# Samsung/tf-fast-rnnt

Hardware: AMD Instinct MI355X
Metric: rnnt_loss_pruned_fwd_bwd_throughput (higher is better)
Workload: dtype f32; 1 GPU; c3: rnnt_loss_pruned fwd+bwd step, B=32/GPU T=1000 S=200 C=500 s_range=5, regular, full boundary, first pass rnnt_loss_simple; global_batch=32, am_pruned=broadcast view

## Files before the change

### tf-fast-rnnt_amd/csrc/capi.hip

```cpp
#include "ftr_common.h"
#ifdef FTR_DIAG
#include "../../include/ftr_diag.h"
#endif
#include <stdlib.h>
#include <string.h>

namespace ftr {
namespace {
thread_local char g_err[512] = {0};
#ifdef FTR_DIAG
int g_mi_impl = -1;
#endif

int device_ok() {
  int n = 0;
  hipError_t e = hipGetDeviceCount(&n);
  if (e != hipSuccess || n <= 0) {
    (void)hipGetLastError();
    set_error("no usable HIP device (%s); this library has no CPU path", e == hipSuccess ? "device count is 0" : hipGetErrorString(e));
    return FTR_ERR_NO_DEVICE;
  }
  return FTR_OK;
}

// ... 547 lines not shown
  clear_error();
  FTR_TRY(check_builder(what, B >= 0 && T >= 1 && S >= 0 && C >= 1 && r >= 1, termination_symbol, C, true, hat));
  FTR_TRY(check_scale_stride(what, scale_stride));
  if (B == 0) return FTR_OK;
  FTR_TRY(pointers_then_device(what, logits && ranges && lse && gpy && glogits && (symbols || S == 0) && (gpx || S == 0)));
  return pruned_logprobs_bwd(logits, dtype, symbols, ranges, boundary, termination_symbol, lse, gpx, gpy, Scale{scale, scale_stride, scale_mul}, glogits, B, T, S, C, r, modified, hat, stream_of(stream));
}

int ftr_pruned_logprobs_bwd_scaled_f32(const float* logits, const int32_t* symbols, const int32_t* ranges,
                                       const int32_t* boundary, int termination_symbol, const float* lse,
                                       const float* gpx, const float* gpy, const float* scale, int scale_stride,
                                       float scale_mul, float* glogits, int B, int T, int S, int C, int r,
                                       int modified, void* stream) {
  return pruned_logprobs_bwd_scaled_entry(logits, FTR_DTYPE_F32, symbols, ranges, boundary, termination_symbol, lse, gpx, gpy, scale, scale_stride, scale_mul, glogits, B, T, S, C, r, modified, 0, stream);
}

int ftr_hat_pruned_logprobs_bwd_scaled_f32(const float* logits, const int32_t* symbols, const int32_t* ranges,
                                           const int32_t* boundary, int termination_symbol, const float* lse,
                                           const float* gpx, const float* gpy, const float* scale, int scale_stride,
                                           float scale_mul, float* glogits, int B, int T, int S, int C, int r,
                                           int modified, void* stream) {
  return pruned_logprobs_bwd_scaled_entry(logits, FTR_DTYPE_F32, symbols, ranges, boundary, termination_symbol, lse, gpx, gpy, scale, scale_stride, scale_mul, glogits, B, T, S, C, r, modified, 1, stream);
}

int ftr_pruned_logprobs_bwd_scaled_dt(const void* logits, int kind, const int32_t* symbols, const int32_t* ranges,
                                      const int32_t* boundary, int termination_symbol, const float* lse,
                                      const float* gpx, const float* gpy, const float* scale, int scale_stride,
                                      float scale_mul, void* glogits, int B, int T, int S, int C, int r, int modified,
                                      int flags, void* stream) {
  clear_error();
  FTR_TRY(check_dtype("pruned_logprobs_bwd_scaled_dt", kind, flags));
  return pruned_logprobs_bwd_scaled_entry(logits, kind, symbols, ranges, boundary, termination_symbol, lse, gpx, gpy, scale, scale_stride, scale_mul, glogits, B, T, S, C, r, modified, flags & FTR_PRUNED_HAT, stream);
}

int ftr_simple_logprobs_fused_supported(int C) { return simple_fused_supported(C); }
int ftr_simple_logprobs_fused_bwd_supported(int T, int C) { return simple_fused_bwd_supported(T, C); }

int ftr_normalizer_gemm_f32(int kind, const float* x, const float* y, float* out, int B, int T, int S1, int C, void* stream) {
  FTR_REQUIRE(B >= 0 && T >= 0 && S1 >= 0 && C >= 0, "normalizer_gemm: bad sizes");
  if ((size_t)B * T * S1 * C == 0) return FTR_OK;
  FTR_REQUIRE(x && y && out, "normalizer_gemm: null pointer");
  return normalizer_gemm(kind, x, y, out, B, T, S1, C, reinterpret_cast<hipStream_t>(stream));
}

int ftr_normalizer_gemm_choice(int kind, int B, int T, int S1, int C, int* solution, float* us, float* us_default, int* candidates) {
  return normalizer_gemm_choice(kind, B, T, S1, C, solution, us, us_default, candidates);
}

int ftr_normalizer_gemm_set_choice(int kind, int B, int T, int S1, int C, int solution) {
  return normalizer_gemm_set_choice(kind, B, T, S1, C, solution);
}

static int fused_fwd_entry(const char* what, bool smoothed, const float* am, const float* lm, const int32_t* symbols,
                           const float* am_probs, const float* lm_probs, const float* am_max, const float* lm_max,
                           const float* lmonly_norm, const float* amonly_norm, const float* unigram_log,
                           const int32_t* boundary, int termination_symbol, double delay_penalty, float combined_scale,
                           float lm_only_scale, float am_only_scale, float* px, float* py, float* prod, int B, int T,
                           int S, int C, int modified, void* stream) {
  clear_error();
  FTR_TRY(check_builder(what, B >= 0 && T >= 1 && S >= 0 && C >= 1, termination_symbol, C));
  if (B == 0) return FTR_OK;
  FTR_TRY(pointers_then_device(what, am && lm && am_probs && lm_probs && am_max && lm_max && (!smoothed || (lmonly_norm && amonly_norm && unigram_log)) && py && (symbols || S == 0) && (px || S == 0)));
  return simple_fused_fwd(am, lm, symbols, am_probs, lm_probs, am_max, lm_max, boundary, termination_symbol, delay_penalty, lmonly_norm, amonly_norm, unigram_log, combined_scale, lm_only_scale, am_only_scale, px, py, prod, B, T, S, C, modified, stream_of(stream));
}

int ftr_simple_logprobs_fused_fwd_f32(const float* am, const float* lm, const int32_t* symbols, const float* am_probs,
                                      const float* lm_probs, const float* am_max, const float* lm_max,
                                      const int32_t* boundary, int termination_symbol, double delay_penalty, float* px,
                                      float* py, float* prod, int B, int T, int S, int C, int modified, void* stream) {
  return fused_fwd_entry("simple_logprobs_fused_fwd", false, am, lm, symbols, am_probs, lm_probs, am_max, lm_max, nullptr, nullptr, nullptr, boundary, termination_symbol, delay_penalty, 1.0f, 0.0f, 0.0f, px, py, prod, B, T, S, C, modified, stream);
}

int ftr_smoothed_logprobs_fused_fwd_f32(const float* am, const float* lm, const int32_t* symbols, const float* am_probs,
                                        const float* lm_probs, const float* am_max, const float* lm_max,
                                        const float* lmonly_norm, const float* amonly_norm, const float* unigram_log,
                                        const int32_t* boundary, int termination_symbol, double delay_penalty,
                                        float combined_scale, float lm_only_scale, float am_only_scale, float* px,
                                        float* py, float* prod, int B, int T, int S, int C, int modified, void* stream) {
  return fused_fwd_entry("smoothed_logprobs_fused_fwd", true, am, lm, symbols, am_probs, lm_probs, am_max, lm_max, lmonly_norm, amonly_norm, unigram_log, boundary, termination_symbol, delay_penalty, combined_scale, lm_only_scale, am_only_scale, px, py, prod, B, T, S, C, modified, stream);
}

static int fused_bwd_am_entry(const char* what, bool smoothed, const float* gpx, const float* gpy, const float* scale,
                              int scale_stride, float scale_mul, const float* prod, const float* lm_probs,
                              const float* am_probs, const int32_t* symbols, const int32_t* boundary,
                              int termination_symbol, float combined_scale, float direct_scale, const float* unigram,
                              const float* am_dot, float am_only_scale, float* R, float* d_am, int B, int T, int S, int C,
                              int modified, void* stream) {
  clear_error();
  FTR_TRY(check_builder(what, B >= 0 && T >= 1 && S >= 0 && C >= 1, termination_symbol, C, true));
  FTR_TRY(check_scale_stride(what, scale_stride));
  if (B == 0) return FTR_OK;
  FTR_TRY(pointers_then_device(what, gpy && prod && lm_probs && am_probs && d_am && (!smoothed || (unigram && am_dot && R)) && (gpx || S == 0) && (symbols || S == 0)));
  return simple_fused_bwd_am(gpx, gpy, Scale{scale, scale_stride, scale_mul}, prod, lm_probs, am_probs, symbols, boundary, termination_symbol, combined_scale, direct_scale, unigram, am_dot, am_only_scale, R, d_am, B, T, S, C, modified, stream_of(stream));
}

int ftr_simple_logprobs_fused_bwd_am_f32(const float* gpx, const float* gpy, const float* scale, int scale_stride,
                                         float scale_mul, const float* prod, const float* lm_probs, const float* am_probs,
                                         const int32_t* symbols, const int32_t* boundary, int termination_symbol,
                                         float* d_am, int B, int T, int S, int C, int modified, void* stream) {
  return fused_bwd_am_entry("simple_logprobs_fused_bwd_am", false, gpx, gpy, scale, scale_stride, scale_mul, prod, lm_probs, am_probs, symbols, boundary, termination_symbol, 1.0f, 1.0f, nullptr, nullptr, 0.0f, nullptr, d_am, B, T, S, C, modified, stream);
}

int ftr_smoothed_logprobs_fused_bwd_am_f32(const float* gpx, const float* gpy, const float* scale, int scale_stride,
                                           float scale_mul, const float* prod, const float* lm_probs,
                                           const float* am_probs, const int32_t* symbols, const int32_t* boundary,
                                           int termination_symbol, float combined_scale, float direct_scale,
                                           const float* unigram, const float* am_dot, float am_only_scale, float* R,
                                           float* d_am, int B, int T, int S, int C, int modified, void* stream) {
  return fused_bwd_am_entry("smoothed_logprobs_fused_bwd_am", true, gpx, gpy, scale, scale_stride, scale_mul, prod, lm_probs, am_probs, symbols, boundary, termination_symbol, combined_scale, direct_scale, unigram, am_dot, am_only_scale, R, d_am, B, T, S, C, modified, stream);
}

static int fused_bwd_am_w_entry(const char* what, bool smoothed, const float* gpx, const float* gpy, const float* scale,
                                int scale_stride, float scale_mul, const float* W, const float* lm_probs,
                                const float* am_probs, const int32_t* symbols, const int32_t* boundary,
                                int termination_symbol, float direct_scale, const float* unigram, const float* am_dot,
                                float am_only_scale, float* R, float* d_am, int B, int T, int S, int C, int modified,
                                void* stream) {
  clear_error();
  FTR_TRY(check_builder(what, B >= 0 && T >= 1 && S >= 0 && C >= 1, termination_symbol, C, true));
  FTR_TRY(check_scale_stride(what, scale_stride));
  if (B == 0) return FTR_OK;
  FTR_TRY(pointers_then_device(what, gpy && W && lm_probs && am_probs && d_am && (!smoothed || (unigram && am_dot && R)) && (gpx || S == 0) && (symbols || S == 0)));
  return simple_fused_bwd_am_w(gpx, gpy, Scale{scale, scale_stride, scale_mul}, W, lm_probs, am_probs, symbols, boundary, termination_symbol, direct_scale, unigram, am_dot, am_only_scale, R, d_am, B, T, S, C, modified, stream_of(stream));
}

int ftr_simple_logprobs_fused_bwd_am_w_f32(const float* gpx, const float* gpy, const float* scale, int scale_stride,
                                           float scale_mul, const float* W, const float* lm_probs, const float* am_probs,
                                           const int32_t* symbols, const int32_t* boundary, int termination_symbol,
                                           float* d_am, int B, int T, int S, int C, int modified, void* stream) {
  return fused_bwd_am_w_entry("simple_logprobs_fused_bwd_am_w", false, gpx, gpy, scale, scale_stride, scale_mul, W, lm_probs, am_probs, symbols, boundary, termination_symbol, 1.0f, nullptr, nullptr, 0.0f, nullptr, d_am, B, T, S, C, modified, stream);
}

int ftr_smoothed_logprobs_fused_bwd_am_w_f32(const float* gpx, const float* gpy, const float* scale, int scale_stride,
                                             float scale_mul, const float* W, const float* lm_probs,
                                             const float* am_probs, const int32_t* symbols, const int32_t* boundary,
                                             int termination_symbol, float direct_scale, const float* unigram,
                                             const float* am_dot, float am_only_scale, float* R, float* d_am, int B, int T,
                                             int S, int C, int modified, void* stream) {
  return fused_bwd_am_w_entry("smoothed_logprobs_fused_bwd_am_w", true, gpx, gpy, scale, scale_stride, scale_mul, W, lm_probs, am_probs, symbols, boundary, termination_symbol, direct_scale, unigram, am_dot, am_only_scale, R, d_am, B, T, S, C, modified, stream);
}

int ftr_simple_logprobs_fused_bwd_am_w_columns(int B, int T, int C) { return simple_fused_bwd_columns(B, T, C); }

int ftr_mutual_information_band_supported(int T, int S, int r) { return mi_band_supported(T, S, r); }

static int pruned_band_fwd_entry(const void* logits, int dtype, const int32_t* symbols, const int32_t* ranges, const int32_t* boundary,
                                 int termination_symbol, double delay_penalty, float* lse, float* px_band, float* py_band,
                                 int B, int T, int S, int C, int r, int modified, int hat, void* stream) {
  const char* what = hat ? "hat_pruned_band_fwd" : "pruned_band_fwd";
  clear_error();
  FTR_TRY(check_builder(what, B >= 0 && T >= 1 && S >= 0 && C >= 1 && r >= 1, termination_symbol, C, false, hat));
  if (B == 0) return FTR_OK;
  FTR_TRY(pointers_then_device(what, logits && ranges && lse && px_band && py_band && (symbols || S == 0)));
  FTR_TRY(lse_rows_dtype(logits, dtype, lse, (size_t)B * T * r, C, termination_symbol, hat, stream_of(stream)));
  return band_gather(logits, dtype, symbols, ranges, boundary, lse, termination_symbol, delay_penalty, px_band, py_band, B, T, S, C, r, modified, hat, stream_of(stream));
}

int ftr_pruned_band_fwd_f32(const float* logits, const int32_t* symbols, const int32_t* ranges, const int32_t* boundary,
                            int termination_symbol, double delay_penalty, float* lse, float* px_band, float* py_band,
                            int B, int T, int S, int C, int r, int modified, void* stream) {
  return pruned_band_fwd_entry(logits, FTR_DTYPE_F32, symbols, ranges, boundary, termination_symbol, delay_penalty, lse, px_band, py_band, B, T, S, C, r, modified, 0, stream);
}

int ftr_hat_pruned_band_fwd_f32(const float* logits, const int32_t* symbols, const int32_t* ranges, const int32_t* boundary,
                                int termination_symbol, double delay_penalty, float* lse, float* px_band, float* py_band,
                                int B, int T, int S, int C, int r, int modified, void* stream) {
  return pruned_band_fwd_entry(logits, FTR_DTYPE_F32, symbols, ranges, boundary, termination_symbol, delay_penalty, lse, px_band, py_band, B, T, S, C, r, modified, 1, stream);
}

int ftr_pruned_band_fwd_dt(const void* logits, int kind, const int32_t* symbols, const int32_t* ranges,
                           const int32_t* boundary, int termination_symbol, double delay_penalty, float* lse,
                           float* px_band, float* py_band, int B, int T, int S, int C, int r, int modified, int flags,
                           void* stream) {
  clear_error();
  FTR_TRY(check_dtype("pruned_band_fwd_dt", kind, flags));
  return pruned_band_fwd_entry(logits, kind, symbols, ranges, boundary, termination_symbol, delay_penalty, lse, px_band, py_band, B, T, S, C, r, modified, flags & FTR_PRUNED_HAT, stream);
}

int ftr_band_ranges_check_i32(const int32_t* ranges, const int32_t* boundary, int32_t* flags, int B, int T, int r, void* stream) {
  clear_error();
  FTR_TRY(check_sizes("band_ranges_check", B >= 0 && T >= 0 && r >= 1));
  FTR_TRY(pointers_then_device("band_ranges_check", flags && (ranges || B == 0 || T == 0)));
  return band_ranges_check(ranges, boundary, flags, B, T, r, stream_of(stream));
}

int ftr_mutual_information_band_f32(const float* px_band, const float* py_band, const int32_t* ranges,
                                    const int32_t* boundary, float* ans, float* gx_band, float* gy_band, int B, int T,
                                    int S, int r, int modified, void* stream) {
  return ftr_mutual_information_band_ws_f32(px_band, py_band, ranges, boundary, nullptr, 0, ans, gx_band, gy_band, B, T, S, r, modified, stream);
}

size_t ftr_mutual_information_band_workspace_floats(int B, int T, int S, int r) {
  return (B < 0 || T < 1 || S < 0 || r < 1) ? 0 : mi_band_workspace_floats(B, T, S, r);
}

int ftr_mutual_information_band_ws_f32(const float* px_band, const float* py_band, const int32_t* ranges,
                                       const int32_t* boundary, float* workspace, size_t workspace_floats, float* ans,
                                       float* gx_band, float* gy_band, int B, int T, int S, int r, int modified,
                                       void* stream) {
  clear_error();
  FTR_TRY(check_sizes("mutual_information_band", B >= 0 && T >= 1 && S >= 0 && r >= 1));
  if (B == 0) return FTR_OK;
  FTR_TRY(pointers_then_device("mutual_information_band", px_band && py_band && ranges && ans && gx_band && gy_band));
  return mi_band(px_band, py_band, ranges, boundary, workspace, workspace_floats, ans, gx_band, gy_band, B, T, S, r, modified, stream_of(stream));
}

static int pruned_band_bwd_scaled_entry(const void* logits, int dtype, const int32_t* symbols, const int32_t* ranges,
                                        const int32_t* boundary, int termination_symbol, const float* lse,
                                        const float* gx_band, const float* gy_band, const float* scale, int scale_stride,
                                        float scale_mul, void* glogits, int B, int T, int S, int C, int r, int modified,
                                        int hat, void* stream) {
  const char* what = hat ? "hat_pruned_band_bwd_scaled" : "pruned_band_bwd_scaled";
  clear_error();
  FTR_TRY(check_builder(what, B >= 0 && T >= 1 && S >= 0 && C >= 1 && r >= 1, termination_symbol, C, true, hat));
  FTR_TRY(check_scale_stride(what, scale_stride));
  if (B == 0) return FTR_OK;
  FTR_TRY(pointers_then_device(what, logits && ranges && lse && gx_band && gy_band && glogits && (symbols || S == 0)));
  return band_grad_banded(logits, dtype, symbols, ranges, boundary, termination_symbol, lse, gx_band, gy_band, Scale{scale, scale_stride, scale_mul}, glogits, B, T, S, C, r, modified, hat, stream_of(stream));
}

int ftr_pruned_band_bwd_scaled_f32(const float* logits, const int32_t* symbols, const int32_t* ranges,
                                   const int32_t* boundary, int termination_symbol, const float* lse,
                                   const float* gx_band, const float* gy_band, const float* scale, int scale_stride,
                                   float scale_mul, float* glogits, int B, int T, int S, int C, int r, int modified,
                                   void* stream) {
  return pruned_band_bwd_scaled_entry(logits, FTR_DTYPE_F32, symbols, ranges, boundary, termination_symbol, lse, gx_band, gy_band, scale, scale_stride, scale_mul, glogits, B, T, S, C, r, modified, 0, stream);
}

int ftr_hat_pruned_band_bwd_scaled_f32(const float* logits, const int32_t* symbols, const int32_t* ranges,
                                       const int32_t* boundary, int termination_symbol, const float* lse,
                                       const float* gx_band, const float* gy_band, const float* scale, int scale_stride,
                                       float scale_mul, float* glogits, int B, int T, int S, int C, int r, int modified,
                                       void* stream) {
  return pruned_band_bwd_scaled_entry(logits, FTR_DTYPE_F32, symbols, ranges, boundary, termination_symbol, lse, gx_band, gy_band, scale, scale_stride, scale_mul, glogits, B, T, S, C, r, modified, 1, stream);
}

int ftr_pruned_band_bwd_scaled_dt(const void* logits, int kind, const int32_t* symbols, const int32_t* ranges,
                                  const int32_t* boundary, int termination_symbol, const float* lse,
                                  const float* gx_band, const float* gy_band, const float* scale, int scale_stride,
                                  float scale_mul, void* glogits, int B, int T, int S, int C, int r, int modified,
                                  int flags, void* stream) {
  clear_error();
  FTR_TRY(check_dtype("pruned_band_bwd_scaled_dt", kind, flags));
  return pruned_band_bwd_scaled_entry(logits, kind, symbols, ranges, boundary, termination_symbol, lse, gx_band, gy_band, scale, scale_stride, scale_mul, glogits, B, T, S, C, r, modified, flags & FTR_PRUNED_HAT, stream);
}

namespace {
int mb_check_durations(const char* what, const int32_t* durations, int D, bool first_is_one) {
  FTR_REQUIRE(D >= 1 && D <= 8, "%s: D = %d, the number of blanks must be in 1..8", what, D);
  FTR_REQUIRE(durations, "%s: null durations", what);
  for (int j = 0; j < D; ++j) {
    FTR_REQUIRE(durations[j] >= 1 && durations[j] <= 32, "%s: durations[%d] = %d is outside 1..32", what, j, durations[j]);
    FTR_REQUIRE(j == 0 || durations[j] > durations[j - 1], "%s: durations must be strictly increasing (durations[%d] = %d after %d)",
                what, j, durations[j], durations[j - 1]);
  }
  FTR_REQUIRE(!first_is_one || durations[0] == 1, "%s: durations[0] = %d, the standard blank advances one frame", what, durations[0]);
  return FTR_OK;
}
int mb_check_ids(const char* what, const int32_t* ids, int D, int blank, int C) {
  FTR_REQUIRE(C >= 1 && blank >= 0 && blank < C, "%s: termination_symbol %d not in [0,%d)", what, blank, C);
  FTR_REQUIRE(ids || D == 1, "%s: null big_blank_ids", what);
  for (int j = 0; j + 1 < D; ++j) {
    FTR_REQUIRE(ids[j] >= 0 && ids[j] < C, "%s: big_blank_ids[%d] = %d not in [0,%d)", what, j, ids[j], C);
    FTR_REQUIRE(ids[j] != blank, "%s: big_blank_ids[%d] = %d is the termination_symbol", what, j, ids[j]);
    for (int i = 0; i < j; ++i)
      FTR_REQUIRE(ids[i] != ids[j], "%s: big_blank_ids[%d] = %d is a duplicate of big_blank_ids[%d]", what, j, ids[j], i);
  }
  return FTR_OK;
}
}

namespace {
int tdt_check_list(const char* what, const char* name, const int32_t* v, int n, int nmax, int lo, int hi = 16) {
  FTR_REQUIRE(n >= 1 && n <= nmax, "%s: %s holds %d values, must be 1..%d", what, name, n, nmax);
  FTR_REQUIRE(v, "%s: null %s", what, name);
  for (int j = 0; j < n; ++j) {
    FTR_REQUIRE(v[j] >= lo && v[j] <= hi, "%s: %s[%d] = %d is outside %d..%d", what, name, j, v[j], lo, hi);
    FTR_REQUIRE(j == 0 || v[j] > v[j - 1], "%s: %s must be strictly increasing (%s[%d] = %d after %d)", what, name, name, j,
                v[j], v[j - 1]);
  }
  return FTR_OK;
}
int tdt_check_moves(const char* what, const int32_t* token_durations, int Dx, const int32_t* blank_durations, int Dy,
                    int blank_hi = 16) {
  FTR_TRY(tdt_check_list(what, "token_durations", token_durations, Dx, 8, 0));
  FTR_TRY(tdt_check_list(what, "blank_durations", blank_durations, Dy, 8, 1, blank_hi));
  FTR_REQUIRE(Dx + Dy <= 9, "%s: Dx + Dy = %d moves (token_durations and blank_durations together), at most 9", what, Dx + Dy);
  return FTR_OK;
}
int tdt_check_head(const char* what, const int32_t* durations, int N, double sigma, int blank, int C) {
  FTR_TRY(tdt_check_list(what, "durations", durations, N, 5, 0));
  FTR_REQUIRE(durations[N - 1] >= 1, "%s: durations holds no positive value: no move advances a frame", what);
  FTR_REQUIRE(sigma >= 0.0, "%s: sigma = %g must not be negative", what, sigma);
  FTR_REQUIRE(C >= 1 && blank >= 0 && blank < C, "%s: termination_symbol %d not in [0,%d)", what, blank, C);
  return FTR_OK;
}
}

size_t ftr_mutual_information_multiblank_workspace_floats(int B, int S, int T) {
  return mi_multiblank_workspace_floats(B, S, T);
}

int ftr_mutual_information_multiblank_fwd_f32(const float* px, const float* py, const int32_t* boundary,
                                              const int32_t* durations, int D, float* workspace, size_t workspace_floats,
                                              float* ans, int B, int S, int T, void* stream) {
  const char* what = "mutual_information_multiblank_fwd";
  clear_error();
  FTR_TRY(mb_check_durations(what, durations, D, false));
  FTR_TRY(check_lattice(what, B, S, T));
  if (B == 0) return FTR_OK;
  FTR_TRY(check_ws_size(what, workspace_floats, mi_multiblank_workspace_floats(B, S, T), "floats"));
  FTR_REQUIRE(workspace && ans && (py || T == 0) && (px || S == 0), "%s: null px / py / workspace / ans", what);
  FTR_TRY(check_ws_aligned(what, workspace));
  FTR_TRY(device_ok());
  return mi_multiblank_fwd(px, py, boundary, durations, D, workspace, workspace_floats, ans, B, S, T, stream_of(stream));
}

int ftr_mutual_information_multiblank_bwd_f32(const float* px, const float* py, const int32_t* boundary,
                                              const int32_t* durations, int D, float* workspace, size_t workspace_floats,
                                              const float* ans_grad, float* px_grad, float* py_grad, int B, int S, int T,
                                              void* stream) {
  const char* what = "mutual_information_multiblank_bwd";
  clear_error();
  FTR_TRY(mb_check_durations(what, durations, D, false));
  FTR_TRY(check_lattice(what, B, S, T));
  if (B == 0) return FTR_OK;
  FTR_TRY(check_ws_size(what, workspace_floats, mi_multiblank_workspace_floats(B, S, T), "floats"));
  FTR_REQUIRE(workspace && (py || T == 0) && (px || S == 0), "%s: null px / py / workspace", what);
  FTR_REQUIRE((py_grad || T == 0) && (px_grad || S == 0), "%s: null px_grad / py_grad", what);
// ... 201 lines not shown
```

### tf-fast-rnnt_amd/csrc/ftr_common.h

```cpp
#pragma once
#include <hip/hip_runtime.h>
#include <stdint.h>
#include <stdio.h>
#include <stdarg.h>
#include "../../include/ftr_kd.h"
#include "../../include/ftr_fused.h"

namespace ftr {

void set_error(const char* fmt, ...);
void clear_error();

inline int check_launch(const char* what) {
  hipError_t e = hipGetLastError();
  if (e != hipSuccess) {
    set_error("%s: launch failed: %s", what, hipGetErrorString(e));
    return FTR_ERR_LAUNCH;
  }
  return FTR_OK;
}

inline int require_rows_32bit(const char* what, size_t rows) {
  if (rows > 0x7fffffffull) {
    set_error("%s: %zu rows (B*T*s_range) exceed the 2^31 - 1 that the launch grids index", what, rows);
    return FTR_ERR_INVALID_ARG;
  }
  return FTR_OK;
}

__global__ void zero_words_kernel(uint32_t* __restrict__ p, size_t n);
__global__ void copy_words_kernel(uint32_t* __restrict__ dst, const uint32_t* __restrict__ src, size_t n);
inline int zero_words(void* p, size_t n_words, hipStream_t st, const char* what) {
  if (n_words == 0) return FTR_OK;
  const size_t blocks = (n_words + 4 * 256 - 1) / (4 * 256);
  hipLaunchKernelGGL(zero_words_kernel, dim3((unsigned)(blocks > 4096 ? 4096 : blocks)), dim3(256), 0, st, static_cast<uint32_t*>(p), n_words);
  return check_launch(what);
}
inline int copy_words(void* dst, const void* src, size_t n_words, hipStream_t st, const char* what) {
  if (n_words == 0) return FTR_OK;
  const size_t blocks = (n_words + 255) / 256;
  hipLaunchKernelGGL(copy_words_kernel, dim3((unsigned)(blocks > 4096 ? 4096 : blocks)), dim3(256), 0, st, static_cast<uint32_t*>(dst),
                     static_cast<const uint32_t*>(src), n_words);
  return check_launch(what);
}

constexpr float kNeg = -1.0e30f;
constexpr float kNegThresh = -1.0e29f;
constexpr float kLog2e = 1.4426950408889634f;
constexpr float kLn2 = 0.6931471805599453f;

typedef float f4u __attribute__((ext_vector_type(4), aligned(4)));
typedef float f4 __attribute__((ext_vector_type(4)));

struct bf16_t { uint16_t bits; };
struct fp16_t { uint16_t bits; };
typedef uint16_t h4 __attribute__((ext_vector_type(4)));

__device__ __forceinline__ float elem_to_float(float v) { return v; }
__device__ __forceinline__ float elem_to_float(bf16_t v) { return (float)__builtin_bit_cast(__bf16, v.bits); }
__device__ __forceinline__ float elem_to_float(fp16_t v) { return (float)__builtin_bit_cast(_Float16, v.bits); }
template <typename E> __device__ __forceinline__ E elem_from_float(float v);
template <> __device__ __forceinline__ float elem_from_float<float>(float v) { return v; }
template <> __device__ __forceinline__ bf16_t elem_from_float<bf16_t>(float v) { return bf16_t{__builtin_bit_cast(uint16_t, (__bf16)v)}; }
template <> __device__ __forceinline__ fp16_t elem_from_float<fp16_t>(float v) { return fp16_t{__builtin_bit_cast(uint16_t, (_Float16)v)}; }

__device__ __forceinline__ f4 load4(const float* row, int i) { return reinterpret_cast<const f4u*>(row)[i]; }
__device__ __forceinline__ void store4(float* row, int i, f4 v) { reinterpret_cast<f4u*>(row)[i] = v; }
template <typename E>
__device__ __forceinline__ f4 load4(const E* row, int i) {
  const h4 h = reinterpret_cast<const h4*>(row)[i];
  f4 v;
#pragma unroll
  for (int e = 0; e < 4; ++e) v[e] = elem_to_float(E{h[e]});
  return v;
}
template <typename E>
__device__ __forceinline__ void store4(E* row, int i, f4 v) {
  h4 h;
#pragma unroll
  for (int e = 0; e < 4; ++e) h[e] = elem_from_float<E>(v[e]).bits;
  reinterpret_cast<h4*>(row)[i] = h;
}

struct Scale {
  const float* p; int stride; float mul;
  __device__ __forceinline__ float at(int b) const { return (p ? p[(size_t)b * stride] : 1.0f) * mul; }
};
inline Scale scale_none() { return Scale{nullptr, 0, 1.0f}; }

template <int CTRL, int ROW_MASK, int BANK_MASK>
__device__ __forceinline__ float dpp_take(float identity, float src) {
  return __builtin_bit_cast(float, __builtin_amdgcn_update_dpp(__builtin_bit_cast(int, identity), __builtin_bit_cast(int, src),
                                                               CTRL, ROW_MASK, BANK_MASK, false));
}
__device__ __forceinline__ float wave_sum_dpp(float v) {
  v += dpp_take<0x111, 0xf, 0xf>(0.0f, v);
  v += dpp_take<0x112, 0xf, 0xf>(0.0f, v);
  v += dpp_take<0x114, 0xf, 0xe>(0.0f, v);
  v += dpp_take<0x118, 0xf, 0xc>(0.0f, v);
  v += dpp_take<0x142, 0xa, 0xf>(0.0f, v);
  v += dpp_take<0x143, 0xc, 0xf>(0.0f, v);
  return __builtin_bit_cast(float, __builtin_amdgcn_readlane(__builtin_bit_cast(int, v), 63));
}
__device__ __forceinline__ float wave_max_dpp(float v) {
  constexpr float ninf = -__builtin_inff();
  v = fmaxf(v, dpp_take<0x111, 0xf, 0xf>(ninf, v));
  v = fmaxf(v, dpp_take<0x112, 0xf, 0xf>(ninf, v));
  v = fmaxf(v, dpp_take<0x114, 0xf, 0xe>(ninf, v));
  v = fmaxf(v, dpp_take<0x118, 0xf, 0xc>(ninf, v));
  v = fmaxf(v, dpp_take<0x142, 0xa, 0xf>(ninf, v));
  v = fmaxf(v, dpp_take<0x143, 0xc, 0xf>(ninf, v));
  return __builtin_bit_cast(float, __builtin_amdgcn_readlane(__builtin_bit_cast(int, v), 63));
}

struct Shift { float cx2, cy2; };
__device__ __forceinline__ bool shift_sample_ok(float v) { return v > -1.0e4f && v < 1.0e4f; }
template <bool MOD>
__device__ __forceinline__ Shift shift_from_sums(float sumx, float nx, float sumy, float ny, int Sn, int Tn) {
  const float steps = MOD ? (float)(Tn - 1) : (float)(Sn - 1 + Tn - 1);
  float f = steps > 0.0f ? (float)(Sn - 1) / steps : 0.5f;
  f = fminf(fmaxf(f, 1.0e-3f), 1.0f - 1.0e-3f);
  const float mx = nx > 0.0f ? sumx / nx : 0.0f, my = ny > 0.0f ? sumy / ny : 0.0f;
  Shift s;
  s.cx2 = mx * kLog2e - __builtin_amdgcn_logf(f);
  s.cy2 = my * kLog2e - __builtin_amdgcn_logf(1.0f - f);
  return s;
}
template <bool MOD>
__device__ __forceinline__ double shift_total(const Shift s, int Sn, int Tn) {
  const int nx = Sn - 1, ny = MOD ? (Tn - 1) - (Sn - 1) : (Tn - 1);
  return (double)nx * (double)s.cx2 + (double)ny * (double)s.cy2;
}

struct Bound { int sb, tb, se, te; };
__device__ __forceinline__ Bound load_boundary(const int32_t* __restrict__ boundary, int b, int S, int T) {
  Bound r;
  if (boundary) {
    r.sb = max(boundary[4 * b + 0], 0); r.tb = max(boundary[4 * b + 1], 0);
    r.se = min(boundary[4 * b + 2], S); r.te = min(boundary[4 * b + 3], T);
  } else { r.sb = 0; r.tb = 0; r.se = S; r.te = T; }
  return r;
}

__device__ __forceinline__ float softplus(float v) { return fmaxf(v, 0.0f) + log1pf(expf(-fabsf(v))); }
__device__ __forceinline__ void hat_logprobs(float xb, float xs, float Z, bool sym_is_blank, float* vx, float* vy) {
  *vy = -softplus(-xb);
  *vx = sym_is_blank ? -INFINITY : (xs - Z) - softplus(xb);
}
__device__ __forceinline__ void hat_sigmoids(float xb, float* sp, float* sn) {
  const float e = expf(-fabsf(xb)), big = 1.0f / (1.0f + e), small = e / (1.0f + e);
  *sp = xb >= 0.0f ? big : small;
  *sn = xb >= 0.0f ? small : big;
}

}

namespace ftr {
int mi_plain_fwd(const float* px, const float* py, const int32_t* boundary, float* p, float* ans, int B, int S, int T, int modified, hipStream_t st);
int mi_plain_bwd(const float* px, const float* py, const int32_t* boundary, const float* p, float* p_grad, float* px_grad, float* py_grad, float* ans_grad, int overwrite, int B, int S, int T, int modified, hipStream_t st);
int mi_bidir_fwd(const float* px, const float* py, const int32_t* boundary, float* ws, size_t ws_floats, int flags, float* ans, int B, int S, int T, int modified, hipStream_t st);
int mi_bidir_bwd(const int32_t* boundary, const float* ws, size_t ws_floats, int flags, float* px_grad, float* py_grad, float* ans_grad, int overwrite, int B, int S, int T, int modified, hipStream_t st, const float* ans = nullptr, float* loss_out = nullptr, int loss_code = 0);
int mi_bidir_ws_init(float* ws, size_t ws_floats, int B, int S, int T, hipStream_t st);
int mi_bidir_status(const float* ws, size_t ws_floats, int B, int S, int T, int* status_host, long long* dirty_host, hipStream_t st);
size_t mi_bidir_workspace_floats(int B, int S, int T);
size_t mi_bidir_handoff_floats(int B, int S, int T);
size_t mi_viterbi_workspace_bytes(int B, int S, int T);
int mi_viterbi(const float* px, const float* py, const int32_t* boundary, void* ws, size_t ws_bytes, float* score, int32_t* frames, int B, int S, int T, int modified, hipStream_t st);
size_t mi_multiblank_workspace_floats(int B, int S, int T);
int mi_multiblank_fwd(const float* px, const float* py, const int32_t* boundary, const int32_t* durations, int D, float* ws, size_t ws_floats, float* ans, int B, int S, int T, hipStream_t st);
int mi_multiblank_bwd(const float* px, const float* py, const int32_t* boundary, const int32_t* durations, int D, float* ws, size_t ws_floats, const float* ans_grad, float* px_grad, float* py_grad, int B, int S, int T, hipStream_t st);
int multiblank_logprobs_fwd(const float* logits, const int32_t* symbols, const int32_t* ranges, const int32_t* boundary, int blank, const int32_t* big_ids, const int32_t* durations, int D, double sigma, double delay_penalty, float* lse, float* px, float* py, int B, int T, int S, int C, int r, hipStream_t st);
int multiblank_logprobs_bwd(const float* logits, const int32_t* symbols, const int32_t* ranges, const int32_t* boundary, int blank, const int32_t* big_ids, const int32_t* durations, int D, const float* lse, const float* gpx, const float* gpy, Scale scale, float* glogits, int B, int T, int S, int C, int r, hipStream_t st);
size_t mi_tdt_workspace_floats(int B, int S, int T);
int mi_tdt_fwd(const float* px, const float* py, const int32_t* boundary, const int32_t* token_durations, int Dx, const int32_t* blank_durations, int Dy, float* ws, size_t ws_floats, float* ans, int B, int S, int T, hipStream_t st);
int mi_tdt_bwd(const float* px, const float* py, const int32_t* boundary, const int32_t* token_durations, int Dx, const int32_t* blank_durations, int Dy, float* ws, size_t ws_floats, const float* ans_grad, float* px_grad, float* py_grad, int B, int S, int T, hipStream_t st);
int tdt_logprobs_fwd(const float* logits, const int32_t* symbols, const int32_t* ranges, const int32_t* boundary, int blank, const int32_t* durations, int N, double sigma, double delay_penalty, float* lse_tok, float* lse_dur, float* px, float* py, int B, int T, int S, int C, int r, hipStream_t st);
int tdt_logprobs_bwd(const float* logits, const int32_t* symbols, const int32_t* ranges, const int32_t* boundary, int blank, const int32_t* durations, int N, const float* lse_tok, const float* lse_dur, const float* gpx, const float* gpy, Scale scale, float* glogits, int B, int T, int S, int C, int r, hipStream_t st);
size_t mi_viterbi_tdt_workspace_bytes(int B, int S, int T);
int mi_viterbi_tdt(const float* px, const float* py, const int32_t* boundary, const int32_t* token_durations, int Dx, const int32_t* blank_durations, int Dy, void* ws, size_t ws_bytes, float* score, int32_t* frames, int32_t* durations, int32_t* blank_steps, int B, int S, int T, hipStream_t st);
int cummin_i32(const int32_t* in, int32_t* out, int rows, int cols, hipStream_t st);
int prune_ranges(const float* px_grad, const float* py_grad, const int32_t* boundary, int32_t* ranges, int32_t* s_begin, int B, int S, int T, int T1, int r, hipStream_t st);
int do_pruning(const float* am, const float* lm, const int32_t* ranges, float* am_p, float* lm_p, int B, int T, int S1, int C, int r, hipStream_t st);
size_t do_pruning_bwd_workspace_bytes(int B, int T, int S1, int C, int r);
int do_pruning_bwd_ws(const float* g_am_p, const float* g_lm_p, const int32_t* ranges, float* d_am, float* d_lm, int B, int T, int S1, int C, int r, void* ws, size_t ws_bytes, hipStream_t st);
int do_pruning_bwd(const float* g_am_p, const float* g_lm_p, const int32_t* ranges, float* d_am, float* d_lm, int B, int T, int S1, int C, int r, hipStream_t st);
int pruned_logprobs_fwd(const void* logits, int dtype, const int32_t* symbols, const int32_t* ranges, const int32_t* boundary, int blank, double delay_penalty, float* lse, float* px, float* py, int B, int T, int S, int C, int r, int modified, int hat, hipStream_t st);
int pruned_logprobs_bwd(const void* logits, int dtype, const int32_t* symbols, const int32_t* ranges, const int32_t* boundary, int blank, const float* lse, const float* gpx, const float* gpy, Scale scale, void* glogits, int B, int T, int S, int C, int r, int modified, int hat, hipStream_t st);
int simple_rowmax_exp(const float* x, float* probs, float* rowmax, float* rowsum, const float* dotvec, float* dot, size_t rows, int C, hipStream_t st);
int simple_rowmax_exp_pair(const float* x1, float* probs1, float* rowmax1, size_t rows1, const float* x2, float* probs2, float* rowmax2, size_t rows2, int C, hipStream_t st);
int simple_rowdot(const float* x, const float* v, float* dot, size_t rows, int C, hipStream_t st);
size_t simple_colsum_workspace_floats(size_t rows, int C);
int simple_colsum_weighted(const float* x, const float* w, float* out, float* ws, size_t ws_floats, size_t rows, int C, hipStream_t st);
int simple_logprobs_fwd(const float* am, const float* lm, const int32_t* symbols, const float* prod, const float* am_max, const float* lm_max, const int32_t* boundary, int blank, double delay_penalty, const float* lmonly_norm, const float* amonly_norm, const float* ulog, float cs, float ls, float as, float* px, float* py, int B, int T, int S, int C, int modified, hipStream_t st);
int simple_logprobs_bwd_w(const float* gpx, const float* gpy, Scale scale, const float* prod, const int32_t* boundary, float* W, float* rsx, float* rsy, float cs, int B, int T, int S, int modified, hipStream_t st);
int simple_logprobs_bwd_am(const float* gpx, const float* gpy, Scale scale, const float* damp, const float* am_probs, const int32_t* symbols, const int32_t* boundary, int blank, float kdir, const float* uvec, const float* amdot, float as, float* Rout, float* d_am, int B, int T, int S, int C, int modified, hipStream_t st);
int simple_logprobs_bwd_lm(const float* dlmp, const float* lm_probs, const int32_t* symbols, const float* rsx, const float* rsy, int blank, float kdir, const float* arow, const float* invsum, const float* gu, float* d_lm, int B, int S, int C, hipStream_t st);
int simple_fused_supported(int C);
int simple_fused_bwd_supported(int T, int C);
int normalizer_gemm(int kind, const float* x, const float* y, float* out, int B, int T, int S1, int C, hipStream_t st);
int normalizer_gemm_choice(int kind, int B, int T, int S1, int C, int* solution, float* us, float* us_default, int* candidates);
int normalizer_gemm_set_choice(int kind, int B, int T, int S1, int C, int solution);
int simple_fused_fwd(const float* am, const float* lm, const int32_t* symbols, const float* am_probs, const float* lm_probs, const float* am_max, const float* lm_max, const int32_t* boundary, int blank, double delay_penalty, const float* lmonly_norm, const float* amonly_norm, const float* ulog, float cs, float ls, float as, float* px, float* py, float* prod_out, int B, int T, int S, int C, int modified, hipStream_t st);
int simple_fused_bwd_am(const float* gpx, const float* gpy, Scale scale, const float* prod, const float* lm_probs, const float* am_probs, const int32_t* symbols, const int32_t* boundary, int blank, float cs, float kdir, const float* uvec, const float* amdot, float as, float* Rout, float* d_am, int B, int T, int S, int C, int modified, hipStream_t st);
int simple_fused_bwd_columns(int B, int T, int C);
int simple_fused_bwd_am_w(const float* gpx, const float* gpy, Scale scale, const float* W, const float* lm_probs, const float* am_probs, const int32_t* symbols, const int32_t* boundary, int blank, float kdir, const float* uvec, const float* amdot, float as, float* Rout, float* d_am, int B, int T, int S, int C, int modified, hipStream_t st);
int negated_reduce(const float* ans, int B, int reduction, float* out, hipStream_t st, float sign = -1.0f);
int pruned_kd_fwd(const void* logits, int dtype, const void* teacher, int teacher_dtype, const int32_t* symbols, const int32_t* ranges, const int32_t* boundary, int blank, float temperature, int collapsed, float* node, float* saved, float* utt, int B, int T, int S, int C, int r, hipStream_t st);
int pruned_kd_bwd(const void* logits, int dtype, const void* teacher, int teacher_dtype, const int32_t* symbols, const int32_t* ranges, const int32_t* boundary, int blank, float temperature, int collapsed, const float* saved, Scale scale, void* glogits, int B, int T, int S, int C, int r, hipStream_t st);
int lse_rows(const float* logits, float* lse, size_t rows, int C, int blank, int hat, hipStream_t st);
int lse_rows_dtype(const void* logits, int dtype, float* lse, size_t rows, int C, int blank, int hat, hipStream_t st);
int mi_band_supported(int T, int S, int r);
int band_ranges_check(const int32_t* ranges, const int32_t* boundary, int* flags, int B, int T, int r, hipStream_t st);
int band_gather(const void* logits, int dtype, const int32_t* symbols, const int32_t* ranges, const int32_t* boundary, const float* lse, int blank, double delay_penalty, float* pxb, float* pyb, int B, int T, int S, int C, int r, int modified, int hat, hipStream_t st);
size_t mi_band_workspace_floats(int B, int T, int S, int r);
int mi_band_seg_supported(int T, int S, int r);
size_t mi_band_seg_workspace_floats(int B, int T, int S, int r);
int mi_band_seg(const float* pxb, const float* pyb, const int32_t* ranges, const int32_t* boundary, float* ws, size_t ws_floats, float* ans, float* gxb, float* gyb, int B, int T, int S, int r, int modified, hipStream_t st);
int mi_band(const float* pxb, const float* pyb, const int32_t* ranges, const int32_t* boundary, float* ws, size_t ws_floats, float* ans, float* gxb, float* gyb, int B, int T, int S, int r, int modified, hipStream_t st);
int band_grad_banded(const void* logits, int dtype, const int32_t* symbols, const int32_t* ranges, const int32_t* boundary, int blank, const float* lse, const float* gxb, const float* gyb, Scale scale, void* glogits, int B, int T, int S, int C, int r, int modified, int hat, hipStream_t st);
int selftest(hipStream_t st, int* result_dev);
int debug_stamps(unsigned long long* out16);
int debug_trace(unsigned long long* out, int n);
}
```

### tf-fast-rnnt_amd/csrc/mi_band.hip

```cpp
#include "ftr_common.h"
#include "launch.h"
#include <type_traits>
#include <cstdlib>

namespace ftr {
namespace {

constexpr int kBandThreads = 512;

__device__ __forceinline__ float dpp_row_ror1(float v) {
  return __builtin_bit_cast(float, __builtin_amdgcn_update_dpp(0, __builtin_bit_cast(int, v), 0x121, 0xf, 0xf, false));
}
template <int N>
__device__ __forceinline__ float dpp_row_ror(float v) {
  return __builtin_bit_cast(float, __builtin_amdgcn_update_dpp(0, __builtin_bit_cast(int, v), 0x120 + N, 0xf, 0xf, false));
}
__device__ __forceinline__ float row16_max(float v) {
  v = fmaxf(v, dpp_row_ror<8>(v)); v = fmaxf(v, dpp_row_ror<4>(v));
  v = fmaxf(v, dpp_row_ror<2>(v)); v = fmaxf(v, dpp_row_ror<1>(v));
  return v;
}
__device__ __forceinline__ float row16_sum(float v) {
  v += dpp_row_ror<8>(v); v += dpp_row_ror<4>(v); v += dpp_row_ror<2>(v); v += dpp_row_ror<1>(v);
  return v;
}

template <typename E, bool MOD, bool HAT>
__global__ void band_gather_kernel(const E* __restrict__ logits, const int32_t* __restrict__ symbols,
                                   const int32_t* __restrict__ ranges, const int32_t* __restrict__ boundary,
                                   const float* __restrict__ lse, int blank, double delay_penalty,
                                   float* __restrict__ pxb, float* __restrict__ pyb, size_t rows, int T, int S, int C, int r) {
  const size_t row = (size_t)blockIdx.x * blockDim.x + threadIdx.x;
  if (row >= rows) return;
  const size_t bt = row / r;
  const int k = (int)(row - bt * r);
  const int b = (int)(bt / T);
  const int t = (int)(bt - (size_t)b * T);
  const int s = ranges[bt * r] + k;
  const int te = boundary ? boundary[4 * b + 3] : T;
  const float l = lse[row];
  float vy = -INFINITY, vx = -INFINITY;
  if (s >= 0 && s <= S) {
    if (HAT) {
      const float xb = elem_to_float(logits[row * C + blank]);
      int c = blank;
      if (s < S) c = min(max(symbols[(size_t)b * S + s], 0), C - 1);
      hat_logprobs(xb, elem_to_float(logits[row * C + c]), l, c == blank, &vx, &vy);
    } else {
      vy = elem_to_float(logits[row * C + blank]) - l;
    }
    if (s < S) {
      if (!HAT) vx = elem_to_float(logits[row * C + min(max(symbols[(size_t)b * S + s], 0), C - 1)]) - l;
      if (!MOD && t == te) vx = -INFINITY;
      if (delay_penalty > 0.0) vx += (float)((((double)te - 1.0) / 2.0 - (double)t) * delay_penalty);
    }
  }
  pxb[row] = vx;
  pyb[row] = vy;
}

__global__ void band_ranges_check_kernel(const int32_t* __restrict__ ranges, const int32_t* __restrict__ boundary,
                                         int* __restrict__ flags, int B, int T, int r) {
  const size_t bt = (size_t)blockIdx.x * blockDim.x + threadIdx.x;
  int bad = 0;
  if (bt < (size_t)B * T) {
    const int b = (int)(bt / T), t = (int)(bt - (size_t)b * T);
    const int tb = boundary ? max(boundary[4 * b + 1], 0) : 0, te = boundary ? min(boundary[4 * b + 3], T) : T;
    if (t >= tb && t < te) {
      const int32_t* row = ranges + bt * r;
      const int s0 = row[0];
      if (t > tb && s0 < row[-r]) bad |= 1;
      for (int k = 1; k < r; ++k) if (row[k] != s0 + k) bad |= 2;
    }
  }
  if (__any(bad != 0)) {
    int all = 0;
    for (int bit = 1; bit <= 2; bit <<= 1) if (__any((bad & bit) != 0)) all |= bit;
    if ((threadIdx.x & 63) == 0) atomicOr(flags, all);
  }
}

#ifdef FTR_BAND_STAMPS
static __device__ unsigned long long g_bstamp[16];
#define FTR_BSTAMP(k) do { if (b == 0 && tid == 0) g_bstamp[k] = __builtin_amdgcn_s_memrealtime(); } while (0)
#else
#define FTR_BSTAMP(k) do {} while (0)
#endif
constexpr int kBandAhead = 4;
constexpr int kRenormEvery = 4;
template <int LANES>
__host__ __device__ inline size_t band_lds_bytes(int T, int S) {
  const size_t ncap = ((size_t)S + T + 5 + 4 * kBandAhead) * LANES;
  return sizeof(int) * ((size_t)(T + 2) + 32) + sizeof(float) * (3 * ncap + 48) + 64;
}

template <bool MOD, int LANES>
__global__ __launch_bounds__(kBandThreads) void mi_band_kernel(
    const float* __restrict__ pxb, const float* __restrict__ pyb, const int32_t* __restrict__ ranges,
    const int32_t* __restrict__ boundary, float* __restrict__ ans, float* __restrict__ gxb, float* __restrict__ gyb,
    int B, int T, int S, int r, unsigned rinv) {
  extern __shared__ __attribute__((aligned(16))) unsigned char smem[];
  const int b = blockIdx.x;
  const int tid = threadIdx.x;
  const int lane = tid & 63;
  const int wave = __builtin_amdgcn_readfirstlane(tid >> 6);
  const Bound bd = load_boundary(boundary, b, S, T);
  const int Sn = bd.se - bd.sb + 1, Tn = bd.te - bd.tb + 1;
  const size_t cells_g = (size_t)T * r;
  float* gx_g = gxb + (size_t)b * cells_g;
  float* gy_g = gyb + (size_t)b * cells_g;
  if (Sn <= 0 || Tn <= 0 || Tn == 1) {
    for (size_t i = tid; i < cells_g; i += kBandThreads) { gx_g[i] = 0.0f; gy_g[i] = 0.0f; }
    if (tid == 0) ans[b] = (Sn <= 0 || Tn <= 0) ? 0.0f : ((Sn == 1) ? 0.0f : -INFINITY);
    return;
  }
  FTR_BSTAMP(0);
  const int te = bd.te, tb = bd.tb, sb = bd.sb, se = bd.se;
  const int D = (MOD ? 0 : (Sn - 1)) + (Tn - 1);
  const int jm = D >> 1;
  const int rowA = 1 + 2 * kBandAhead, rowB = rowA + jm + 2;
  int* lo = reinterpret_cast<int*>(smem);
  int* cutSA = lo + ((T + 2) & ~1); int* cutSB = cutSA + 16;
  const int ncap = (S + T + 5 + 4 * kBandAhead) * LANES;
  float2* O2 = reinterpret_cast<float2*>(cutSB + 16);
  float* G = reinterpret_cast<float*>(O2 + ncap);
  float* cutA = G + ncap; float* cutB = cutA + 16; float* occ = cutB + 16;
  auto div_r = [&](int i) { return rinv ? (int)__umulhi((unsigned)i, rinv) : i; };

  const int32_t* rg = ranges + (size_t)b * T * r;
  for (int t0 = 0; t0 <= T; t0 += 4 * kBandThreads) {
    int v[4];
#pragma unroll
    for (int u = 0; u < 4; ++u) { const int t = t0 + u * kBandThreads + tid; v[u] = (t <= T) ? rg[(size_t)min(t, te - 1) * r] : 0; }
#pragma unroll
    for (int u = 0; u < 4; ++u) { const int t = t0 + u * kBandThreads + tid; if (t <= T) lo[t] = v[u]; }
  }
  for (int i = tid; i < ncap; i += kBandThreads) O2[i] = make_float2(kNeg, kNeg);
  if (tid < 32) cutSA[tid] = -1;
  __syncthreads();
  FTR_BSTAMP(1);
  {
    int bad = 0;
    for (int t = tb + 1 + tid; t < te; t += kBandThreads) bad |= (lo[t] < lo[t - 1]);
    if (__syncthreads_or(bad)) {
      for (size_t i = tid; i < cells_g; i += kBandThreads) { gx_g[i] = 0.0f; gy_g[i] = 0.0f; }
      if (tid == 0) ans[b] = __builtin_nanf("");
      return;
    }
  }
  if (tid < LANES) O2[(rowA + jm + 1) * LANES + tid] = make_float2(kNeg, 0.0f);
  const bool end_above = MOD && se == lo[te] + r;
  auto in_band = [&](int s, int t) { const int l = lo[t]; return (s >= l && s <= l + r - 1) || (end_above && t == te && s == se); };
  auto slotA = [&](int s, int t) { return (rowA + (MOD ? (t - tb) : (s - sb) + (t - tb))) * LANES + ((s - sb) & (LANES - 1)); };
  auto slotB = [&](int s, int t) { return (rowB + (MOD ? (te - t) : (se - s) + (te - t))) * LANES + ((se - s) & (LANES - 1)); };

  const int nfr = (te - tb) * r;
  float* red = cutA;
  auto stage = [&](const float* src) {
    const float* g0 = src + ((size_t)b * T + tb) * r;
    float ssum = 0.0f, scnt = 0.0f;
    for (int i0 = 0; i0 < nfr; i0 += 8 * 4 * kBandThreads) {
      f4 v[8];
#pragma unroll
      for (int u = 0; u < 8; ++u) {
        const int i = i0 + 4 * (u * kBandThreads + tid);
        if (i + 3 < nfr) v[u] = *reinterpret_cast<const f4u*>(g0 + i);
        else { v[u] = f4{0.f, 0.f, 0.f, 0.f}; for (int e = 0; e < 4; ++e) if (i + e < nfr) v[u][e] = g0[i + e]; }
      }
#pragma unroll
      for (int u = 0; u < 8; ++u) {
        const int i = i0 + 4 * (u * kBandThreads + tid);
        for (int e = 0; e < 4; ++e) if (i + e < nfr) {
          G[i + e] = v[u][e] * kLog2e;
          if (shift_sample_ok(v[u][e])) { ssum += v[u][e]; scnt += 1.0f; }
        }
      }
    }
    ssum = wave_sum_dpp(ssum); scnt = wave_sum_dpp(scnt);
    if (lane == 0) { red[wave] = ssum; red[8 + wave] = scnt; }
  };
  auto staged_sums = [&](float& sum, float& cnt) {
    sum = 0.0f; cnt = 0.0f;
#pragma unroll
    for (int u = 0; u < kBandThreads / 64; ++u) { sum += red[u]; cnt += red[8 + u]; }
  };
  auto staged = [&](int s, int t) { return G[(t - tb) * r + (s - lo[t])]; };
  unsigned nan_acc = 0;
  auto operands = [&](auto xtag, const float c2) {
    constexpr bool ISX = decltype(xtag)::value;
    float* O = reinterpret_cast<float*>(O2) + (ISX ? 0 : 1);
    for (int i = tid; i < Tn * r; i += kBandThreads) {
      const int q = div_r(i);
      const int t = tb + q, k = i - q * r;
      const int s = lo[t] + k;
      if (s < sb || s > se) continue;
      const int dg = MOD ? (t - tb) : (s - sb) + (t - tb);
      if (dg <= jm) {
        float av = kNeg;
        if (ISX) { const int tx = MOD ? t - 1 : t; if (s - 1 >= sb && tx >= tb && tx <= te - 1 && in_band(s - 1, tx)) av = staged(s - 1, tx) - c2; }
        else { if (t - 1 >= tb && in_band(s, t - 1)) av = staged(s, t - 1) - c2; if (s == sb && t == tb) av = 0.0f; }
        nan_acc = max(nan_acc, __float_as_uint(av) & 0x7fffffffu);
        O[2 * slotA(s, t)] = fmaxf(av, kNeg);
        if (ISX && dg == jm) cutSA[(s - sb) & (LANES - 1)] = s;
      }
      if (dg >= jm) {
        float bv = kNeg;
        if (t <= te - 1) {
          if (ISX) { const int tnx = MOD ? t + 1 : t; if (s + 1 <= se && tnx <= te && in_band(s + 1, tnx)) bv = staged(s, t) - c2; }
          else if (in_band(s, t + 1)) bv = staged(s, t) - c2;
        }
        if (!ISX && s == se && t == te) bv = 0.0f;
// ... 352 lines not shown
    {
      float g[NS][U];
#pragma unroll
      for (int k = 0; k < NS - 1; ++k)
#pragma unroll
        for (int u = 0; u < U; ++u) g[k][u] = G[top - (1 + k * U + u) * LANES];
      for (int i = 1; i < 1 + nrun2; i += P) {
#pragma unroll
        for (int k = 0; k < NS; ++k) {
          const int kf = (k + NS - 1) % NS;
#pragma unroll
          for (int u = 0; u < U; ++u) g[kf][u] = G[top - (i + (k + NS - 1) * U + u) * LANES];
#pragma unroll
          for (int u = 0; u < U; ++u) flow(top - (i + k * U + u) * LANES, g[k][u], std::false_type{});
        }
      }
    }
    __builtin_amdgcn_s_waitcnt(0);
  }
  __syncthreads();
  __threadfence();
  for (int i = tid; i < T * r; i += kBandThreads) {
    const int t = div_r(i), k = i - t * r;
    float fx = 0.0f, fy = 0.0f;
    if (t >= tb && t < te) {
      const int s = lo[t] + k;
      if (s >= sb && s <= se) {
        const int dg = MOD ? (t - tb) : (s - sb) + (t - tb);
        if (dg < jm) { const float2 f = O2[slotA(s, t)]; fx = f.x; fy = f.y; }
        else {
          const int tnx = MOD ? t + 1 : t;
          if (s + 1 <= se && tnx <= te && in_band(s + 1, tnx)) fx = O2[slotB(s + 1, tnx)].x;
          if (in_band(s, t + 1)) fy = O2[slotB(s, t + 1)].y;
        }
      }
    }
    gx_g[i] = fx;
    gy_g[i] = fy;
  }
}

template <typename E, bool VEC, bool HAT>
__global__ void band_grad_banded_kernel(const E* __restrict__ logits, const int32_t* __restrict__ symbols,
                                        const int32_t* __restrict__ ranges, const int32_t* __restrict__ boundary,
                                        const float* __restrict__ lse, const float* __restrict__ gxb,
                                        const float* __restrict__ gyb, const Scale scale, int blank, int modified,
                                        E* __restrict__ glogits, size_t rows, int T, int S, int C, int r) {
  const int lane = threadIdx.x & 63;
  const size_t rowi = (size_t)blockIdx.x * (blockDim.x >> 6) + (threadIdx.x >> 6);
  if (rowi >= rows) return;
  const size_t row = rows - 1 - rowi;
  const size_t bt = row / r;
  const int k = (int)(row - bt * r);
  const int b = (int)(bt / T);
  const int t = (int)(bt - (size_t)b * T);
  const int s = ranges[bt * r] + k;
  const int te = boundary ? boundary[4 * b + 3] : T;
  const float sc = scale.at(b);
  float gx = 0.0f;
  int sym = blank;
  const bool sok = s >= 0 && s <= S;
  if (sok && s < S) {
    sym = symbols[(size_t)b * S + s];
    if (modified || t != te) gx = gxb[row] * sc;
  }
  const float gy = sok ? gyb[row] * sc : 0.0f;
  float tot = gx + gy;
  const float l = lse[row];
  if (HAT) {
    sym = min(max(sym, 0), C - 1);
    if (sym == blank) gx = 0.0f;
    tot = gx;
  }
  const E* x = logits + row * C;
  E* g = glogits + row * C;
  if (VEC) {
    const int n4 = C >> 2;
    for (int i = lane; i < n4; i += 64) {
      const f4 v = load4(x, i);
      f4 o;
#pragma unroll
      for (int e = 0; e < 4; ++e) {
        const int cc = 4 * i + e;
        float val = -tot * __expf(v[e] - l);
        if (cc == sym) val += gx;
        if (cc == blank) {
          if (HAT) {
            float sp, sn;
            hat_sigmoids(v[e], &sp, &sn);
            val = gy * sn - gx * sp;
          } else {
            val += gy;
          }
        }
        o[e] = val;
      }
      store4(g, i, o);
    }
  } else {
    for (int cc = lane; cc < C; cc += 64) {
      const float xc = elem_to_float(x[cc]);
      float val = -tot * __expf(xc - l);
      if (cc == sym) val += gx;
      if (cc == blank) {
        if (HAT) {
          float sp, sn;
          hat_sigmoids(xc, &sp, &sn);
          val = gy * sn - gx * sp;
        } else {
          val += gy;
        }
      }
      g[cc] = elem_from_float<E>(val);
    }
  }
}

}

static int band_lanes(int T, int S, int r) {
  if (r < 1 || T < 1 || S < 0) return 0;
  if (r <= 7 && band_lds_bytes<8>(T, S) <= (size_t)150 * 1024) return 8;
  if (r <= 15 && band_lds_bytes<16>(T, S) <= (size_t)150 * 1024) return 16;
  return 0;
}
static int band_stream_lanes(int T, int r) {
  if (r < 1 || r > 15 || band_stream_lds_bytes(T) > (size_t)150 * 1024) return 0;
  return r <= 7 ? 8 : 16;
}
int mi_band_supported(int T, int S, int r) {
  static const bool force_stream = getenv("FTR_BAND_FORCE_STREAM") != nullptr;
  if (!force_stream && band_lanes(T, S, r) != 0) return 1;
  return (T >= 1 && S >= 0 && band_stream_lanes(T, r) != 0) ? 2 : 0;
}
static size_t band_chain_workspace_floats(int B, int T, int S, int r) {
  if (mi_band_supported(T, S, r) != 2) return 0;
  const size_t per = band_stream_lanes(T, r) == 8 ? band_stream_floats_per_utt<8>(T, S) : band_stream_floats_per_utt<16>(T, S);
  return per * (size_t)B;
}
size_t mi_band_workspace_floats(int B, int T, int S, int r) {
  const size_t chain = band_chain_workspace_floats(B, T, S, r), seg = mi_band_seg_workspace_floats(B, T, S, r);
  return seg > chain ? seg : chain;
}

int band_ranges_check(const int32_t* ranges, const int32_t* boundary, int* flags, int B, int T, int r, hipStream_t st) {
  const int rcz = zero_words(flags, 1, st, "band_ranges_check");
  if (rcz != FTR_OK) return rcz;
  const size_t n = (size_t)B * T;
  if (n == 0) return FTR_OK;
  hipLaunchKernelGGL(band_ranges_check_kernel, dim3((unsigned)((n + 255) / 256)), dim3(256), 0, st, ranges, boundary, flags, B, T, r);
  return check_launch("band_ranges_check");
}

int band_gather(const void* logits, int dtype, const int32_t* symbols, const int32_t* ranges, const int32_t* boundary,
                const float* lse, int blank, double delay_penalty, float* pxb, float* pyb, int B, int T, int S, int C,
                int r, int modified, int hat, hipStream_t st) {
  const size_t rows = (size_t)B * T * r;
  if (rows == 0) return FTR_OK;
  { const int rc32 = require_rows_32bit("pruned_band_fwd", rows); if (rc32 != FTR_OK) return rc32; }
  const unsigned blocks = (unsigned)((rows + 255) / 256);
  dispatch_dtype(dtype, [&](auto tag) {
    using E = typename decltype(tag)::type;
    dispatch(modified != 0, [&](auto mod) {
      dispatch(hat != 0, [&](auto h) {
        hipLaunchKernelGGL((band_gather_kernel<E, decltype(mod)::value, decltype(h)::value>), dim3(blocks), dim3(256), 0, st,
                           static_cast<const E*>(logits), symbols, ranges, boundary, lse, blank, delay_penalty, pxb, pyb, rows, T, S, C, r);
      });
    });
  });
  return check_launch("band_gather");
}

constexpr size_t kBandLdsCeiling = 156 * 1024;

int mi_band(const float* pxb, const float* pyb, const int32_t* ranges, const int32_t* boundary, float* ws, size_t ws_floats,
            float* ans, float* gxb, float* gyb, int B, int T, int S, int r, int modified, hipStream_t st) {
  const int kind = mi_band_supported(T, S, r);
  if (!kind) { set_error("mutual_information_band: T=%d S=%d r=%d is outside the band kernels' domain (r <= 15)", T, S, r); return FTR_ERR_UNSUPPORTED; }
  if (B <= 65535 && mi_band_seg_supported(T, S, r) && ws && (reinterpret_cast<uintptr_t>(ws) & 15) == 0 && ws_floats >= mi_band_seg_workspace_floats(B, T, S, r))
    return mi_band_seg(pxb, pyb, ranges, boundary, ws, ws_floats, ans, gxb, gyb, B, T, S, r, modified, st);
  if ((uint64_t)(T + 1) * r * r >= (1ull << 32)) { set_error("mutual_information_band: T * r too large"); return FTR_ERR_UNSUPPORTED; }
  const unsigned rinv = (r == 1) ? 0u : (unsigned)(((1ull << 32) + r - 1) / r);
  if (kind == 2) {
    const size_t need = band_chain_workspace_floats(B, T, S, r);
    if (!ws || ws_floats < need || (reinterpret_cast<uintptr_t>(ws) & 15) != 0) {
      set_error("mutual_information_band: this size streams through a workspace of %zu floats (16-byte aligned), got %zu", need, ws_floats);
      return FTR_ERR_INVALID_ARG;
    }
    const size_t lds = band_stream_lds_bytes(T);
    return dispatch_among<8, 16>(band_stream_lanes(T, r), [&](auto lanes) {
      return dispatch(modified != 0, [&](auto mod) {
        constexpr auto kernel = mi_band_stream_kernel<decltype(mod)::value, decltype(lanes)::value>;
        const int rc = reserve_lds<kernel>(kBandLdsCeiling, "mutual_information_band");
        if (rc != FTR_OK) return rc;
        hipLaunchKernelGGL(kernel, dim3(B), dim3(kBandThreads), lds, st, pxb, pyb, ranges, boundary, ws, ans, gxb, gyb, B, T, S, r, rinv);
        return check_launch("mi_band_stream");
      });
    });
  }
  return dispatch_among<8, 16>(band_lanes(T, S, r), [&](auto lanes) {
    return dispatch(modified != 0, [&](auto mod) {
      constexpr int L = decltype(lanes)::value;
      constexpr auto kernel = mi_band_kernel<decltype(mod)::value, L>;
      const int rc = reserve_lds<kernel>(kBandLdsCeiling, "mutual_information_band");
      if (rc != FTR_OK) return rc;
      hipLaunchKernelGGL(kernel, dim3(B), dim3(kBandThreads), band_lds_bytes<L>(T, S), st, pxb, pyb, ranges, boundary, ans, gxb, gyb, B, T, S, r, rinv);
      return check_launch("mi_band");
    });
  });
}

#ifdef FTR_BAND_STAMPS
extern "C" int ftr_debug_band_stamps(unsigned long long* out) {
  return hipMemcpyFromSymbol(out, HIP_SYMBOL(g_bstamp), sizeof(unsigned long long) * 16) == hipSuccess ? 0 : 1;
}
#endif

int band_grad_banded(const void* logits, int dtype, const int32_t* symbols, const int32_t* ranges, const int32_t* boundary,
                     int blank, const float* lse, const float* gxb, const float* gyb, Scale scale, void* glogits, int B,
                     int T, int S, int C, int r, int modified, int hat, hipStream_t st) {
  const size_t rows = (size_t)B * T * r;
  if (rows == 0) return FTR_OK;
  { const int rc32 = require_rows_32bit("pruned_band_bwd", rows); if (rc32 != FTR_OK) return rc32; }
  const int wpb = 4;
  const unsigned blocks = (unsigned)((rows + wpb - 1) / wpb);
  dispatch_dtype(dtype, [&](auto tag) {
    using E = typename decltype(tag)::type;
    dispatch(rows_vec4<E>(C, logits, glogits), [&](auto vec) {
      dispatch(hat != 0, [&](auto h) {
        hipLaunchKernelGGL((band_grad_banded_kernel<E, decltype(vec)::value, decltype(h)::value>), dim3(blocks), dim3(64 * wpb), 0, st,
                           static_cast<const E*>(logits), symbols, ranges, boundary, lse, gxb, gyb, scale, blank, modified, static_cast<E*>(glogits), rows, T, S, C, r);
      });
    });
  });
  return check_launch("band_grad_banded");
}

}
```

### tf-fast-rnnt_amd/csrc/mi_band_seg.hip

```cpp
#include "ftr_common.h"
#include "launch.h"
#include <cstdlib>
#include <cstring>

namespace ftr {
namespace {

constexpr int kSegMaxK = 32;
constexpr int kSegTarget = 64;
constexpr int kSegU = 4;
constexpr int kSegFlagBad = 1, kSegFlagNaN = 2, kSegFlagNoOrigin = 4, kSegFlagNoEnd = 8;

__device__ __forceinline__ float seg_ror1(float v) {
  return __builtin_bit_cast(float, __builtin_amdgcn_update_dpp(0, __builtin_bit_cast(int, v), 0x121, 0xf, 0xf, false));
}
template <int N>
__device__ __forceinline__ float seg_ror(float v) {
  return __builtin_bit_cast(float, __builtin_amdgcn_update_dpp(0, __builtin_bit_cast(int, v), 0x120 + N, 0xf, 0xf, false));
}
__device__ __forceinline__ float seg_row_max(float v) {
  v = fmaxf(v, seg_ror<8>(v)); v = fmaxf(v, seg_ror<4>(v));
  v = fmaxf(v, seg_ror<2>(v)); v = fmaxf(v, seg_ror<1>(v));
  return v;
}

__device__ __forceinline__ double seg_ror1d(double v) {
  const int lo = __builtin_amdgcn_update_dpp(0, __double2loint(v), 0x121, 0xf, 0xf, false);
  const int hi = __builtin_amdgcn_update_dpp(0, __double2hiint(v), 0x121, 0xf, 0xf, false);
  return __hiloint2double(hi, lo);
}
template <int N>
__device__ __forceinline__ double seg_rord(double v) {
  const int lo = __builtin_amdgcn_update_dpp(0, __double2loint(v), 0x120 + N, 0xf, 0xf, false);
  const int hi = __builtin_amdgcn_update_dpp(0, __double2hiint(v), 0x120 + N, 0xf, 0xf, false);
  return __hiloint2double(hi, lo);
}
constexpr double kNegD = -1.0e30, kNegThreshD = -1.0e29;

struct SegGeom { int D, K, L; };
__host__ __device__ inline SegGeom seg_geom(int D) {
  const int steps = D + 1;
  int K = (steps + kSegTarget - 1) / kSegTarget;
  K = K > kSegMaxK ? kSegMaxK : (K < 1 ? 1 : K);
  const int L = (steps + K - 1) / K;
  K = (steps + L - 1) / L;
  return SegGeom{D, K, L};
}
__host__ __device__ inline int seg_lmax(int T, int S) {
  const int steps = S + T + 1;
  const int l = (steps + kSegMaxK - 1) / kSegMaxK;
  return l > kSegTarget ? l : kSegTarget;
}
__host__ __device__ inline size_t seg_rows(int T, int S) { return (size_t)S + T + 2 + seg_lmax(T, S) + 2 * kSegU + 2; }
template <int LANES>
__host__ __device__ inline size_t seg_floats_per_utt(int T, int S) {
  const size_t nr = seg_rows(T, S);
  const size_t f = 8 * nr * LANES + 2 * 2 * (size_t)kSegMaxK * (LANES * LANES + LANES) + 16;
  return (f + 3) & ~(size_t)3;
}
template <int LANES>
struct SegWs {
  float2* OA; float2* OB; double* PA; double* QB; double* M; double* ST; float* hdr;
  __device__ SegWs(float* base, int T, int S) {
    const size_t nr = seg_rows(T, S);
    OA = reinterpret_cast<float2*>(base); OB = OA + nr * LANES;
    PA = reinterpret_cast<double*>(base + 4 * nr * LANES); QB = PA + nr * LANES;
    M = QB + nr * LANES; ST = M + 2 * (size_t)kSegMaxK * (LANES * LANES);
    hdr = reinterpret_cast<float*>(ST + 2 * (size_t)kSegMaxK * LANES);
  }
  __device__ int* flags() const { return reinterpret_cast<int*>(hdr); }
  __device__ double* shift_back() const { return reinterpret_cast<double*>(hdr + 4); }
  __device__ double* mat(int dir, int seg) const { return M + ((size_t)dir * kSegMaxK + seg) * (LANES * LANES); }
  __device__ double* state(int dir, int seg) const { return ST + ((size_t)dir * kSegMaxK + seg) * LANES; }
};
constexpr int kRow0 = 1;

struct SegUtt { Bound bd; int Sn, Tn, D; bool degenerate; };
template <bool MOD>
__device__ __forceinline__ SegUtt seg_utt(const int32_t* boundary, int b, int S, int T) {
  SegUtt u;
  u.bd = load_boundary(boundary, b, S, T);
  u.Sn = u.bd.se - u.bd.sb + 1; u.Tn = u.bd.te - u.bd.tb + 1;
  u.degenerate = u.Sn <= 0 || u.Tn <= 0 || u.Tn == 1;
  u.D = (MOD ? 0 : (u.Sn - 1)) + (u.Tn - 1);
  return u;
}

template <bool MOD, int LANES>
__global__ __launch_bounds__(256) void band_seg_init_kernel(const float* __restrict__ pxb, const float* __restrict__ pyb,
                                                            const int32_t* __restrict__ ranges, const int32_t* __restrict__ boundary,
                                                            float* __restrict__ ws, int T, int S, int r) {
  const int b = blockIdx.y;
  const SegWs<LANES> w(ws + (size_t)b * seg_floats_per_utt<LANES>(T, S), T, S);
  const size_t n = 2 * seg_rows(T, S) * LANES;
  for (size_t i = (size_t)blockIdx.x * 256 + threadIdx.x; i < n; i += (size_t)gridDim.x * 256) w.OA[i] = make_float2(kNeg, 0.0f);
  if (blockIdx.x != 0) return;
  __shared__ float red[16];
  const SegUtt u = seg_utt<MOD>(boundary, b, S, T);
  if (threadIdx.x == 0) {
    int f = 0;
    if (!u.degenerate) {
      const int32_t* rg = ranges + (size_t)b * T * r;
      const int lo_b = rg[(size_t)min(u.bd.tb, u.bd.te - 1) * r], lo_e = rg[(size_t)(u.bd.te - 1) * r];
      if (!(u.bd.sb >= lo_b && u.bd.sb <= lo_b + r - 1)) f |= kSegFlagNoOrigin;
      if (!((u.bd.se >= lo_e && u.bd.se <= lo_e + r - 1) || (MOD && u.bd.se == lo_e + r))) f |= kSegFlagNoEnd;
    }
    *w.flags() = f;
  }
  if (u.degenerate) return;
  const float* pxu = pxb + (size_t)b * T * r;
  const float* pyu = pyb + (size_t)b * T * r;
  const unsigned nfr = (unsigned)(u.bd.te - u.bd.tb) * (unsigned)r;
  float sx = 0.0f, nx = 0.0f, sy = 0.0f, ny = 0.0f;
  float vx[8], vy[8];
#pragma unroll
  for (int q = 0; q < 8; ++q) {
    const unsigned i = (unsigned)u.bd.tb * (unsigned)r + __umulhi((unsigned)(threadIdx.x + 256 * q) * 0x9E3779B1u, nfr);
    vx[q] = pxu[i]; vy[q] = pyu[i];
  }
#pragma unroll
  for (int q = 0; q < 8; ++q) {
    if (shift_sample_ok(vx[q])) { sx += vx[q]; nx += 1.0f; }
    if (shift_sample_ok(vy[q])) { sy += vy[q]; ny += 1.0f; }
  }
  sx = wave_sum_dpp(sx); nx = wave_sum_dpp(nx); sy = wave_sum_dpp(sy); ny = wave_sum_dpp(ny);
  const int wave = threadIdx.x >> 6;
  if ((threadIdx.x & 63) == 0) { red[wave] = sx; red[4 + wave] = nx; red[8 + wave] = sy; red[12 + wave] = ny; }
  __syncthreads();
  if (threadIdx.x == 0) {
    float a = 0.f, c = 0.f, d = 0.f, e = 0.f;
    for (int q = 0; q < 4; ++q) { a += red[q]; c += red[4 + q]; d += red[8 + q]; e += red[12 + q]; }
    const Shift sh = shift_from_sums<MOD>(a, c, d, e, u.Sn, u.Tn);
    w.hdr[1] = sh.cx2; w.hdr[2] = sh.cy2;
    *w.shift_back() = shift_total<MOD>(sh, u.Sn, u.Tn);
  }
}

template <bool MOD, int LANES>
struct SegBand {
  const int32_t* rg; int r, sb, tb, se, te; bool end_above; int lo_te;
  __device__ SegBand(const int32_t* ranges, int b, int T, int r_, const Bound& bd) : rg(ranges + (size_t)b * T * r_), r(r_), sb(bd.sb), tb(bd.tb), se(bd.se), te(bd.te) {
    lo_te = lo(te);
    end_above = MOD && se == lo_te + r;
  }
  __device__ int lo(int t) const { return rg[(size_t)min(t, te - 1) * r]; }
  __device__ bool in_band(int s, int t, int l) const { return (s >= l && s <= l + r - 1) || (end_above && t == te && s == se); }
  __device__ int dgA(int s, int t) const { return MOD ? (t - tb) : (s - sb) + (t - tb); }
  __device__ int dgB(int s, int t) const { return MOD ? (te - t) : (se - s) + (te - t); }
  __device__ int slotA(int s, int t) const { return (kRow0 + dgA(s, t)) * LANES + ((s - sb) & (LANES - 1)); }
  __device__ int slotB(int s, int t) const { return (kRow0 + dgB(s, t)) * LANES + ((se - s) & (LANES - 1)); }
};

template <bool MOD, int LANES>
__device__ __forceinline__ void seg_cell_operands(const SegBand<MOD, LANES>& g, const float* __restrict__ pxu, const float* __restrict__ pyu,
                                                  float cx2, float cy2, int s, int t, int l0, int lm, int lp,
                                                  float& ax, float& ay, float& bx, float& by) {
  const int r = g.r, sb = g.sb, tb = g.tb, se = g.se, te = g.te;
  auto at = [&](const float* src, float c2, int ss, int tt, int l) { return __builtin_fmaf(src[(size_t)tt * r + (ss - l)], kLog2e, -c2); };
  ax = kNeg; ay = kNeg; bx = kNeg; by = kNeg;
  {
    const int tx = MOD ? t - 1 : t;
    const int lx = MOD ? lm : l0;
    if (s - 1 >= sb && tx >= tb && tx <= te - 1 && g.in_band(s - 1, tx, lx)) ax = at(pxu, cx2, s - 1, tx, lx);
    if (t - 1 >= tb && g.in_band(s, t - 1, lm)) ay = at(pyu, cy2, s, t - 1, lm);
    if (s == sb && t == tb) ay = 0.0f;
  }
  if (t <= te - 1) {
    const int tnx = MOD ? t + 1 : t;
    const int ln = MOD ? lp : l0;
    if (s + 1 <= se && tnx <= te && g.in_band(s + 1, tnx, ln)) bx = at(pxu, cx2, s, t, l0);
    if (g.in_band(s, t + 1, lp)) by = at(pyu, cy2, s, t, l0);
  }
  if (s == se && t == te) by = 0.0f;
}

template <bool MOD, int LANES>
__global__ __launch_bounds__(256) void band_seg_scatter_kernel(const float* __restrict__ pxb, const float* __restrict__ pyb,
                                                               const int32_t* __restrict__ ranges, const int32_t* __restrict__ boundary,
                                                               float* __restrict__ ws, int T, int S, int r) {
  const int b = blockIdx.y;
  const SegUtt u = seg_utt<MOD>(boundary, b, S, T);
  if (u.degenerate) return;
  const SegWs<LANES> w(ws + (size_t)b * seg_floats_per_utt<LANES>(T, S), T, S);
  const SegBand<MOD, LANES> g(ranges, b, T, r, u.bd);
  const int i = blockIdx.x * 256 + threadIdx.x;
  const int q = i / r, k = i - q * r;
  const int t = u.bd.tb + q;
  if (t > u.bd.te) return;
  const float cx2 = w.hdr[1], cy2 = w.hdr[2];
  const float* pxu = pxb + (size_t)b * T * r;
  const float* pyu = pyb + (size_t)b * T * r;
  const int sb = u.bd.sb, tb = u.bd.tb, se = u.bd.se, te = u.bd.te;
  const int l0 = g.lo(t), lm = t > tb ? g.lo(t - 1) : l0, lp = t < te ? g.lo(t + 1) : l0;
  unsigned nan_acc = 0;
  int bad = 0;
  if (k == 0 && t > tb && t < te && l0 < lm) bad = kSegFlagBad;
  auto at = [&](const float* src, float c2, int s, int tt, int l) { return __builtin_fmaf(src[(size_t)tt * r + (s - l)], kLog2e, -c2); };
  auto put = [&](float2* O, int slot, float x, float y) {
    nan_acc = max(nan_acc, max(__float_as_uint(x) & 0x7fffffffu, __float_as_uint(y) & 0x7fffffffu));
    O[slot] = make_float2(fmaxf(x, kNeg), fmaxf(y, kNeg));
  };
  const int s = l0 + k;
  if (s >= sb && s <= se) {
    float ax, ay, bx, by;
    seg_cell_operands<MOD, LANES>(g, pxu, pyu, cx2, cy2, s, t, l0, lm, lp, ax, ay, bx, by);
    put(w.OA, g.slotA(s, t), ax, ay);
    put(w.OB, g.slotB(s, t), bx, by);
  }
  if (g.end_above && i == 0) {
    float ax = kNeg;
    const int lq = g.lo(te - 1);
    if (se - 1 >= sb && te - 1 >= tb && g.in_band(se - 1, te - 1, lq)) ax = at(pxu, cx2, se - 1, te - 1, lq);
    put(w.OA, g.slotA(se, te), ax, kNeg);
    w.OB[g.slotB(se, te)] = make_float2(kNeg, 0.0f);
  }
  int fl = bad | ((nan_acc > 0x7f800000u) ? kSegFlagNaN : 0);
  if (__any(fl != 0)) {
    int all = 0;
    for (int bit = 1; bit <= 2; bit <<= 1) if (__any((fl & bit) != 0)) all |= bit;
    if ((threadIdx.x & 63) == 0) atomicOr(w.flags(), all);
  }
}

template <int LANES, bool STORE>
__device__ __forceinline__ void seg_chain(const float2* __restrict__ seg, int L, int lg, double& val, double* __restrict__ pbuf, bool writer) {
  constexpr int U = kSegU;
  auto fwd = [&](int row, float2 o) {
    const double up = seg_ror1d(val);
    const double a_ = up + (double)o.x, b_ = val + (double)o.y;
    const float d = (float)(a_ - b_);
    const float ex = __builtin_amdgcn_exp2f(-__builtin_fabsf(d));
    val = fmax(a_, b_) + (double)__builtin_amdgcn_logf(1.0f + ex);
    if (STORE && writer) pbuf[row * LANES + lg] = val;
  };
  float2 oa[U], ob[U];
#pragma unroll
  for (int q = 0; q < U; ++q) oa[q] = seg[q * LANES + lg];
  int i = 0;
  for (; i + 2 * U <= L; i += 2 * U) {
#pragma unroll
    for (int q = 0; q < U; ++q) ob[q] = seg[(i + U + q) * LANES + lg];
#pragma unroll
    for (int q = 0; q < U; ++q) fwd(i + q, oa[q]);
#pragma unroll
    for (int q = 0; q < U; ++q) oa[q] = seg[(i + 2 * U + q) * LANES + lg];
#pragma unroll
    for (int q = 0; q < U; ++q) fwd(i + U + q, ob[q]);
  }
  for (; i < L; ++i) fwd(i, seg[i * LANES + lg]);
}

template <int LANES>
__device__ __forceinline__ void seg_stage(float2* __restrict__ seg, const float2* __restrict__ O, int row0, int L, int tid, int nthreads) {
  const int n = (L + 2 * kSegU) * LANES;
  const float2* src = O + (size_t)row0 * LANES;
  for (int i = tid; i < n; i += nthreads) seg[i] = src[i];
}

template <bool MOD, int LANES>
__global__ __launch_bounds__(16 * LANES) void band_seg_transfer_kernel(const int32_t* __restrict__ boundary, float* __restrict__ ws, int T, int S) {
  extern __shared__ __attribute__((aligned(16))) float2 seg[];
  const int sg = blockIdx.x, dir = blockIdx.y, b = blockIdx.z;
  const SegUtt u = seg_utt<MOD>(boundary, b, S, T);
  if (u.degenerate) return;
  const SegGeom gm = seg_geom(u.D);
  if (sg >= gm.K - 1) return;
  const SegWs<LANES> w(ws + (size_t)b * seg_floats_per_utt<LANES>(T, S), T, S);
  seg_stage<LANES>(seg, dir ? w.OB : w.OA, kRow0 + sg * gm.L, gm.L, threadIdx.x, 16 * LANES);
  __syncthreads();
  const int l16 = threadIdx.x & 15, lg = l16 & (LANES - 1);
  const int basis = threadIdx.x >> 4;
  double val = (lg == basis) ? 0.0 : kNegD;
  seg_chain<LANES, false>(seg, gm.L, lg, val, nullptr, false);
  double* m = w.mat(dir, sg);
  if (l16 < LANES) m[basis * LANES + lg] = val;
}

template <bool MOD, int LANES>
__global__ __launch_bounds__(64) void band_seg_prefix_kernel(const int32_t* __restrict__ boundary, float* __restrict__ ws, int T, int S) {
  extern __shared__ __attribute__((aligned(16))) double mats[];
  const int dir = blockIdx.x, b = blockIdx.y;
  const SegUtt u = seg_utt<MOD>(boundary, b, S, T);
  if (u.degenerate) return;
  const SegGeom gm = seg_geom(u.D);
  const SegWs<LANES> w(ws + (size_t)b * seg_floats_per_utt<LANES>(T, S), T, S);
  const int lane = threadIdx.x, l16 = lane & 15, lg = l16 & (LANES - 1);
  const int nm = (gm.K - 1) * LANES * LANES;
  const double* m0 = w.mat(dir, 0);
  for (int i = lane; i < nm; i += 64) mats[i] = m0[i];
  const bool start_ok = (*w.flags() & (dir ? kSegFlagNoEnd : kSegFlagNoOrigin)) == 0;
  double val = (lg == 0 && start_ok) ? 0.0 : kNegD;
  if (lane < LANES) w.state(dir, 0)[lg] = val;
  __syncthreads();
  for (int g = 0; g + 1 < gm.K; ++g) {
    const double* m = mats + (size_t)g * LANES * LANES;
    double tt[LANES];
    double best = kNegD;
#pragma unroll
    for (int i = 0; i < LANES; ++i) {
      double si = val;
      switch (i) {
        case 0: break;
#define FTR_ROT(N) case N: si = seg_rord<N>(val); break;
        FTR_ROT(1) FTR_ROT(2) FTR_ROT(3) FTR_ROT(4) FTR_ROT(5) FTR_ROT(6) FTR_ROT(7) FTR_ROT(8)
        FTR_ROT(9) FTR_ROT(10) FTR_ROT(11) FTR_ROT(12) FTR_ROT(13) FTR_ROT(14) FTR_ROT(15)
#undef FTR_ROT
      }
      const int src = (lg - i) & (LANES - 1);
      tt[i] = si + m[src * LANES + lg];
      best = fmax(best, tt[i]);
    }
    if (best > kNegThreshD) {
      float sum = 0.0f;
#pragma unroll
      for (int i = 0; i < LANES; ++i) sum += __builtin_amdgcn_exp2f((float)(tt[i] - best));
      val = best + (double)__builtin_amdgcn_logf(sum);
    } else {
      val = kNegD;
    }
    if (lane < LANES) w.state(dir, g + 1)[lg] = val;
  }
}

template <bool MOD, int LANES>
__global__ __launch_bounds__(64) void band_seg_final_kernel(const int32_t* __restrict__ boundary, float* __restrict__ ws, int T, int S) {
  extern __shared__ __attribute__((aligned(16))) float2 seg[];
  const int sg = blockIdx.x, dir = blockIdx.y, b = blockIdx.z;
  const SegUtt u = seg_utt<MOD>(boundary, b, S, T);
  if (u.degenerate) return;
  const SegGeom gm = seg_geom(u.D);
  if (sg >= gm.K) return;
  const SegWs<LANES> w(ws + (size_t)b * seg_floats_per_utt<LANES>(T, S), T, S);
  const int lane = threadIdx.x, l16 = lane & 15, lg = l16 & (LANES - 1);
  double* pbuf = reinterpret_cast<double*>(seg + (size_t)(gm.L + 2 * kSegU) * LANES);
  seg_stage<LANES>(seg, dir ? w.OB : w.OA, kRow0 + sg * gm.L, gm.L, lane, 64);
  double val = w.state(dir, sg)[lg];
  __syncthreads();
  seg_chain<LANES, true>(seg, gm.L, lg, val, pbuf, lane < LANES);
  __syncthreads();
  double* P = (dir ? w.QB : w.PA) + (size_t)(kRow0 + sg * gm.L) * LANES;
  for (int i = lane; i < gm.L * LANES; i += 64) P[i] = pbuf[i];
}

template <bool MOD, int LANES>
__global__ __launch_bounds__(256) void band_seg_occupancy_kernel(const int32_t* __restrict__ ranges, const int32_t* __restrict__ boundary,
                                                                 const float* __restrict__ ws, float* __restrict__ ans,
                                                                 float* __restrict__ gxb, float* __restrict__ gyb, int T, int S, int r) {
  const int b = blockIdx.y;
  const int i = blockIdx.x * 256 + threadIdx.x;
  const size_t cells = (size_t)T * r;
  const SegUtt u = seg_utt<MOD>(boundary, b, S, T);
  float* gx_g = gxb + (size_t)b * cells;
  float* gy_g = gyb + (size_t)b * cells;
  if (u.degenerate) {
    if ((size_t)i < cells) { gx_g[i] = 0.0f; gy_g[i] = 0.0f; }
    if (i == 0) ans[b] = (u.Sn <= 0 || u.Tn <= 0) ? 0.0f : ((u.Sn == 1) ? 0.0f : -INFINITY);
    return;
  }
  const SegWs<LANES> w(const_cast<float*>(ws) + (size_t)b * seg_floats_per_utt<LANES>(T, S), T, S);
  const SegBand<MOD, LANES> g(ranges, b, T, r, u.bd);
  const int flags = *w.flags();
  const int fl = flags & (kSegFlagBad | kSegFlagNaN);
  const int sb = u.bd.sb, tb = u.bd.tb, se = u.bd.se, te = u.bd.te;
  const double pend = w.PA[g.slotA(se, te)];
  const double ans2 = pend;
  const bool dead = (flags & (kSegFlagNoOrigin | kSegFlagNoEnd)) != 0 || !(pend > kNegThreshD);
  if (i == 0) ans[b] = fl ? __builtin_nanf("") : (dead ? -INFINITY : (float)((ans2 + *w.shift_back()) * 0.6931471805599453));
  if ((size_t)i >= cells) return;
  const int t = i / r, k = i - t * r;
  float fx = 0.0f, fy = 0.0f;
  if (!fl && !dead && t >= tb && t < te) {
    const int l0 = g.lo(t);
    const int s = l0 + k;
    if (s >= sb && s <= se) {
      const double pa = w.PA[g.slotA(s, t)];
      if (pa > kNegThreshD) {
        const float2 ob = w.OB[g.slotB(s, t)];
        if (ob.x > kNegThresh) {
          const double qv = w.QB[g.slotB(s + 1, MOD ? t + 1 : t)];
          if (qv > kNegThreshD) fx = exp2f((float)((pa + (double)ob.x + qv) - ans2));
        }
        if (ob.y > kNegThresh) {
          const double qv = w.QB[g.slotB(s, t + 1)];
          if (qv > kNegThreshD) fy = exp2f((float)((pa + (double)ob.y + qv) - ans2));
        }
      }
    }
  }
  gx_g[i] = fx;
  gy_g[i] = fy;
}

inline int seg_lanes(int r) { return r <= 7 ? 8 : (r <= 15 ? 16 : 0); }
constexpr int kSegFrom = 1100;
inline size_t seg_lds_bytes(int T, int S, int lanes, bool store) {
  const size_t L = (size_t)seg_lmax(T, S);
  return sizeof(float2) * (L + 2 * kSegU) * lanes + (store ? sizeof(double) * (L * lanes) : 0) + 64;
}

}

int mi_band_seg_supported(int T, int S, int r) {
  bool forced = false;
  if (const char* e = getenv("FTR_BAND_IMPL")) { if (!strcmp(e, "chain")) return 0; forced = !strcmp(e, "segments"); }
  const int lanes = seg_lanes(r);
  if (!lanes || T < 1 || S < 0 || r < 1) return 0;
  if (!forced && (long long)S + T < kSegFrom) return 0;
  if (seg_lds_bytes(T, S, lanes, true) > (size_t)150 * 1024) return 0;
  if ((uint64_t)(T + 1) * r >= (1ull << 31) || (uint64_t)seg_rows(T, S) * lanes >= (1ull << 31)) return 0;
  return 1;
}
size_t mi_band_seg_workspace_floats(int B, int T, int S, int r) {
  if (!mi_band_seg_supported(T, S, r)) return 0;
  return (size_t)B * (seg_lanes(r) == 8 ? seg_floats_per_utt<8>(T, S) : seg_floats_per_utt<16>(T, S));
}

int mi_band_seg(const float* pxb, const float* pyb, const int32_t* ranges, const int32_t* boundary, float* ws, size_t ws_floats,
                float* ans, float* gxb, float* gyb, int B, int T, int S, int r, int modified, hipStream_t st) {
  if (B == 0) return FTR_OK;
  const size_t need = mi_band_seg_workspace_floats(B, T, S, r);
  if (!need || !ws || ws_floats < need || (reinterpret_cast<uintptr_t>(ws) & 15) != 0) {
    set_error("mutual_information_band (segments): workspace of %zu floats (16-byte aligned) required, got %zu", need, ws_floats);
    return FTR_ERR_INVALID_ARG;
  }
  const int lanes = seg_lanes(r);
  const size_t lds_t = seg_lds_bytes(T, S, lanes, false), lds_f = seg_lds_bytes(T, S, lanes, true);
  const unsigned cells_blocks = (unsigned)(((size_t)(T + 1) * r + 255) / 256);
  const unsigned fill_blocks = (unsigned)((2 * seg_rows(T, S) * lanes + 255) / 256);
  const dim3 gseg(kSegMaxK, 2, B);
  constexpr size_t ceiling = 156 * 1024;
  const char* what = "mutual_information_band (segments)";
  const int rc = dispatch_among<8, 16>(lanes, [&](auto lv) {
    return dispatch(modified != 0, [&](auto mod) {
      constexpr bool MODV = decltype(mod)::value;
      constexpr int LV = decltype(lv)::value;
      constexpr auto transfer = band_seg_transfer_kernel<MODV, LV>;
      constexpr auto final_k = band_seg_final_kernel<MODV, LV>;
      int rcl = reserve_lds<transfer>(ceiling, what);
      if (rcl == FTR_OK) rcl = reserve_lds<final_k>(ceiling, what);
      if (rcl != FTR_OK) return rcl;
      hipLaunchKernelGGL((band_seg_init_kernel<MODV, LV>), dim3(fill_blocks, B), dim3(256), 0, st, pxb, pyb, ranges, boundary, ws, T, S, r);
      hipLaunchKernelGGL((band_seg_scatter_kernel<MODV, LV>), dim3(cells_blocks, B), dim3(256), 0, st, pxb, pyb, ranges, boundary, ws, T, S, r);
      hipLaunchKernelGGL(transfer, gseg, dim3(16 * LV), lds_t, st, boundary, ws, T, S);
      hipLaunchKernelGGL((band_seg_prefix_kernel<MODV, LV>), dim3(2, B), dim3(64), sizeof(double) * (kSegMaxK - 1) * LV * LV, st, boundary, ws, T, S);
      hipLaunchKernelGGL(final_k, gseg, dim3(64), lds_f, st, boundary, ws, T, S);
      hipLaunchKernelGGL((band_seg_occupancy_kernel<MODV, LV>), dim3((unsigned)(((size_t)T * r + 255) / 256), B), dim3(256), 0, st,
                         ranges, boundary, ws, ans, gxb, gyb, T, S, r);
      return FTR_OK;
    });
  });
  if (rc != FTR_OK) return rc;
  return check_launch("mi_band_seg");
}

}
```

### tf-fast-rnnt_amd/csrc/pruned_logprobs.hip

```cpp
#include "ftr_common.h"
#include "launch.h"

namespace ftr {
namespace {

__device__ __forceinline__ float wave_max(float v) { return wave_max_dpp(v); }
__device__ __forceinline__ float wave_sum(float v) { return wave_sum_dpp(v); }

template <typename E, int NQ, bool HAT>
__global__ __launch_bounds__(256) void lse_rows_reg_kernel(const E* __restrict__ logits, float* __restrict__ lse,
                                                           size_t rows, int C, int blank) {
  const int lane = threadIdx.x & 63;
  const size_t rowi = (size_t)blockIdx.x * (blockDim.x >> 6) + (threadIdx.x >> 6);
  if (rowi >= rows) return;
  const size_t row = rows - 1 - rowi;
  const int n4 = C >> 2;
  const f4 ninf = {-INFINITY, -INFINITY, -INFINITY, -INFINITY};
  const E* x = logits + row * C;
  f4 v[NQ];
#pragma unroll
  for (int q = 0; q < NQ; ++q) {
    const int i = lane + 64 * q;
    v[q] = (i < n4) ? load4(x, i) : ninf;
    if (HAT) {
#pragma unroll
      for (int e = 0; e < 4; ++e) v[q][e] = (4 * i + e == blank) ? -INFINITY : v[q][e];
    }
  }
  float m = -INFINITY;
#pragma unroll
  for (int q = 0; q < NQ; ++q) m = fmaxf(fmaxf(m, fmaxf(v[q][0], v[q][1])), fmaxf(v[q][2], v[q][3]));
  m = wave_max(m);
  float sum = 0.0f;
#pragma unroll
  for (int q = 0; q < NQ; ++q) {
    if (lane + 64 * q < n4)
      sum += __expf(v[q][0] - m) + __expf(v[q][1] - m) + __expf(v[q][2] - m) + __expf(v[q][3] - m);
  }
  sum = wave_sum(sum);
  if (lane == 0) lse[row] = m + __logf(sum);
}

template <typename E, bool VEC, bool HAT>
__global__ void lse_rows_kernel(const E* __restrict__ logits, float* __restrict__ lse, size_t rows, int C, int blank) {
  const int lane = threadIdx.x & 63;
  const size_t row = (size_t)blockIdx.x * (blockDim.x >> 6) + (threadIdx.x >> 6);
  if (row >= rows) return;
  const E* x = logits + row * C;
  float m = -INFINITY;
  if (VEC) {
    const int n4 = C >> 2;
    for (int i = lane; i < n4; i += 64) {
      f4 v = load4(x, i);
      if (HAT) {
#pragma unroll
        for (int e = 0; e < 4; ++e) v[e] = (4 * i + e == blank) ? -INFINITY : v[e];
      }
      m = fmaxf(fmaxf(m, fmaxf(v[0], v[1])), fmaxf(v[2], v[3]));
    }
    m = wave_max(m);
    float s = 0.0f;
    for (int i = lane; i < n4; i += 64) {
      f4 v = load4(x, i);
      if (HAT) {
#pragma unroll
        for (int e = 0; e < 4; ++e) v[e] = (4 * i + e == blank) ? -INFINITY : v[e];
      }
      s += __expf(v[0] - m) + __expf(v[1] - m) + __expf(v[2] - m) + __expf(v[3] - m);
    }
    s = wave_sum(s);
    if (lane == 0) lse[row] = m + __logf(s);
  } else {
    for (int i = lane; i < C; i += 64) m = fmaxf(m, (HAT && i == blank) ? -INFINITY : elem_to_float(x[i]));
    m = wave_max(m);
    float s = 0.0f;
    for (int i = lane; i < C; i += 64) s += __expf(((HAT && i == blank) ? -INFINITY : elem_to_float(x[i])) - m);
    s = wave_sum(s);
    if (lane == 0) lse[row] = m + __logf(s);
  }
}

template <typename E, bool MOD, bool HAT>
__global__ void band_to_lattice_kernel(const E* __restrict__ logits, const int32_t* __restrict__ symbols,
                                       const int32_t* __restrict__ ranges, const int32_t* __restrict__ boundary,
                                       const float* __restrict__ lse, int blank, double delay_penalty,
                                       float* __restrict__ px, float* __restrict__ py, int T, int S, int C, int r) {
  const int t = blockIdx.x * blockDim.x + threadIdx.x;
  const int s = blockIdx.y, b = blockIdx.z;
  const int T1 = MOD ? T : T + 1;
  if (t >= T1 && t >= T) return;
  const int te = boundary ? boundary[4 * b + 3] : T;
  float vx = -INFINITY, vy = -INFINITY;
  if (t < T) {
    const size_t bt = (size_t)b * T + t;
    const int s0 = ranges[bt * r];
    int k = s - s0;
    if (k < 0) k += S + 1;
    if (k < r) {
      const size_t row = bt * r + k;
      const float l = lse[row];
      if (HAT) {
        const float xb = elem_to_float(logits[row * C + blank]);
        int c = blank;
        if (s < S) c = min(max(symbols[(size_t)b * S + s], 0), C - 1);
        float hx, hy;
        hat_logprobs(xb, elem_to_float(logits[row * C + c]), l, c == blank, &hx, &hy);
        vy = hy;
        if (s < S) vx = hx;
      } else {
        vy = elem_to_float(logits[row * C + blank]) - l;
        if (s < S) vx = elem_to_float(logits[row * C + min(max(symbols[(size_t)b * S + s], 0), C - 1)]) - l;
      }
    }
  }
  if (t < T) py[((size_t)b * (S + 1) + s) * T + t] = vy;
  if (s < S && t < T1) {
    if (!MOD && t == te) vx = -INFINITY;
    if (delay_penalty > 0.0) {
      const double offset = ((double)te - 1.0) / 2.0;
      vx += (float)((offset - (double)t) * delay_penalty);
    }
    px[((size_t)b * S + s) * T1 + t] = vx;
  }
}

template <typename E, bool MOD, bool VEC, bool HAT>
__global__ void band_grad_kernel(const E* __restrict__ logits, const int32_t* __restrict__ symbols,
                                 const int32_t* __restrict__ ranges, const int32_t* __restrict__ boundary,
                                 const float* __restrict__ lse, const float* __restrict__ gpx,
                                 const float* __restrict__ gpy, const Scale scale, int blank,
                                 E* __restrict__ glogits, size_t rows, int T, int S, int C, int r) {
  const int lane = threadIdx.x & 63;
  const size_t row = (size_t)blockIdx.x * (blockDim.x >> 6) + (threadIdx.x >> 6);
  if (row >= rows) return;
  const int T1 = MOD ? T : T + 1;
  const size_t bt = row / r;
  const int k = (int)(row - bt * r);
  const int b = (int)(bt / T);
  const int t = (int)(bt - (size_t)b * T);
  const int s0 = ranges[bt * r];
  int s = s0 + k;
  if (s > S) s -= S + 1;
  const int te = boundary ? boundary[4 * b + 3] : T;
  const float sc = scale.at(b);
  float gx = 0.0f;
  int sym = blank;
  const bool sok = s >= 0 && s <= S;
  if (sok && s < S) {
    sym = symbols[(size_t)b * S + s];
    if (MOD || t != te) gx = gpx[((size_t)b * S + s) * T1 + t] * sc;
  }
  const float gy = sok ? gpy[((size_t)b * (S + 1) + s) * T + t] * sc : 0.0f;
  float tot = gx + gy;
  const float l = lse[row];
  if (HAT) {
    sym = min(max(sym, 0), C - 1);
    if (sym == blank) gx = 0.0f;
    tot = gx;
  }
  const E* x = logits + row * C;
  E* g = glogits + row * C;
  if (VEC) {
    const int n4 = C >> 2;
    for (int i = lane; i < n4; i += 64) {
      const f4 v = load4(x, i);
      f4 o;
#pragma unroll
      for (int e = 0; e < 4; ++e) {
        const int c = 4 * i + e;
        float val = -tot * __expf(v[e] - l);
        if (c == sym) val += gx;
        if (c == blank) {
          if (HAT) {
            float sp, sn;
            hat_sigmoids(v[e], &sp, &sn);
            val = gy * sn - gx * sp;
          } else {
            val += gy;
          }
        }
        o[e] = val;
      }
      store4(g, i, o);
    }
  } else {
    for (int c = lane; c < C; c += 64) {
      const float xc = elem_to_float(x[c]);
      float val = -tot * __expf(xc - l);
      if (c == sym) val += gx;
      if (c == blank) {
        if (HAT) {
          float sp, sn;
          hat_sigmoids(xc, &sp, &sn);
          val = gy * sn - gx * sp;
        } else {
          val += gy;
        }
      }
      g[c] = elem_from_float<E>(val);
    }
  }
}

__global__ __launch_bounds__(256) void negated_reduce_kernel(const float* __restrict__ ans, int B, int reduction,
                                                             float* __restrict__ out, float sign) {
  __shared__ float red[4];
  if (reduction == 0) {
    for (int b = threadIdx.x; b < B; b += 256) out[b] = sign * ans[b];
    return;
  }
  float s = 0.0f;
  for (int b = threadIdx.x; b < B; b += 256) s += ans[b];
  s = wave_sum(s);
  if ((threadIdx.x & 63) == 0) red[threadIdx.x >> 6] = s;
  __syncthreads();
  if (threadIdx.x == 0) {
    const float t = (red[0] + red[1]) + (red[2] + red[3]);
    out[0] = sign * ((reduction == 1) ? t / (float)B : t);
  }
}
}

int negated_reduce(const float* ans, int B, int reduction, float* out, hipStream_t st, float sign) {
  hipLaunchKernelGGL(negated_reduce_kernel, dim3(1), dim3(256), 0, st, ans, B, reduction, out, sign);
  return check_launch("negated_reduce");
}

namespace {
template <typename E>
int lse_rows_of(const E* logits, float* lse, size_t rows, int C, int blank, int hat, hipStream_t st) {
  if (rows == 0) return FTR_OK;
  { const int rc32 = require_rows_32bit("lse_rows", rows); if (rc32 != FTR_OK) return rc32; }
  const int wpb = 4;
  const unsigned blocks = (unsigned)((rows + wpb - 1) / wpb);
  dispatch(hat != 0, [&](auto h) {
    constexpr bool HAT = decltype(h)::value;
    const bool vec4 = rows_vec4<E>(C, logits);
    if (vec4 && C <= 2048)
      dispatch_among<1, 2, 4, 8>(C <= 256 ? 1 : C <= 512 ? 2 : C <= 1024 ? 4 : 8, [&](auto n) {
        hipLaunchKernelGGL((lse_rows_reg_kernel<E, decltype(n)::value, HAT>), dim3(blocks), dim3(64 * wpb), 0, st, logits, lse, rows, C, blank);
      });
    else
      dispatch(vec4, [&](auto vec) {
        hipLaunchKernelGGL((lse_rows_kernel<E, decltype(vec)::value, HAT>), dim3(blocks), dim3(64 * wpb), 0, st, logits, lse, rows, C, blank);
      });
  });
  return check_launch("lse_rows");
}
}

int lse_rows(const float* logits, float* lse, size_t rows, int C, int blank, int hat, hipStream_t st) {
  return lse_rows_of(logits, lse, rows, C, blank, hat, st);
}
int lse_rows_dtype(const void* logits, int dtype, float* lse, size_t rows, int C, int blank, int hat, hipStream_t st) {
  return dispatch_dtype(dtype, [&](auto tag) {
    using E = typename decltype(tag)::type;
    return lse_rows_of(static_cast<const E*>(logits), lse, rows, C, blank, hat, st);
  });
}

int pruned_logprobs_fwd(const void* logits, int dtype, const int32_t* symbols, const int32_t* ranges,
                        const int32_t* boundary, int blank, double delay_penalty, float* lse, float* px,
                        float* py, int B, int T, int S, int C, int r, int modified, int hat, hipStream_t st) {
  const size_t rows = (size_t)B * T * r;
  if (rows == 0) return FTR_OK;
  { const int rc32 = require_rows_32bit("pruned_logprobs_fwd", rows); if (rc32 != FTR_OK) return rc32; }
  int rc = lse_rows_dtype(logits, dtype, lse, rows, C, blank, hat, st);
  if (rc != FTR_OK) return rc;
  const int threads = 256;
  const dim3 grid((T + 1 + threads - 1) / threads, S + 1, B);
  dispatch_dtype(dtype, [&](auto tag) {
    using E = typename decltype(tag)::type;
    dispatch(modified != 0, [&](auto mod) {
      dispatch(hat != 0, [&](auto h) {
        hipLaunchKernelGGL((band_to_lattice_kernel<E, decltype(mod)::value, decltype(h)::value>), grid, dim3(threads), 0, st,
                           static_cast<const E*>(logits), symbols, ranges, boundary, lse, blank, delay_penalty, px, py, T, S, C, r);
      });
    });
  });
  return check_launch("band_to_lattice");
}

int pruned_logprobs_bwd(const void* logits, int dtype, const int32_t* symbols, const int32_t* ranges,
                        const int32_t* boundary, int blank, const float* lse, const float* gpx,
                        const float* gpy, Scale scale, void* glogits, int B, int T, int S, int C,
                        int r, int modified, int hat, hipStream_t st) {
  const size_t rows = (size_t)B * T * r;
  if (rows == 0) return FTR_OK;
  { const int rc32 = require_rows_32bit("pruned_logprobs_bwd", rows); if (rc32 != FTR_OK) return rc32; }
  const int wpb = 4;
  const unsigned blocks = (unsigned)((rows + wpb - 1) / wpb);
  dispatch_dtype(dtype, [&](auto tag) {
    using E = typename decltype(tag)::type;
    dispatch(modified != 0, [&](auto mod) {
      dispatch(rows_vec4<E>(C, logits, glogits), [&](auto vec) {
        dispatch(hat != 0, [&](auto h) {
          hipLaunchKernelGGL((band_grad_kernel<E, decltype(mod)::value, decltype(vec)::value, decltype(h)::value>), dim3(blocks), dim3(64 * wpb), 0, st,
                             static_cast<const E*>(logits), symbols, ranges, boundary, lse, gpx, gpy, scale, blank, static_cast<E*>(glogits), rows, T, S, C, r);
        });
      });
    });
  });
  return check_launch("band_grad");
}

namespace {

struct MbCols { int id[8]; int d[8]; int D; };

__device__ __forceinline__ bool mb_is_big_blank(const MbCols& mc, int c) {
  bool hit = false;
  for (int j = 1; j < mc.D; ++j) hit |= (c == mc.id[j]);
  return hit;
}

__global__ void mb_to_lattice_kernel(const float* __restrict__ logits, const int32_t* __restrict__ symbols,
                                     const int32_t* __restrict__ ranges, const int32_t* __restrict__ boundary,
                                     const float* __restrict__ lse, const MbCols mc, float sigma, double delay_penalty,
                                     float* __restrict__ px, float* __restrict__ py, int T, int S, int C, int r) {
  const int t = blockIdx.x * blockDim.x + threadIdx.x;
  const int s = blockIdx.y, b = blockIdx.z;
  if (t > T) return;
  const int te = boundary ? boundary[4 * b + 3] : T;
  float vx = -INFINITY;
  bool inband = false;
  size_t row = 0;
  float l = 0.0f;
  if (t < T) {
    const size_t bt = (size_t)b * T + t;
    const int s0 = ranges[bt * r];
    int k = s - s0;
    if (k < 0) k += S + 1;
    if (k < r) {
      inband = true;
      row = bt * r + k;
      l = lse[row] + sigma;
      if (s < S) {
        const int c = min(max(symbols[(size_t)b * S + s], 0), C - 1);
        if (!mb_is_big_blank(mc, c)) vx = logits[row * C + c] - l;
      }
    }
    for (int j = 0; j < mc.D; ++j) {
      float vy = -INFINITY;
      if (inband && t + mc.d[j] <= te) vy = logits[row * C + mc.id[j]] - l;
      py[(((size_t)b * mc.D + j) * (S + 1) + s) * T + t] = vy;
    }
  }
  if (s < S) {
    if (t == te) vx = -INFINITY;
    if (delay_penalty > 0.0) {
      const double offset = ((double)te - 1.0) / 2.0;
      vx += (float)((offset - (double)t) * delay_penalty);
    }
    px[((size_t)b * S + s) * (T + 1) + t] = vx;
  }
}

template <bool VEC>
__global__ void mb_grad_kernel(const float* __restrict__ logits, const int32_t* __restrict__ symbols,
                               const int32_t* __restrict__ ranges, const int32_t* __restrict__ boundary,
                               const float* __restrict__ lse, const float* __restrict__ gpx,
                               const float* __restrict__ gpy, const Scale scale, const MbCols mc,
                               float* __restrict__ glogits, size_t rows, int T, int S, int C, int r) {
  const int lane = threadIdx.x & 63;
  const size_t row = (size_t)blockIdx.x * (blockDim.x >> 6) + (threadIdx.x >> 6);
  if (row >= rows) return;
  const int T1 = T + 1;
  const size_t bt = row / r;
  const int k = (int)(row - bt * r);
  const int b = (int)(bt / T);
  const int t = (int)(bt - (size_t)b * T);
  const int s0 = ranges[bt * r];
  int s = s0 + k;
  if (s > S) s -= S + 1;
  const int te = boundary ? boundary[4 * b + 3] : T;
  const float sc = scale.at(b);
  float gx = 0.0f;
  int sym = -1;
  const bool sok = s >= 0 && s <= S;
  if (sok && s < S) {
    sym = min(max(symbols[(size_t)b * S + s], 0), C - 1);
    if (t != te && !mb_is_big_blank(mc, sym)) gx = gpx[((size_t)b * S + s) * T1 + t] * sc;
  }
  float gy[8];
  float tot = gx;
#pragma unroll
  for (int j = 0; j < 8; ++j) {
    gy[j] = 0.0f;
    if (j < mc.D && sok && t + mc.d[j] <= te) gy[j] = gpy[(((size_t)b * mc.D + j) * (S + 1) + s) * T + t] * sc;
    tot += gy[j];
  }
  const float l = lse[row];
  const float* x = logits + row * C;
  float* g = glogits + row * C;
  if (VEC) {
    const f4u* x4 = reinterpret_cast<const f4u*>(x);
    f4u* g4 = reinterpret_cast<f4u*>(g);
    const int n4 = C >> 2;
    for (int i = lane; i < n4; i += 64) {
      const f4 v = x4[i];
      f4 o;
// ... 72 lines not shown
```

### tf-fast-rnnt_amd/tf_fast_rnnt/_lib.py

```python
from __future__ import annotations

import ctypes
import os

_HERE = os.path.dirname(os.path.abspath(__file__))
LIB_PATH = os.environ.get("FTR_LIB_PATH") or os.path.join(_HERE, "libftr_hip.so")
_lib = None

_c_fp = ctypes.c_void_p
_c_ip = ctypes.c_void_p
_c_st = ctypes.c_void_p
_c_hi = ctypes.POINTER(ctypes.c_int32)
_i = ctypes.c_int
_f = ctypes.c_float

_SIGNATURES = {
    "ftr_abi_version": (ctypes.c_int, []),
    "ftr_package_version": (ctypes.c_char_p, []),
    "ftr_last_error": (ctypes.c_char_p, []),
    "ftr_mutual_information_workspace_floats": (ctypes.c_size_t, [_i, _i, _i]),
    "ftr_mutual_information_handoff_floats": (ctypes.c_size_t, [_i, _i, _i]),
    "ftr_mutual_information_fwd_f32": (_i, [_c_fp, _c_fp, _c_ip, _c_fp, _c_fp, _i, _i, _i, _i, _c_st]),
    "ftr_mutual_information_bwd_f32": (_i, [_c_fp, _c_fp, _c_ip, _c_fp, _c_fp, _c_fp, _c_fp, _c_fp, _i, _i, _i, _i, _i, _c_st]),
    "ftr_mutual_information_fwd_ws_f32": (_i, [_c_fp, _c_fp, _c_ip, _c_fp, ctypes.c_size_t, _i, _c_fp, _i, _i, _i, _i, _c_st]),
    "ftr_mutual_information_bwd_ws_f32": (_i, [_c_fp, _c_fp, _c_ip, _c_fp, ctypes.c_size_t, _i, _c_fp, _c_fp, _c_fp, _c_fp, _i, _i, _i, _i, _i, _c_st]),
    "ftr_mutual_information_bwd_loss_ws_f32": (_i, [_c_fp, _c_fp, _c_ip, _c_fp, ctypes.c_size_t, _i, _c_fp, _c_fp, _c_fp, _i, _c_fp, _i, _i, _i, _i, _c_st]),
    "ftr_mutual_information_workspace_init": (_i, [_c_fp, ctypes.c_size_t, _i, _i, _i, _c_st]),
    "ftr_mutual_information_status": (_i, [_c_fp, ctypes.c_size_t, _i, _i, _i, ctypes.POINTER(ctypes.c_int), ctypes.POINTER(ctypes.c_longlong), _c_st]),
    "ftr_mutual_information_viterbi_workspace_bytes": (ctypes.c_size_t, [_i, _i, _i]),
    "ftr_mutual_information_viterbi_f32": (_i, [_c_fp, _c_fp, _c_ip, ctypes.c_void_p, ctypes.c_size_t, _c_fp, _c_ip, _i, _i, _i, _i, _c_st]),
    "ftr_cummin_i32": (_i, [_c_ip, _c_ip, _i, _i, _c_st]),
    "ftr_prune_ranges_i32": (_i, [_c_fp, _c_fp, _c_ip, _c_ip, _c_ip, _i, _i, _i, _i, _i, ctypes.POINTER(ctypes.c_int), _c_st]),
    "ftr_do_pruning_f32": (_i, [_c_fp, _c_fp, _c_ip, _c_fp, _c_fp, _i, _i, _i, _i, _i, _c_st]),
    "ftr_do_pruning_bwd_f32": (_i, [_c_fp, _c_fp, _c_ip, _c_fp, _c_fp, _i, _i, _i, _i, _i, _c_st]),
    "ftr_do_pruning_bwd_workspace_bytes": (ctypes.c_size_t, [_i, _i, _i, _i, _i]),
    "ftr_do_pruning_bwd_ws_f32": (_i, [_c_fp, _c_fp, _c_ip, _c_fp, _c_fp, _i, _i, _i, _i, _i, ctypes.c_void_p, ctypes.c_size_t, _c_st]),
    "ftr_pruned_logprobs_fwd_f32": (_i, [_c_fp, _c_ip, _c_ip, _c_ip, _i, ctypes.c_double, _c_fp, _c_fp, _c_fp, _i, _i, _i, _i, _i, _i, _c_st]),
    "ftr_pruned_logprobs_bwd_f32": (_i, [_c_fp, _c_ip, _c_ip, _c_ip, _i, _c_fp, _c_fp, _c_fp, _c_fp, _c_fp, _i, _i, _i, _i, _i, _i, _c_st]),
    "ftr_negated_reduce_f32": (_i, [_c_fp, _i, _i, _c_fp, _c_st]),
    "ftr_pruned_logprobs_bwd_scaled_f32": (_i, [_c_fp, _c_ip, _c_ip, _c_ip, _i, _c_fp, _c_fp, _c_fp, _c_fp, _i, _f, _c_fp, _i, _i, _i, _i, _i, _i, _c_st]),
    "ftr_simple_logprobs_bwd_w_scaled_f32": (_i, [_c_fp, _c_fp, _c_fp, _i, _f, _c_fp, _c_ip, _c_fp, _c_fp, _c_fp, _i, _i, _i, _i, _c_st]),
    "ftr_simple_logprobs_bwd_am_scaled_f32": (_i, [_c_fp, _c_fp, _c_fp, _i, _f, _c_fp, _c_fp, _c_ip, _c_ip, _i, _c_fp, _i, _i, _i, _i, _i, _c_st]),
    "ftr_rowmax_exp_f32": (_i, [_c_fp, _c_fp, _c_fp, ctypes.c_longlong, _i, _c_st]),
    "ftr_rowmax_exp_pair_f32": (_i, [_c_fp, _c_fp, _c_fp, ctypes.c_longlong, _c_fp, _c_fp, _c_fp, ctypes.c_longlong, _i, _c_st]),
    "ftr_rowmax_exp_sum_f32": (_i, [_c_fp, _c_fp, _c_fp, _c_fp, ctypes.c_longlong, _i, _c_st]),
    "ftr_smoothed_logprobs_fwd_f32": (_i, [_c_fp, _c_fp, _c_ip, _c_fp, _c_fp, _c_fp, _c_fp, _c_fp, _c_fp, _c_ip, _i, _f, _f, _f, _c_fp, _c_fp, _i, _i, _i, _i, _i, _c_st]),
    "ftr_smoothed_logprobs_bwd_w_f32": (_i, [_c_fp, _c_fp, _c_fp, _c_ip, _f, _c_fp, _c_fp, _c_fp, _i, _i, _i, _i, _c_st]),
    "ftr_smoothed_logprobs_bwd_am_f32": (_i, [_c_fp, _c_fp, _c_fp, _c_fp, _c_ip, _c_ip, _i, _f, _c_fp, _c_fp, _f, _c_fp, _c_fp, _i, _i, _i, _i, _i, _c_st]),
    "ftr_smoothed_logprobs_bwd_lm_f32": (_i, [_c_fp, _c_fp, _c_ip, _c_fp, _c_fp, _i, _f, _c_fp, _c_fp, _c_fp, _c_fp, _i, _i, _i, _c_st]),
    "ftr_smoothed_logprobs_fwd_pen_f32": (_i, [_c_fp, _c_fp, _c_ip, _c_fp, _c_fp, _c_fp, _c_fp, _c_fp, _c_fp, _c_ip, _i, ctypes.c_double, _f, _f, _f, _c_fp, _c_fp, _i, _i, _i, _i, _i, _c_st]),
    "ftr_smoothed_logprobs_bwd_w_scaled_f32": (_i, [_c_fp, _c_fp, _c_fp, _i, _f, _c_fp, _c_ip, _f, _c_fp, _c_fp, _c_fp, _i, _i, _i, _i, _c_st]),
    "ftr_smoothed_logprobs_bwd_am_scaled_f32": (_i, [_c_fp, _c_fp, _c_fp, _i, _f, _c_fp, _c_fp, _c_ip, _c_ip, _i, _f, _c_fp, _c_fp, _f, _c_fp, _c_fp, _i, _i, _i, _i, _i, _c_st]),
    "ftr_rowmax_exp_dot_f32": (_i, [_c_fp, _c_fp, _c_fp, _c_fp, _c_fp, ctypes.c_longlong, _i, _c_st]),
    "ftr_rowdot_f32": (_i, [_c_fp, _c_fp, _c_fp, ctypes.c_longlong, _i, _c_st]),
    "ftr_colsum_weighted_workspace_floats": (ctypes.c_size_t, [ctypes.c_longlong, _i]),
    "ftr_colsum_weighted_f32": (_i, [_c_fp, _c_fp, _c_fp, _c_fp, ctypes.c_size_t, ctypes.c_longlong, _i, _c_st]),
    "ftr_simple_logprobs_fused_supported": (_i, [_i]),
    "ftr_simple_logprobs_fused_bwd_supported": (_i, [_i, _i]),
    "ftr_normalizer_gemm_f32": (_i, [_i, _c_fp, _c_fp, _c_fp, _i, _i, _i, _i, _c_st]),
    "ftr_normalizer_gemm_set_choice": (_i, [_i, _i, _i, _i, _i, _i]),
    "ftr_normalizer_gemm_choice": (_i, [_i, _i, _i, _i, _i, ctypes.POINTER(ctypes.c_int), ctypes.POINTER(ctypes.c_float), ctypes.POINTER(ctypes.c_float), ctypes.POINTER(ctypes.c_int)]),
    "ftr_simple_logprobs_fused_fwd_f32": (_i, [_c_fp, _c_fp, _c_ip, _c_fp, _c_fp, _c_fp, _c_fp, _c_ip, _i, ctypes.c_double, _c_fp, _c_fp, _c_fp, _i, _i, _i, _i, _i, _c_st]),
    "ftr_smoothed_logprobs_fused_fwd_f32": (_i, [_c_fp, _c_fp, _c_ip, _c_fp, _c_fp, _c_fp, _c_fp, _c_fp, _c_fp, _c_fp, _c_ip, _i, ctypes.c_double, _f, _f, _f, _c_fp, _c_fp, _c_fp, _i, _i, _i, _i, _i, _c_st]),
    "ftr_simple_logprobs_fused_bwd_am_f32": (_i, [_c_fp, _c_fp, _c_fp, _i, _f, _c_fp, _c_fp, _c_fp, _c_ip, _c_ip, _i, _c_fp, _i, _i, _i, _i, _i, _c_st]),
    "ftr_smoothed_logprobs_fused_bwd_am_f32": (_i, [_c_fp, _c_fp, _c_fp, _i, _f, _c_fp, _c_fp, _c_fp, _c_ip, _c_ip, _i, _f, _f, _c_fp, _c_fp, _f, _c_fp, _c_fp, _i, _i, _i, _i, _i, _c_st]),
    "ftr_mutual_information_band_supported": (_i, [_i, _i, _i]),
    "ftr_band_ranges_check_i32": (_i, [_c_ip, _c_ip, _c_ip, _i, _i, _i, _c_st]),
    "ftr_pruned_band_fwd_f32": (_i, [_c_fp, _c_ip, _c_ip, _c_ip, _i, ctypes.c_double, _c_fp, _c_fp, _c_fp, _i, _i, _i, _i, _i, _i, _c_st]),
    "ftr_mutual_information_band_f32": (_i, [_c_fp, _c_fp, _c_ip, _c_ip, _c_fp, _c_fp, _c_fp, _i, _i, _i, _i, _i, _c_st]),
    "ftr_mutual_information_band_workspace_floats": (ctypes.c_size_t, [_i, _i, _i, _i]),
    "ftr_mutual_information_band_ws_f32": (_i, [_c_fp, _c_fp, _c_ip, _c_ip, _c_fp, ctypes.c_size_t, _c_fp, _c_fp, _c_fp, _i, _i, _i, _i, _i, _c_st]),
    "ftr_pruned_band_bwd_scaled_f32": (_i, [_c_fp, _c_ip, _c_ip, _c_ip, _i, _c_fp, _c_fp, _c_fp, _c_fp, _i, _f, _c_fp, _i, _i, _i, _i, _i, _i, _c_st]),
    "ftr_hat_pruned_logprobs_fwd_f32": (_i, [_c_fp, _c_ip, _c_ip, _c_ip, _i, ctypes.c_double, _c_fp, _c_fp, _c_fp, _i, _i, _i, _i, _i, _i, _c_st]),
    "ftr_hat_pruned_logprobs_bwd_scaled_f32": (_i, [_c_fp, _c_ip, _c_ip, _c_ip, _i, _c_fp, _c_fp, _c_fp, _c_fp, _i, _f, _c_fp, _i, _i, _i, _i, _i, _i, _c_st]),
    "ftr_hat_pruned_band_fwd_f32": (_i, [_c_fp, _c_ip, _c_ip, _c_ip, _i, ctypes.c_double, _c_fp, _c_fp, _c_fp, _i, _i, _i, _i, _i, _i, _c_st]),
    "ftr_hat_pruned_band_bwd_scaled_f32": (_i, [_c_fp, _c_ip, _c_ip, _c_ip, _i, _c_fp, _c_fp, _c_fp, _c_fp, _i, _f, _c_fp, _i, _i, _i, _i, _i, _i, _c_st]),
    "ftr_mutual_information_multiblank_workspace_floats": (ctypes.c_size_t, [_i, _i, _i]),
    "ftr_mutual_information_multiblank_fwd_f32": (_i, [_c_fp, _c_fp, _c_ip, _c_hi, _i, _c_fp, ctypes.c_size_t, _c_fp, _i, _i, _i, _c_st]),
    "ftr_mutual_information_multiblank_bwd_f32": (_i, [_c_fp, _c_fp, _c_ip, _c_hi, _i, _c_fp, ctypes.c_size_t, _c_fp, _c_fp, _c_fp, _i, _i, _i, _c_st]),
    "ftr_multiblank_pruned_logprobs_fwd_f32": (_i, [_c_fp, _c_ip, _c_ip, _c_ip, _i, _c_hi, _c_hi, _i, ctypes.c_double, ctypes.c_double, _c_fp, _c_fp, _c_fp, _i, _i, _i, _i, _i, _c_st]),
    "ftr_multiblank_pruned_logprobs_bwd_scaled_f32": (_i, [_c_fp, _c_ip, _c_ip, _c_ip, _i, _c_hi, _c_hi, _i, _c_fp, _c_fp, _c_fp, _c_fp, _i, _f, _c_fp, _i, _i, _i, _i, _i, _c_st]),
    "ftr_mutual_information_tdt_workspace_floats": (ctypes.c_size_t, [_i, _i, _i]),
    "ftr_mutual_information_tdt_fwd_f32": (_i, [_c_fp, _c_fp, _c_ip, _c_hi, _i, _c_hi, _i, _c_fp, ctypes.c_size_t, _c_fp, _i, _i, _i, _c_st]),
    "ftr_mutual_information_tdt_bwd_f32": (_i, [_c_fp, _c_fp, _c_ip, _c_hi, _i, _c_hi, _i, _c_fp, ctypes.c_size_t, _c_fp, _c_fp, _c_fp, _i, _i, _i, _c_st]),
    "ftr_mutual_information_viterbi_tdt_workspace_bytes": (ctypes.c_size_t, [_i, _i, _i]),
    "ftr_mutual_information_viterbi_tdt_f32": (_i, [_c_fp, _c_fp, _c_ip, _c_hi, _i, _c_hi, _i, ctypes.c_void_p, ctypes.c_size_t, _c_fp, _c_ip, _c_ip, _c_ip, _i, _i, _i, _c_st]),
    "ftr_tdt_pruned_logprobs_fwd_f32": (_i, [_c_fp, _c_ip, _c_ip, _c_ip, _i, _c_hi, _i, ctypes.c_double, ctypes.c_double, _c_fp, _c_fp, _c_fp, _c_fp, _i, _i, _i, _i, _i, _c_st]),
    "ftr_tdt_pruned_logprobs_bwd_scaled_f32": (_i, [_c_fp, _c_ip, _c_ip, _c_ip, _i, _c_hi, _i, ctypes.c_double, ctypes.c_double, _c_fp, _c_fp, _c_fp, _c_fp, _c_fp, _i, _f, _c_fp, _i, _i, _i, _i, _i, _c_st]),
    "ftr_simple_logprobs_fwd_f32": (_i, [_c_fp, _c_fp, _c_ip, _c_fp, _c_fp, _c_fp, _c_ip, _i, ctypes.c_double, _c_fp, _c_fp, _i, _i, _i, _i, _i, _c_st]),
    "ftr_simple_logprobs_bwd_w_f32": (_i, [_c_fp, _c_fp, _c_fp, _c_ip, _c_fp, _c_fp, _c_fp, _i, _i, _i, _i, _c_st]),
    "ftr_simple_logprobs_bwd_am_f32": (_i, [_c_fp, _c_fp, _c_fp, _c_fp, _c_ip, _c_ip, _i, _c_fp, _i, _i, _i, _i, _i, _c_st]),
    "ftr_simple_logprobs_bwd_lm_f32": (_i, [_c_fp, _c_fp, _c_ip, _c_fp, _c_fp, _i, _c_fp, _i, _i, _i, _c_st]),
    "ftr_selftest": (_i, [ctypes.c_void_p, _c_st]),
}
_LOWP_SIGNATURES = {
    "ftr_pruned_logprobs_fwd_dt": (_i, [_c_fp, _i, _c_ip, _c_ip, _c_ip, _i, ctypes.c_double, _c_fp, _c_fp, _c_fp, _i, _i, _i, _i, _i, _i, _i, _c_st]),
    "ftr_pruned_logprobs_bwd_scaled_dt": (_i, [_c_fp, _i, _c_ip, _c_ip, _c_ip, _i, _c_fp, _c_fp, _c_fp, _c_fp, _i, _f, _c_fp, _i, _i, _i, _i, _i, _i, _i, _c_st]),
    "ftr_pruned_band_fwd_dt": (_i, [_c_fp, _i, _c_ip, _c_ip, _c_ip, _i, ctypes.c_double, _c_fp, _c_fp, _c_fp, _i, _i, _i, _i, _i, _i, _i, _c_st]),
    "ftr_pruned_band_bwd_scaled_dt": (_i, [_c_fp, _i, _c_ip, _c_ip, _c_ip, _i, _c_fp, _c_fp, _c_fp, _c_fp, _i, _f, _c_fp, _i, _i, _i, _i, _i, _i, _i, _c_st]),
}
_KD_SIGNATURES = {
    "ftr_pruned_kd_fwd_dt": (_i, [_c_fp, _i, _c_fp, _i, _c_ip, _c_ip, _c_ip, _i, _f, _i, _c_fp, _c_fp, _c_fp, _i, _i, _i, _i, _i, _c_st]),
    "ftr_pruned_kd_bwd_scaled_dt": (_i, [_c_fp, _i, _c_fp, _i, _c_ip, _c_ip, _c_ip, _i, _f, _i, _c_fp, _c_fp, _i, _f, _c_fp, _i, _i, _i, _i, _i, _c_st]),
    "ftr_pruned_kd_reduce_f32": (_i, [_c_fp, _i, _i, _c_fp, _c_st]),
}
_FUSED_SIGNATURES = {
    "ftr_simple_logprobs_fused_bwd_am_w_f32": (_i, [_c_fp, _c_fp, _c_fp, _i, _f, _c_fp, _c_fp, _c_fp, _c_ip, _c_ip, _i, _c_fp, _i, _i, _i, _i, _i, _c_st]),
    "ftr_smoothed_logprobs_fused_bwd_am_w_f32": (_i, [_c_fp, _c_fp, _c_fp, _i, _f, _c_fp, _c_fp, _c_fp, _c_ip, _c_ip, _i, _f, _c_fp, _c_fp, _f, _c_fp, _c_fp, _i, _i, _i, _i, _i, _c_st]),
    "ftr_simple_logprobs_fused_bwd_am_w_columns": (_i, [_i, _i, _i]),
}
EXPORTED_SYMBOLS = tuple(_SIGNATURES)
LOWP_SYMBOLS = tuple(_LOWP_SIGNATURES)
KD_SYMBOLS = tuple(_KD_SIGNATURES)
FUSED_SYMBOLS = tuple(_FUSED_SIGNATURES)
FTR_KD_FULL, FTR_KD_COLLAPSED = 0, 1
FTR_MI_WS_CLEAN = 1
FTR_DTYPE_F32, FTR_DTYPE_BF16, FTR_DTYPE_FP16 = 0, 1, 2
FTR_PRUNED_HAT = 1


def lib() -> ctypes.CDLL:
    global _lib
    if _lib is None:
        if not os.path.exists(LIB_PATH):
            raise ImportError(
                f"{LIB_PATH} is missing: build the HIP extension first (python -c 'import __graft_entry__ as g; "
                "g.build()' or make -C tf-fast-rnnt_amd/csrc).  tf_fast_rnnt has no CPU fallback.")
        handle = ctypes.CDLL(LIB_PATH)
        for name, (restype, argtypes) in {**_SIGNATURES, **_LOWP_SIGNATURES, **_KD_SIGNATURES, **_FUSED_SIGNATURES}.items():
            fn = getattr(handle, name)
            fn.restype = restype
            fn.argtypes = argtypes
        _lib = handle
    return _lib


class FtrError(RuntimeError):
    """A native entry point returned an FTR_ERR_* code (the reference raises tf.errors.Internal,
    tf_fast_rnnt_op.cc:114-116)."""


def check(rc: int, what: str) -> None:
    if rc != 1:
        msg = lib().ftr_last_error().decode("utf-8", "replace")
        raise FtrError(f"{what} failed with code {rc}: {msg}")


_profile_hook = None


def set_profile_hook(hook) -> None:
    global _profile_hook
    _profile_hook = hook


def call(name: str, *args) -> None:
    fn = getattr(lib(), name)
    if _profile_hook is None:
        rc = fn(*args)
    else:
        with _profile_hook(name):
            rc = fn(*args)
    check(rc, name)
```

### tf-fast-rnnt_amd/tf_fast_rnnt/rnnt_loss.py

```python
from __future__ import annotations

from typing import Optional, Tuple, Union

import ctypes
import os

import torch

from . import _lib
from .mutual_information import (_as_boundary, _ptr, _require_gpu, _stream_ptr, cummin,
                                 mb_forward_backward, mi_forward_backward, mutual_information_recursion,
                                 mutual_information_viterbi, mutual_information_viterbi_tdt, tdt_forward_backward)

_NEG_INF = float("-inf")
_TINY = 1.401298464324817e-45


def tune_normalizer_gemms(enable: bool = True, filename: Optional[str] = None, search: bool = True, when: str = "second") -> None:
    if when not in ("first", "second"):
        raise ValueError("when must be 'first' or 'second'")
    os.environ["FTR_GEMM_TUNE"] = when if (enable and search) else "off"


def normalizer_gemm_choice(kind: int, B: int, T: int, S: int, C: int):
# ... 451 lines not shown
    lse = torch.empty((B, T, r), dtype=torch.float32, device=x.device)
    px = torch.empty((B, S, T if modified else T + 1), dtype=torch.float32, device=x.device)
    py = torch.empty((B, S + 1, T), dtype=torch.float32, device=x.device)
    with torch.cuda.device(x.device):
        _pruned_call("pruned_logprobs_fwd", hat, x, (_ptr(symbols), _ptr(ranges), _ptr(boundary), int(blank),
                     float(delay_penalty), _ptr(lse), _ptr(px), _ptr(py), B, T, S, C, r, int(modified)), (_stream_ptr(x),))
    return lse, px, py


def _pruned_builder_bwd(x, symbols, ranges, boundary, blank, modified, lse, gpx, gpy, scale, stride, mul, band, hat):
    B, T, r, C = x.shape
    S = symbols.shape[1]
    g = torch.empty_like(x)
    with torch.cuda.device(x.device):
        _pruned_call("pruned_band_bwd_scaled" if band else "pruned_logprobs_bwd_scaled", hat, x,
                     (_ptr(symbols), _ptr(ranges), _ptr(boundary), blank, _ptr(lse), _ptr(gpx), _ptr(gpy), _ptr(scale), stride,
                      mul, _ptr(g), B, T, S, C, r, modified), (_stream_ptr(x),))
    return g


class _PrunedLogprobs(torch.autograd.Function):

    @staticmethod
    def forward(ctx, logits, symbols, ranges, termination_symbol, boundary, modified, delay_penalty, hat):
        x = logits.detach().contiguous()
        lse, px, py = _pruned_builder_fwd(x, symbols, ranges, boundary, termination_symbol, delay_penalty, modified, hat)
        ctx.save_for_backward(x, symbols, ranges, lse, boundary)
        ctx.meta = (int(termination_symbol), int(modified), bool(hat))
        return px, py

    @staticmethod
    def backward(ctx, gpx, gpy):
        x, symbols, ranges, lse, boundary = ctx.saved_tensors
        blank, modified, hat = ctx.meta
        g = _pruned_builder_bwd(x, symbols, ranges, boundary, blank, modified, lse, gpx.contiguous(), gpy.contiguous(),
                                None, 0, 1.0, False, hat)
        return g, None, None, None, None, None, None, None


def _pruned_inputs(logits, symbols, ranges, boundary, lowp=False):
    _require_gpu(logits, "logits")
    if logits.dim() != 4:
        raise ValueError("logits must be [B,T,s_range,C]")
    if lowp and logits.dtype in _LOWP_KIND:
        pass
    elif logits.dtype != torch.float32:
        raise TypeError("logits must be float32, bfloat16 or float16" if lowp else "logits must be float32")
    B, T, r, C = logits.shape
    symbols = torch.as_tensor(symbols, device=logits.device).to(torch.int32).contiguous()
    ranges_in = ranges
    ranges = torch.as_tensor(ranges, device=logits.device).to(torch.int32).contiguous()
    if ranges is not ranges_in and isinstance(ranges_in, torch.Tensor) and _band_mark_valid(ranges_in):
        _mark_band(ranges)
    if tuple(ranges.shape) != (B, T, r):
        raise ValueError(f"ranges must have shape {(B, T, r)}, got {tuple(ranges.shape)}")
    if symbols.dim() != 2 or symbols.shape[0] != B:
        raise ValueError("symbols must be [B,S]")
    boundary = _as_boundary(boundary, B, logits.device)
    return symbols, ranges, boundary


def get_rnnt_logprobs_pruned(
    logits: torch.Tensor,
    symbols: torch.Tensor,
    ranges: torch.Tensor,
    termination_symbol: int,
    boundary: torch.Tensor,
    rnnt_type: str = "regular",
) -> Tuple[torch.Tensor, torch.Tensor]:
    return _pruned_logprobs(logits, symbols, ranges, termination_symbol, boundary, rnnt_type, False)


def _pruned_logprobs(logits, symbols, ranges, termination_symbol, boundary, rnnt_type, hat):
    _check_type(rnnt_type)
    symbols, ranges, boundary = _pruned_inputs(logits, symbols, ranges, boundary, lowp=True)
    modified = rnnt_type != "regular"
    px, py = _PrunedLogprobs.apply(logits, symbols, ranges, termination_symbol, boundary, modified, 0.0, hat)
    if rnnt_type == "constrained":
        px = px + py[:, 1:, :]
    return px, py


def get_hat_logprobs_pruned(
    logits: torch.Tensor,
    symbols: torch.Tensor,
    ranges: torch.Tensor,
    termination_symbol: int,
    boundary: torch.Tensor,
    rnnt_type: str = "regular",
) -> Tuple[torch.Tensor, torch.Tensor]:
    return _pruned_logprobs(logits, symbols, ranges, termination_symbol, boundary, rnnt_type, True)


def rnnt_alignment_pruned(
    logits: torch.Tensor,
    symbols: torch.Tensor,
    ranges: torch.Tensor,
    termination_symbol: int,
    boundary: Optional[torch.Tensor] = None,
    rnnt_type: str = "regular",
) -> Tuple[torch.Tensor, torch.Tensor]:
    _check_type(rnnt_type)
    with torch.no_grad():
        symbols, ranges, boundary = _pruned_inputs(logits, symbols, ranges, boundary, lowp=True)
        _, px, py = _pruned_builder_fwd(logits.detach().contiguous(), symbols, ranges, boundary, termination_symbol, 0.0,
                                        rnnt_type != "regular", False)
        if rnnt_type == "constrained":
            px += py[:, 1:, :]
        return mutual_information_viterbi(px, py, boundary)


def _mark_band(ranges: torch.Tensor) -> None:
    ranges._ftr_band = ranges._version


def _band_mark_valid(ranges: torch.Tensor) -> bool:
    return getattr(ranges, "_ftr_band", None) == ranges._version


def _is_band(ranges: torch.Tensor, boundary) -> bool:
    if _band_mark_valid(ranges):
        return True
    if getattr(ranges, "_ftr_not_band", None) == ranges._version:
        return False
    if torch.cuda.is_current_stream_capturing():
        return False
    B, T, r = ranges.shape
    flags = torch.empty((1,), dtype=torch.int32, device=ranges.device)
    with torch.cuda.device(ranges.device):
        _lib.call("ftr_band_ranges_check_i32", _ptr(ranges), _ptr(boundary), _ptr(flags), B, T, r, _stream_ptr(ranges))
    ok = int(flags.item()) == 0
    if ok:
        _mark_band(ranges)
    else:
        ranges._ftr_not_band = ranges._version
    return ok


def _band_path_ok(ranges, boundary, T: int, S: int, r: int) -> bool:
    if os.environ.get("FTR_PRUNED_ROUTE") == "lattice":
        return False
    return _lib.lib().ftr_mutual_information_band_supported(int(T), int(S), int(r)) != 0 and _is_band(ranges, boundary)


class _PrunedLoss(torch.autograd.Function):

    @staticmethod
    def forward(ctx, logits, symbols, ranges, termination_symbol, boundary, modified, delay_penalty, code, hat):
        B, T, r, C = logits.shape
        S = symbols.shape[1]
        x = logits.detach().contiguous()
        need = logits.requires_grad
        ctx.band = _band_path_ok(ranges, boundary, T, S, r)
        if ctx.band:
            lse = torch.empty((B, T, r), dtype=torch.float32, device=x.device)
            pxb = torch.empty((B, T, r), dtype=torch.float32, device=x.device)
            pyb = torch.empty((B, T, r), dtype=torch.float32, device=x.device)
            gxb = torch.empty((B, T, r), dtype=torch.float32, device=x.device)
            gyb = torch.empty((B, T, r), dtype=torch.float32, device=x.device)
            ans = torch.empty((B,), dtype=torch.float32, device=x.device)
            with torch.cuda.device(x.device):
                st = _stream_ptr(x)
                _pruned_call("pruned_band_fwd", hat, x, (_ptr(symbols), _ptr(ranges), _ptr(boundary),
                             int(termination_symbol), float(delay_penalty), _ptr(lse), _ptr(pxb), _ptr(pyb),
                             B, T, S, C, r, int(modified)), (st,))
                nws = _lib.lib().ftr_mutual_information_band_workspace_floats(B, T, S, r)
                bws = torch.empty((nws,), dtype=torch.float32, device=x.device) if nws else None
                _lib.call("ftr_mutual_information_band_ws_f32", _ptr(pxb), _ptr(pyb), _ptr(ranges), _ptr(boundary), _ptr(bws),
                          nws, _ptr(ans), _ptr(gxb), _ptr(gyb), B, T, S, r, int(modified), st)
                del bws
            del pxb, pyb
            if need:
                ctx.save_for_backward(x, symbols, ranges, lse, gxb, gyb, boundary)
        else:
            lse, px, py = _pruned_builder_fwd(x, symbols, ranges, boundary, termination_symbol, delay_penalty, modified, hat)
            ans, px_grad, py_grad = mi_forward_backward(px, py, boundary, need, ans_grad_is_one=True)
            del px, py
            if need:
                ctx.save_for_backward(x, symbols, ranges, lse, px_grad, py_grad, boundary)
        ctx.meta = (int(termination_symbol), int(modified), int(code), bool(hat))
        return _negated_reduce_native(ans, code)

    @staticmethod
    def backward(ctx, g_loss):
        x, symbols, ranges, lse, px_grad, py_grad, boundary = ctx.saved_tensors
        blank, modified, code, hat = ctx.meta
        scale, stride, mul = _upstream_scale(g_loss, code, x.shape[0])
        g = _pruned_builder_bwd(x, symbols, ranges, boundary, blank, modified, lse, px_grad, py_grad, scale, stride, mul,
                                ctx.band, hat)
        return g, None, None, None, None, None, None, None, None


def rnnt_loss_pruned(
    logits: torch.Tensor,
    symbols: torch.Tensor,
    ranges: torch.Tensor,
    termination_symbol: int,
    boundary: torch.Tensor = None,
    rnnt_type: str = "regular",
    delay_penalty: float = 0.0,
    reduction: Optional[str] = "mean",
    calc_gradients: bool = False,
) -> torch.Tensor:
    return _pruned_loss(logits, symbols, ranges, termination_symbol, boundary, rnnt_type, delay_penalty, reduction, False)


def _pruned_loss(logits, symbols, ranges, termination_symbol, boundary, rnnt_type, delay_penalty, reduction, hat):
    _check_type(rnnt_type)
    code = _reduction_code(reduction)
    symbols_i, ranges_i, boundary_i = _pruned_inputs(logits, symbols, ranges, boundary, lowp=True)
    if rnnt_type == "constrained":
        px, py = _pruned_logprobs(logits, symbols_i, ranges_i, termination_symbol, boundary_i, rnnt_type, hat)
        px = _apply_delay_penalty(px, boundary_i, rnnt_type, delay_penalty)
        negated_loss = mutual_information_recursion(px=px, py=py, boundary=boundary_i, calc_gradients=False)
        return _reduce(negated_loss, reduction)
    return _PrunedLoss.apply(logits, symbols_i, ranges_i, termination_symbol, boundary_i, rnnt_type != "regular",
                             _penalty(delay_penalty), code, hat)


def hat_loss_pruned(
    logits: torch.Tensor,
    symbols: torch.Tensor,
    ranges: torch.Tensor,
    termination_symbol: int,
    boundary: torch.Tensor = None,
    rnnt_type: str = "regular",
    delay_penalty: float = 0.0,
    reduction: Optional[str] = "mean",
) -> torch.Tensor:
    return _pruned_loss(logits, symbols, ranges, termination_symbol, boundary, rnnt_type, delay_penalty, reduction, True)


def hat_loss(
    logits: torch.Tensor,
    symbols: torch.Tensor,
    termination_symbol: int,
    boundary: Optional[torch.Tensor] = None,
    rnnt_type: str = "regular",
    delay_penalty: float = 0.0,
    reduction: Optional[str] = "mean",
) -> torch.Tensor:
    _check_type(rnnt_type)
    boundary = _as_boundary(boundary, logits.shape[0], logits.device)
    return hat_loss_pruned(logits=logits, symbols=symbols, ranges=_joint_inputs(logits, symbols),
                           termination_symbol=termination_symbol, boundary=boundary, rnnt_type=rnnt_type,
                           delay_penalty=delay_penalty, reduction=reduction)



_KD_MODES = {"full": _lib.FTR_KD_FULL, "collapsed": _lib.FTR_KD_COLLAPSED}
_KD_DTYPES = (torch.float32, torch.bfloat16, torch.float16)


def _kd_head(x, y):
    return (_ptr(x), _LOWP_KIND.get(x.dtype, _lib.FTR_DTYPE_F32), _ptr(y), _LOWP_KIND.get(y.dtype, _lib.FTR_DTYPE_F32))


class _PrunedKdLoss(torch.autograd.Function):

    @staticmethod
    def forward(ctx, logits, teacher_logits, symbols, ranges, termination_symbol, boundary, mode, temperature, code):
        B, T, r, C = logits.shape
        S = symbols.shape[1]
        x = logits.detach().contiguous()
        y = teacher_logits.detach().contiguous()
        node = torch.empty((B, T, r), dtype=torch.float32, device=x.device)
        saved = torch.empty((4 if mode == _lib.FTR_KD_COLLAPSED else 2, B, T, r), dtype=torch.float32, device=x.device)
        utt = torch.empty((B,), dtype=torch.float32, device=x.device)
        out = utt
        with torch.cuda.device(x.device):
            st = _stream_ptr(x)
            _lib.call("ftr_pruned_kd_fwd_dt", *_kd_head(x, y), _ptr(symbols), _ptr(ranges), _ptr(boundary),
                      int(termination_symbol), float(temperature), mode, _ptr(node), _ptr(saved), _ptr(utt), B, T, S, C, r, st)
            if code != 0:
                out = torch.empty((), dtype=torch.float32, device=x.device)
                _lib.call("ftr_pruned_kd_reduce_f32", _ptr(utt), B, code, _ptr(out), st)
        if logits.requires_grad:
            ctx.save_for_backward(x, y, symbols, ranges, saved, boundary)
        ctx.meta = (int(termination_symbol), mode, float(temperature), int(code))
        return out

    @staticmethod
    def backward(ctx, g_loss):
        x, y, symbols, ranges, saved, boundary = ctx.saved_tensors
        blank, mode, temperature, code = ctx.meta
        B, T, r, C = x.shape
        scale, stride, mul = _upstream_scale(g_loss, code, B)
        g = torch.empty_like(x)
        with torch.cuda.device(x.device):
            _lib.call("ftr_pruned_kd_bwd_scaled_dt", *_kd_head(x, y), _ptr(symbols), _ptr(ranges), _ptr(boundary), blank,
                      temperature, mode, _ptr(saved), _ptr(scale), stride, -mul, _ptr(g), B, T, symbols.shape[1], C, r,
                      _stream_ptr(x))
        return g, None, None, None, None, None, None, None, None


def rnnt_kd_loss_pruned(
    logits: torch.Tensor,
    teacher_logits: torch.Tensor,
    symbols: torch.Tensor,
    ranges: torch.Tensor,
    termination_symbol: int,
    boundary: Optional[torch.Tensor] = None,
    mode: str = "full",
    temperature: float = 1.0,
    reduction: Optional[str] = "mean",
) -> torch.Tensor:
    for name, t in (("logits", logits), ("teacher_logits", teacher_logits)):
        if t.dtype not in _KD_DTYPES:
            raise TypeError(f"{name} must be float32, bfloat16 or float16, got {t.dtype}")
    if logits.dim() != 4:
        raise ValueError("logits must be [B,T,s_range,C]")
    if tuple(teacher_logits.shape) != tuple(logits.shape):
        raise ValueError(f"teacher_logits must have the shape of logits {tuple(logits.shape)}, got {tuple(teacher_logits.shape)}")
    if mode not in _KD_MODES:
        raise ValueError(f"mode should be ('full' | 'collapsed'), given {mode}")
    temperature = float(temperature)
    if not (0.0 < temperature < float("inf")):
        raise ValueError(f"temperature must be a finite number > 0, given {temperature}")
    code = _reduction_code(reduction)
    if not 0 <= int(termination_symbol) < logits.shape[3]:
        raise ValueError(f"termination_symbol {termination_symbol} not in [0,{logits.shape[3]})")
    symbols, ranges, boundary = _pruned_inputs(logits, symbols, ranges, boundary, lowp=True)
    _require_gpu(teacher_logits, "teacher_logits")
    if teacher_logits.device != logits.device:
        raise ValueError("teacher_logits and logits must be on the same device")
    return _PrunedKdLoss.apply(logits, teacher_logits, symbols, ranges, int(termination_symbol), boundary, _KD_MODES[mode],
                               temperature, code)



def _big_blank_args(big_blanks, termination_symbol: int, C: int):
    pairs = [(int(i), int(d)) for i, d in big_blanks]
    ids = [i for i, _ in pairs]
# ... 556 lines not shown
```

Measured before the change: 24380 utterances/s.

## Fuse band gather into LSE kernel and fold fill/reduce into band loss path

Moves the px/py band gather into the row log-sum-exp kernel so logits rows are read once and the separate gather launch goes away. The seg MI kernel's workspace fill and the final negated loss reduction are folded into existing launches, and a new single C entry point replaces several Python-side allocations and calls. The goal is fewer kernel launches, fewer allocations and less host overhead per step, at the cost of more template variants and a more complex kernel interface.

```diff
diff --git a/include/ftr_band_loss.h b/include/ftr_band_loss.h
--- /dev/null
+++ b/include/ftr_band_loss.h
@@ -0,0 +1,27 @@
+#ifndef FTR_BAND_LOSS_H_
+#define FTR_BAND_LOSS_H_
+#include "ftr_lowp.h"
+
+#ifdef __cplusplus
+extern "C" {
+#endif
+
+size_t ftr_pruned_band_loss_workspace_floats(int B, int T, int S, int r);
+int ftr_pruned_band_loss_fwd_f32(const float* logits, const int32_t* symbols, const int32_t* ranges, const int32_t* boundary,
+                                 int termination_symbol, double delay_penalty, int reduction, float* workspace,
+                                 size_t workspace_floats, float* lse, float* gx_band, float* gy_band, float* ans, float* loss,
+                                 int B, int T, int S, int C, int r, int modified, void* stream);
+int ftr_hat_pruned_band_loss_fwd_f32(const float* logits, const int32_t* symbols, const int32_t* ranges,
+                                     const int32_t* boundary, int termination_symbol, double delay_penalty, int reduction,
+                                     float* workspace, size_t workspace_floats, float* lse, float* gx_band, float* gy_band,
+                                     float* ans, float* loss, int B, int T, int S, int C, int r, int modified, void* stream);
+int ftr_pruned_band_loss_fwd_dt(const void* logits, int kind, const int32_t* symbols, const int32_t* ranges,
+                                const int32_t* boundary, int termination_symbol, double delay_penalty, int reduction,
+                                float* workspace, size_t workspace_floats, float* lse, float* gx_band, float* gy_band,
+                                float* ans, float* loss, int B, int T, int S, int C, int r, int modified, int flags,
+                                void* stream);
+
+#ifdef __cplusplus
+}
+#endif
+#endif
diff --git a/tf-fast-rnnt_amd/csrc/capi.hip b/tf-fast-rnnt_amd/csrc/capi.hip
--- a/tf-fast-rnnt_amd/csrc/capi.hip
+++ b/tf-fast-rnnt_amd/csrc/capi.hip
@@ -723,8 +723,8 @@
   FTR_TRY(check_builder(what, B >= 0 && T >= 1 && S >= 0 && C >= 1 && r >= 1, termination_symbol, C, false, hat));
   if (B == 0) return FTR_OK;
   FTR_TRY(pointers_then_device(what, logits && ranges && lse && px_band && py_band && (symbols || S == 0)));
-  FTR_TRY(lse_rows_dtype(logits, dtype, lse, (size_t)B * T * r, C, termination_symbol, hat, stream_of(stream)));
-  return band_gather(logits, dtype, symbols, ranges, boundary, lse, termination_symbol, delay_penalty, px_band, py_band, B, T, S, C, r, modified, hat, stream_of(stream));
+  return pruned_band_fwd(logits, dtype, symbols, ranges, boundary, termination_symbol, delay_penalty, lse, px_band, py_band, B, T, S, C, r, modified, hat,
+                         BandFill{nullptr, 0, 0, nullptr, 0, 0}, stream_of(stream));
 }
 
 int ftr_pruned_band_fwd_f32(const float* logits, const int32_t* symbols, const int32_t* ranges, const int32_t* boundary,
@@ -746,6 +746,55 @@
   clear_error();
   FTR_TRY(check_dtype("pruned_band_fwd_dt", kind, flags));
   return pruned_band_fwd_entry(logits, kind, symbols, ranges, boundary, termination_symbol, delay_penalty, lse, px_band, py_band, B, T, S, C, r, modified, flags & FTR_PRUNED_HAT, stream);
+}
+
+size_t ftr_pruned_band_loss_workspace_floats(int B, int T, int S, int r) {
+  return (B < 0 || T < 1 || S < 0 || r < 1) ? 0 : pruned_band_loss_workspace_floats(B, T, S, r);
+}
+
+static int pruned_band_loss_fwd_entry(const char* what, const void* logits, int dtype, const int32_t* symbols, const int32_t* ranges,
+                                      const int32_t* boundary, int termination_symbol, double delay_penalty, int reduction,
+                                      float* workspace, size_t workspace_floats, float* lse, float* gx_band, float* gy_band,
+                                      float* ans, float* loss, int B, int T, int S, int C, int r, int modified, int hat, void* stream) {
+  FTR_TRY(check_builder(what, B >= 0 && T >= 1 && S >= 0 && C >= 1 && r >= 1, termination_symbol, C, false, hat));
+  FTR_REQUIRE(reduction >= 0 && reduction <= 2, "%s: reduction %d is not 0 (none), 1 (mean) or 2 (sum)", what, reduction);
+  if (B == 0) {
+    if (reduction == 0) return FTR_OK;
+    FTR_TRY(pointers_then_device(what, loss != nullptr));
+    return negated_reduce(ans, 0, reduction, loss, stream_of(stream));
+  }
+  FTR_TRY(pointers_then_device(what, logits && ranges && workspace && lse && gx_band && gy_band && ans && loss && (symbols || S == 0)));
+  return pruned_band_loss_fwd(logits, dtype, symbols, ranges, boundary, termination_symbol, delay_penalty, reduction, workspace, workspace_floats,
+                              lse, gx_band, gy_band, ans, loss, B, T, S, C, r, modified, hat, stream_of(stream));
+}
+
+int ftr_pruned_band_loss_fwd_f32(const float* logits, const int32_t* symbols, const int32_t* ranges, const int32_t* boundary,
+                                 int termination_symbol, double delay_penalty, int reduction, float* workspace,
+                                 size_t workspace_floats, float* lse, float* gx_band, float* gy_band, float* ans, float* loss,
+                                 int B, int T, int S, int C, int r, int modified, void* stream) {
+  clear_error();
+  return pruned_band_loss_fwd_entry("pruned_band_loss_fwd", logits, FTR_DTYPE_F32, symbols, ranges, boundary, termination_symbol, delay_penalty, reduction,
+                                    workspace, workspace_floats, lse, gx_band, gy_band, ans, loss, B, T, S, C, r, modified, 0, stream);
+}
+
+int ftr_hat_pruned_band_loss_fwd_f32(const float* logits, const int32_t* symbols, const int32_t* ranges,
+                                     const int32_t* boundary, int termination_symbol, double delay_penalty, int reduction,
+                                     float* workspace, size_t workspace_floats, float* lse, float* gx_band, float* gy_band,
+                                     float* ans, float* loss, int B, int T, int S, int C, int r, int modified, void* stream) {
+  clear_error();
+  return pruned_band_loss_fwd_entry("hat_pruned_band_loss_fwd", logits, FTR_DTYPE_F32, symbols, ranges, boundary, termination_symbol, delay_penalty, reduction,
+                                    workspace, workspace_floats, lse, gx_band, gy_band, ans, loss, B, T, S, C, r, modified, 1, stream);
+}
+
+int ftr_pruned_band_loss_fwd_dt(const void* logits, int kind, const int32_t* symbols, const int32_t* ranges,
+                                const int32_t* boundary, int termination_symbol, double delay_penalty, int reduction,
+                                float* workspace, size_t workspace_floats, float* lse, float* gx_band, float* gy_band,
+                                float* ans, float* loss, int B, int T, int S, int C, int r, int modified, int flags,
+                                void* stream) {
+  clear_error();
+  FTR_TRY(check_dtype("pruned_band_loss_fwd_dt", kind, flags));
+  return pruned_band_loss_fwd_entry("pruned_band_loss_fwd_dt", logits, kind, symbols, ranges, boundary, termination_symbol, delay_penalty, reduction,
+                                    workspace, workspace_floats, lse, gx_band, gy_band, ans, loss, B, T, S, C, r, modified, flags & FTR_PRUNED_HAT, stream);
 }
 
 int ftr_band_ranges_check_i32(const int32_t* ranges, const int32_t* boundary, int32_t* flags, int B, int T, int r, void* stream) {
diff --git a/tf-fast-rnnt_amd/csrc/ftr_common.h b/tf-fast-rnnt_amd/csrc/ftr_common.h
--- a/tf-fast-rnnt_amd/csrc/ftr_common.h
+++ b/tf-fast-rnnt_amd/csrc/ftr_common.h
@@ -5,6 +5,7 @@
 #include <stdarg.h>
 #include "../../include/ftr_kd.h"
 #include "../../include/ftr_fused.h"
+#include "../../include/ftr_band_loss.h"
 
 namespace ftr {
 
@@ -130,6 +131,33 @@
 __device__ __forceinline__ double shift_total(const Shift s, int Sn, int Tn) {
   const int nx = Sn - 1, ny = MOD ? (Tn - 1) - (Sn - 1) : (Tn - 1);
   return (double)nx * (double)s.cx2 + (double)ny * (double)s.cy2;
+}
+
+template <typename F>
+__device__ __forceinline__ void negated_reduce_block(F ans_of, int B, int reduction, float* __restrict__ out, float sign, float* red) {
+  if (reduction == 0) {
+    for (int b = threadIdx.x; b < B; b += 256) out[b] = sign * ans_of(b);
+    return;
+  }
+  float s = 0.0f;
+  for (int b = threadIdx.x; b < B; b += 256) s += ans_of(b);
+  s = wave_sum_dpp(s);
+  if ((threadIdx.x & 63) == 0) red[threadIdx.x >> 6] = s;
+  __syncthreads();
+  if (threadIdx.x == 0) {
+    const float t = (red[0] + red[1]) + (red[2] + red[3]);
+    out[0] = sign * ((reduction == 1) ? t / (float)B : t);
+  }
+}
+
+struct BandFill { float2* base; size_t utt_stride; size_t n; int32_t* flag0; size_t flag_stride; int B; };
+__device__ __forceinline__ void band_fill(const BandFill& f, size_t gid, size_t gsize) {
+  const size_t total = f.n * (size_t)f.B;
+  for (size_t i = gid; i < total; i += gsize) {
+    const size_t b = total <= 0xffffffffull ? (size_t)((unsigned)i / (unsigned)f.n) : i / f.n, k = i - b * f.n;
+    f.base[b * f.utt_stride + k] = make_float2(kNeg, 0.0f);
+    if (k == 0) f.flag0[b * f.flag_stride] = 0;
+  }
 }
 
 struct Bound { int sb, tb, se, te; };
@@ -211,11 +239,14 @@
 int lse_rows_dtype(const void* logits, int dtype, float* lse, size_t rows, int C, int blank, int hat, hipStream_t st);
 int mi_band_supported(int T, int S, int r);
 int band_ranges_check(const int32_t* ranges, const int32_t* boundary, int* flags, int B, int T, int r, hipStream_t st);
-int band_gather(const void* logits, int dtype, const int32_t* symbols, const int32_t* ranges, const int32_t* boundary, const float* lse, int blank, double delay_penalty, float* pxb, float* pyb, int B, int T, int S, int C, int r, int modified, int hat, hipStream_t st);
+int pruned_band_fwd(const void* logits, int dtype, const int32_t* symbols, const int32_t* ranges, const int32_t* boundary, int blank, double delay_penalty, float* lse, float* pxb, float* pyb, int B, int T, int S, int C, int r, int modified, int hat, const BandFill& fill, hipStream_t st);
 size_t mi_band_workspace_floats(int B, int T, int S, int r);
 int mi_band_seg_supported(int T, int S, int r);
 size_t mi_band_seg_workspace_floats(int B, int T, int S, int r);
-int mi_band_seg(const float* pxb, const float* pyb, const int32_t* ranges, const int32_t* boundary, float* ws, size_t ws_floats, float* ans, float* gxb, float* gyb, int B, int T, int S, int r, int modified, hipStream_t st);
+BandFill mi_band_seg_fill(float* ws, int B, int T, int S, int r);
+int mi_band_seg(const float* pxb, const float* pyb, const int32_t* ranges, const int32_t* boundary, float* ws, size_t ws_floats, float* ans, float* gxb, float* gyb, int B, int T, int S, int r, int modified, hipStream_t st, bool filled = false, float* loss_out = nullptr, int reduction = 0);
+size_t pruned_band_loss_workspace_floats(int B, int T, int S, int r);
+int pruned_band_loss_fwd(const void* logits, int dtype, const int32_t* symbols, const int32_t* ranges, const int32_t* boundary, int blank, double delay_penalty, int reduction, float* ws, size_t ws_floats, float* lse, float* gxb, float* gyb, float* ans, float* loss, int B, int T, int S, int C, int r, int modified, int hat, hipStream_t st);
 int mi_band(const float* pxb, const float* pyb, const int32_t* ranges, const int32_t* boundary, float* ws, size_t ws_floats, float* ans, float* gxb, float* gyb, int B, int T, int S, int r, int modified, hipStream_t st);
 int band_grad_banded(const void* logits, int dtype, const int32_t* symbols, const int32_t* ranges, const int32_t* boundary, int blank, const float* lse, const float* gxb, const float* gyb, Scale scale, void* glogits, int B, int T, int S, int C, int r, int modified, int hat, hipStream_t st);
 int selftest(hipStream_t st, int* result_dev);
diff --git a/tf-fast-rnnt_amd/csrc/mi_band.hip b/tf-fast-rnnt_amd/csrc/mi_band.hip
--- a/tf-fast-rnnt_amd/csrc/mi_band.hip
+++ b/tf-fast-rnnt_amd/csrc/mi_band.hip
@@ -23,40 +23,6 @@
 __device__ __forceinline__ float row16_sum(float v) {
   v += dpp_row_ror<8>(v); v += dpp_row_ror<4>(v); v += dpp_row_ror<2>(v); v += dpp_row_ror<1>(v);
   return v;
-}
-
-template <typename E, bool MOD, bool HAT>
-__global__ void band_gather_kernel(const E* __restrict__ logits, const int32_t* __restrict__ symbols,
-                                   const int32_t* __restrict__ ranges, const int32_t* __restrict__ boundary,
-                                   const float* __restrict__ lse, int blank, double delay_penalty,
-                                   float* __restrict__ pxb, float* __restrict__ pyb, size_t rows, int T, int S, int C, int r) {
-  const size_t row = (size_t)blockIdx.x * blockDim.x + threadIdx.x;
-  if (row >= rows) return;
-  const size_t bt = row / r;
-  const int k = (int)(row - bt * r);
-  const int b = (int)(bt / T);
-  const int t = (int)(bt - (size_t)b * T);
-  const int s = ranges[bt * r] + k;
-  const int te = boundary ? boundary[4 * b + 3] : T;
-  const float l = lse[row];
-  float vy = -INFINITY, vx = -INFINITY;
-  if (s >= 0 && s <= S) {
-    if (HAT) {
-      const float xb = elem_to_float(logits[row * C + blank]);
-      int c = blank;
-      if (s < S) c = min(max(symbols[(size_t)b * S + s], 0), C - 1);
-      hat_logprobs(xb, elem_to_float(logits[row * C + c]), l, c == blank, &vx, &vy);
-    } else {
-      vy = elem_to_float(logits[row * C + blank]) - l;
-    }
-    if (s < S) {
-      if (!HAT) vx = elem_to_float(logits[row * C + min(max(symbols[(size_t)b * S + s], 0), C - 1)]) - l;
-      if (!MOD && t == te) vx = -INFINITY;
-      if (delay_penalty > 0.0) vx += (float)((((double)te - 1.0) / 2.0 - (double)t) * delay_penalty);
-    }
-  }
-  pxb[row] = vx;
-  pyb[row] = vy;
 }
 
 __global__ void band_ranges_check_kernel(const int32_t* __restrict__ ranges, const int32_t* __restrict__ boundary,
@@ -715,25 +681,6 @@
   return check_launch("band_ranges_check");
 }
 
-int band_gather(const void* logits, int dtype, const int32_t* symbols, const int32_t* ranges, const int32_t* boundary,
-                const float* lse, int blank, double delay_penalty, float* pxb, float* pyb, int B, int T, int S, int C,
-                int r, int modified, int hat, hipStream_t st) {
-  const size_t rows = (size_t)B * T * r;
-  if (rows == 0) return FTR_OK;
-  { const int rc32 = require_rows_32bit("pruned_band_fwd", rows); if (rc32 != FTR_OK) return rc32; }
-  const unsigned blocks = (unsigned)((rows + 255) / 256);
-  dispatch_dtype(dtype, [&](auto tag) {
-    using E = typename decltype(tag)::type;
-    dispatch(modified != 0, [&](auto mod) {
-      dispatch(hat != 0, [&](auto h) {
-        hipLaunchKernelGGL((band_gather_kernel<E, decltype(mod)::value, decltype(h)::value>), dim3(blocks), dim3(256), 0, st,
-                           static_cast<const E*>(logits), symbols, ranges, boundary, lse, blank, delay_penalty, pxb, pyb, rows, T, S, C, r);
-      });
-    });
-  });
-  return check_launch("band_gather");
-}
-
 constexpr size_t kBandLdsCeiling = 156 * 1024;
 
 int mi_band(const float* pxb, const float* pyb, const int32_t* ranges, const int32_t* boundary, float* ws, size_t ws_floats,
@@ -771,6 +718,33 @@
       return check_launch("mi_band");
     });
   });
+}
+
+static size_t band_loss_arrays_floats(int B, int T, int r) { return ((size_t)2 * B * T * r + 3) & ~(size_t)3; }
+size_t pruned_band_loss_workspace_floats(int B, int T, int S, int r) {
+  return band_loss_arrays_floats(B, T, r) + mi_band_workspace_floats(B, T, S, r);
+}
+int pruned_band_loss_fwd(const void* logits, int dtype, const int32_t* symbols, const int32_t* ranges, const int32_t* boundary,
+                         int blank, double delay_penalty, int reduction, float* ws, size_t ws_floats, float* lse, float* gxb,
+                         float* gyb, float* ans, float* loss, int B, int T, int S, int C, int r, int modified, int hat, hipStream_t st) {
+  if (!mi_band_supported(T, S, r)) { set_error("pruned_band_loss_fwd: T=%d S=%d r=%d is outside the band kernels' domain (r <= 15)", T, S, r); return FTR_ERR_UNSUPPORTED; }
+  const size_t need = pruned_band_loss_workspace_floats(B, T, S, r);
+  if (!ws || ws_floats < need || (reinterpret_cast<uintptr_t>(ws) & 15) != 0) {
+    set_error("pruned_band_loss_fwd: workspace of %zu floats (16-byte aligned) required, got %zu", need, ws_floats);
+    return FTR_ERR_INVALID_ARG;
+  }
+  float* pxb = ws;
+  float* pyb = ws + (size_t)B * T * r;
+  float* bws = ws + band_loss_arrays_floats(B, T, r);
+  const size_t bws_floats = ws_floats - band_loss_arrays_floats(B, T, r);
+  const bool seg = B <= 65535 && mi_band_seg_supported(T, S, r);
+  const BandFill fill = seg ? mi_band_seg_fill(bws, B, T, S, r) : BandFill{nullptr, 0, 0, nullptr, 0, 0};
+  int rc = pruned_band_fwd(logits, dtype, symbols, ranges, boundary, blank, delay_penalty, lse, pxb, pyb, B, T, S, C, r, modified, hat, fill, st);
+  if (rc != FTR_OK) return rc;
+  if (seg) return mi_band_seg(pxb, pyb, ranges, boundary, bws, bws_floats, ans, gxb, gyb, B, T, S, r, modified, st, true, loss, reduction);
+  rc = mi_band(pxb, pyb, ranges, boundary, bws, bws_floats, ans, gxb, gyb, B, T, S, r, modified, st);
+  if (rc != FTR_OK) return rc;
+  return negated_reduce(ans, B, reduction, loss, st);
 }
 
 #ifdef FTR_BAND_STAMPS
diff --git a/tf-fast-rnnt_amd/csrc/mi_band_seg.hip b/tf-fast-rnnt_amd/csrc/mi_band_seg.hip
--- a/tf-fast-rnnt_amd/csrc/mi_band_seg.hip
+++ b/tf-fast-rnnt_amd/csrc/mi_band_seg.hip
@@ -61,7 +61,7 @@
 template <int LANES>
 struct SegWs {
   float2* OA; float2* OB; double* PA; double* QB; double* M; double* ST; float* hdr;
-  __device__ SegWs(float* base, int T, int S) {
+  __host__ __device__ SegWs(float* base, int T, int S) {
     const size_t nr = seg_rows(T, S);
     OA = reinterpret_cast<float2*>(base); OB = OA + nr * LANES;
     PA = reinterpret_cast<double*>(base + 4 * nr * LANES); QB = PA + nr * LANES;
@@ -69,9 +69,10 @@
     hdr = reinterpret_cast<float*>(ST + 2 * (size_t)kSegMaxK * LANES);
   }
   __device__ int* flags() const { return reinterpret_cast<int*>(hdr); }
+  __device__ int* start_flags() const { return reinterpret_cast<int*>(hdr) + 3; }
+  __device__ int all_flags() const { return *flags() | *start_flags(); }
   __device__ double* shift_back() const { return reinterpret_cast<double*>(hdr + 4); }
   __device__ double* mat(int dir, int seg) const { return M + ((size_t)dir * kSegMaxK + seg) * (LANES * LANES); }
-  __device__ double* state(int dir, int seg) const { return ST + ((size_t)dir * kSegMaxK + seg) * LANES; }
 };
 constexpr int kRow0 = 1;
 
@@ -86,30 +87,12 @@
   return u;
 }
 
-template <bool MOD, int LANES>
-__global__ __launch_bounds__(256) void band_seg_init_kernel(const float* __restrict__ pxb, const float* __restrict__ pyb,
-                                                            const int32_t* __restrict__ ranges, const int32_t* __restrict__ boundary,
-                                                            float* __restrict__ ws, int T, int S, int r) {
-  const int b = blockIdx.y;
-  const SegWs<LANES> w(ws + (size_t)b * seg_floats_per_utt<LANES>(T, S), T, S);
-  const size_t n = 2 * seg_rows(T, S) * LANES;
-  for (size_t i = (size_t)blockIdx.x * 256 + threadIdx.x; i < n; i += (size_t)gridDim.x * 256) w.OA[i] = make_float2(kNeg, 0.0f);
-  if (blockIdx.x != 0) return;
-  __shared__ float red[16];
-  const SegUtt u = seg_utt<MOD>(boundary, b, S, T);
-  if (threadIdx.x == 0) {
-    int f = 0;
-    if (!u.degenerate) {
-      const int32_t* rg = ranges + (size_t)b * T * r;
-      const int lo_b = rg[(size_t)min(u.bd.tb, u.bd.te - 1) * r], lo_e = rg[(size_t)(u.bd.te - 1) * r];
-      if (!(u.bd.sb >= lo_b && u.bd.sb <= lo_b + r - 1)) f |= kSegFlagNoOrigin;
-      if (!((u.bd.se >= lo_e && u.bd.se <= lo_e + r - 1) || (MOD && u.bd.se == lo_e + r))) f |= kSegFlagNoEnd;
-    }
-    *w.flags() = f;
-  }
-  if (u.degenerate) return;
-  const float* pxu = pxb + (size_t)b * T * r;
-  const float* pyu = pyb + (size_t)b * T * r;
+__global__ __launch_bounds__(256) void band_seg_fill_kernel(const BandFill f) {
+  band_fill(f, (size_t)blockIdx.x * 256 + threadIdx.x, (size_t)gridDim.x * 256);
+}
+
+template <bool MOD>
+__device__ __forceinline__ Shift seg_shift_block(const float* __restrict__ pxu, const float* __restrict__ pyu, const SegUtt& u, int r, float* red) {
   const unsigned nfr = (unsigned)(u.bd.te - u.bd.tb) * (unsigned)r;
   float sx = 0.0f, nx = 0.0f, sy = 0.0f, ny = 0.0f;
   float vx[8], vy[8];
@@ -131,9 +114,10 @@
     float a = 0.f, c = 0.f, d = 0.f, e = 0.f;
     for (int q = 0; q < 4; ++q) { a += red[q]; c += red[4 + q]; d += red[8 + q]; e += red[12 + q]; }
     const Shift sh = shift_from_sums<MOD>(a, c, d, e, u.Sn, u.Tn);
-    w.hdr[1] = sh.cx2; w.hdr[2] = sh.cy2;
-    *w.shift_back() = shift_total<MOD>(sh, u.Sn, u.Tn);
-  }
+    red[16] = sh.cx2; red[17] = sh.cy2;
+  }
+  __syncthreads();
+  return Shift{red[16], red[17]};
 }
 
 template <bool MOD, int LANES>
@@ -183,13 +167,24 @@
   if (u.degenerate) return;
   const SegWs<LANES> w(ws + (size_t)b * seg_floats_per_utt<LANES>(T, S), T, S);
   const SegBand<MOD, LANES> g(ranges, b, T, r, u.bd);
+  const float* pxu = pxb + (size_t)b * T * r;
+  const float* pyu = pyb + (size_t)b * T * r;
+  __shared__ float red[18];
+  const Shift sh = seg_shift_block<MOD>(pxu, pyu, u, r, red);
+  const float cx2 = sh.cx2, cy2 = sh.cy2;
+  if (blockIdx.x == 0 && threadIdx.x == 0) {
+    int f = 0;
+    const int lo_b = g.rg[(size_t)min(u.bd.tb, u.bd.te - 1) * r], lo_e = g.rg[(size_t)(u.bd.te - 1) * r];
+    if (!(u.bd.sb >= lo_b && u.bd.sb <= lo_b + r - 1)) f |= kSegFlagNoOrigin;
+    if (!((u.bd.se >= lo_e && u.bd.se <= lo_e + r - 1) || (MOD && u.bd.se == lo_e + r))) f |= kSegFlagNoEnd;
+    *w.start_flags() = f;
+    w.hdr[1] = sh.cx2; w.hdr[2] = sh.cy2;
+    *w.shift_back() = shift_total<MOD>(sh, u.Sn, u.Tn);
+  }
   const int i = blockIdx.x * 256 + threadIdx.x;
   const int q = i / r, k = i - q * r;
   const int t = u.bd.tb + q;
   if (t > u.bd.te) return;
-  const float cx2 = w.hdr[1], cy2 = w.hdr[2];
-  const float* pxu = pxb + (size_t)b * T * r;
-  const float* pyu = pyb + (size_t)b * T * r;
   const int sb = u.bd.sb, tb = u.bd.tb, se = u.bd.se, te = u.bd.te;
   const int l0 = g.lo(t), lm = t > tb ? g.lo(t - 1) : l0, lp = t < te ? g.lo(t + 1) : l0;
   unsigned nan_acc = 0;
@@ -276,54 +271,37 @@
   if (l16 < LANES) m[basis * LANES + lg] = val;
 }
 
-template <bool MOD, int LANES>
-__global__ __launch_bounds__(64) void band_seg_prefix_kernel(const int32_t* __restrict__ boundary, float* __restrict__ ws, int T, int S) {
-  extern __shared__ __attribute__((aligned(16))) double mats[];
-  const int dir = blockIdx.x, b = blockIdx.y;
-  const SegUtt u = seg_utt<MOD>(boundary, b, S, T);
-  if (u.degenerate) return;
-  const SegGeom gm = seg_geom(u.D);
-  const SegWs<LANES> w(ws + (size_t)b * seg_floats_per_utt<LANES>(T, S), T, S);
-  const int lane = threadIdx.x, l16 = lane & 15, lg = l16 & (LANES - 1);
-  const int nm = (gm.K - 1) * LANES * LANES;
-  const double* m0 = w.mat(dir, 0);
-  for (int i = lane; i < nm; i += 64) mats[i] = m0[i];
-  const bool start_ok = (*w.flags() & (dir ? kSegFlagNoEnd : kSegFlagNoOrigin)) == 0;
-  double val = (lg == 0 && start_ok) ? 0.0 : kNegD;
-  if (lane < LANES) w.state(dir, 0)[lg] = val;
-  __syncthreads();
-  for (int g = 0; g + 1 < gm.K; ++g) {
-    const double* m = mats + (size_t)g * LANES * LANES;
-    double tt[LANES];
-    double best = kNegD;
-#pragma unroll
-    for (int i = 0; i < LANES; ++i) {
-      double si = val;
-      switch (i) {
-        case 0: break;
+template <int LANES>
+__device__ __forceinline__ void seg_mat_column(double (&mm)[LANES], const double* __restrict__ m, int lg) {
+#pragma unroll
+  for (int i = 0; i < LANES; ++i) mm[i] = m[((lg - i) & (LANES - 1)) * LANES + lg];
+}
+template <int LANES>
+__device__ __forceinline__ double seg_mat_vec(double val, const double (&mm)[LANES]) {
+  double tt[LANES];
+  double best = kNegD;
+#pragma unroll
+  for (int i = 0; i < LANES; ++i) {
+    double si = val;
+    switch (i) {
+      case 0: break;
 #define FTR_ROT(N) case N: si = seg_rord<N>(val); break;
-        FTR_ROT(1) FTR_ROT(2) FTR_ROT(3) FTR_ROT(4) FTR_ROT(5) FTR_ROT(6) FTR_ROT(7) FTR_ROT(8)
-        FTR_ROT(9) FTR_ROT(10) FTR_ROT(11) FTR_ROT(12) FTR_ROT(13) FTR_ROT(14) FTR_ROT(15)
+      FTR_ROT(1) FTR_ROT(2) FTR_ROT(3) FTR_ROT(4) FTR_ROT(5) FTR_ROT(6) FTR_ROT(7) FTR_ROT(8)
+      FTR_ROT(9) FTR_ROT(10) FTR_ROT(11) FTR_ROT(12) FTR_ROT(13) FTR_ROT(14) FTR_ROT(15)
 #undef FTR_ROT
-      }
-      const int src = (lg - i) & (LANES - 1);
-      tt[i] = si + m[src * LANES + lg];
-      best = fmax(best, tt[i]);
     }
-    if (best > kNegThreshD) {
-      float sum = 0.0f;
-#pragma unroll
-      for (int i = 0; i < LANES; ++i) sum += __builtin_amdgcn_exp2f((float)(tt[i] - best));
-      val = best + (double)__builtin_amdgcn_logf(sum);
-    } else {
-      val = kNegD;
-    }
-    if (lane < LANES) w.state(dir, g + 1)[lg] = val;
-  }
-}
-
-template <bool MOD, int LANES>
-__global__ __launch_bounds__(64) void band_seg_final_kernel(const int32_t* __restrict__ boundary, float* __restrict__ ws, int T, int S) {
+    tt[i] = si + mm[i];
+    best = fmax(best, tt[i]);
+  }
+  if (!(best > kNegThreshD)) return kNegD;
+  float sum = 0.0f;
+#pragma unroll
+  for (int i = 0; i < LANES; ++i) sum += __builtin_amdgcn_exp2f((float)(tt[i] - best));
+  return best + (double)__builtin_amdgcn_logf(sum);
+}
+
+template <bool MOD, int LANES>
+__global__ __launch_bounds__(128) void band_seg_final_kernel(const int32_t* __restrict__ boundary, float* __restrict__ ws, int T, int S) {
   extern __shared__ __attribute__((aligned(16))) float2 seg[];
   const int sg = blockIdx.x, dir = blockIdx.y, b = blockIdx.z;
   const SegUtt u = seg_utt<MOD>(boundary, b, S, T);
@@ -331,21 +309,63 @@
   const SegGeom gm = seg_geom(u.D);
   if (sg >= gm.K) return;
   const SegWs<LANES> w(ws + (size_t)b * seg_floats_per_utt<LANES>(T, S), T, S);
-  const int lane = threadIdx.x, l16 = lane & 15, lg = l16 & (LANES - 1);
+  const int lane = threadIdx.x & 63, l16 = lane & 15, lg = l16 & (LANES - 1);
+  const bool chain_wave = threadIdx.x < 64;
   double* pbuf = reinterpret_cast<double*>(seg + (size_t)(gm.L + 2 * kSegU) * LANES);
-  seg_stage<LANES>(seg, dir ? w.OB : w.OA, kRow0 + sg * gm.L, gm.L, lane, 64);
-  double val = w.state(dir, sg)[lg];
+  double val = kNegD;
+  if (chain_wave) {
+    const bool start_ok = (w.all_flags() & (dir ? kSegFlagNoEnd : kSegFlagNoOrigin)) == 0;
+    val = (lg == 0 && start_ok) ? 0.0 : kNegD;
+    double mc[LANES] = {}, mn[LANES] = {};
+    if (sg > 0) seg_mat_column<LANES>(mc, w.mat(dir, 0), lg);
+    for (int g = 0; g < sg; ++g) {
+      if (g + 1 < sg) seg_mat_column<LANES>(mn, w.mat(dir, g + 1), lg);
+      val = seg_mat_vec<LANES>(val, mc);
+#pragma unroll
+      for (int i = 0; i < LANES; ++i) mc[i] = mn[i];
+    }
+  } else {
+    seg_stage<LANES>(seg, dir ? w.OB : w.OA, kRow0 + sg * gm.L, gm.L, lane, 64);
+  }
   __syncthreads();
-  seg_chain<LANES, true>(seg, gm.L, lg, val, pbuf, lane < LANES);
+  if (chain_wave) seg_chain<LANES, true>(seg, gm.L, lg, val, pbuf, lane < LANES);
   __syncthreads();
   double* P = (dir ? w.QB : w.PA) + (size_t)(kRow0 + sg * gm.L) * LANES;
-  for (int i = lane; i < gm.L * LANES; i += 64) P[i] = pbuf[i];
+  for (int i = threadIdx.x; i < gm.L * LANES; i += 128) P[i] = pbuf[i];
+}
+
+struct SegAns { float ans; double ans2; bool off; };
+template <bool MOD, int LANES>
+__device__ __forceinline__ SegAns seg_ans(const SegUtt& u, const SegWs<LANES>& w, const SegBand<MOD, LANES>& g) {
+  const int flags = w.all_flags();
+  const int fl = flags & (kSegFlagBad | kSegFlagNaN);
+  const double pend = w.PA[g.slotA(u.bd.se, u.bd.te)];
+  const bool dead = (flags & (kSegFlagNoOrigin | kSegFlagNoEnd)) != 0 || !(pend > kNegThreshD);
+  SegAns a;
+  a.ans2 = pend;
+  a.off = fl != 0 || dead;
+  a.ans = fl ? __builtin_nanf("") : (dead ? -INFINITY : (float)((pend + *w.shift_back()) * 0.6931471805599453));
+  return a;
+}
+__device__ __forceinline__ float seg_ans_degenerate(const SegUtt& u) { return (u.Sn <= 0 || u.Tn <= 0) ? 0.0f : ((u.Sn == 1) ? 0.0f : -INFINITY); }
+template <bool MOD, int LANES>
+__device__ __forceinline__ float seg_ans_of(const int32_t* __restrict__ ranges, const int32_t* __restrict__ boundary, const float* __restrict__ ws,
+                                            int b, int T, int S, int r) {
+  const SegUtt u = seg_utt<MOD>(boundary, b, S, T);
+  if (u.degenerate) return seg_ans_degenerate(u);
+  const SegWs<LANES> w(const_cast<float*>(ws) + (size_t)b * seg_floats_per_utt<LANES>(T, S), T, S);
+  const SegBand<MOD, LANES> g(ranges, b, T, r, u.bd);
+  return seg_ans<MOD, LANES>(u, w, g).ans;
 }
 
 template <bool MOD, int LANES>
 __global__ __launch_bounds__(256) void band_seg_occupancy_kernel(const int32_t* __restrict__ ranges, const int32_t* __restrict__ boundary,
                                                                  const float* __restrict__ ws, float* __restrict__ ans,
-                                                                 float* __restrict__ gxb, float* __restrict__ gyb, int T, int S, int r) {
+                                                                 float* __restrict__ gxb, float* __restrict__ gyb, int T, int S, int r,
+                                                                 float* __restrict__ loss_out, int reduction, float loss_sign, int B) {
+  __shared__ float red[4];
+  if (loss_out && blockIdx.x == 0 && blockIdx.y == 0)
+    negated_reduce_block([&](int bb) { return seg_ans_of<MOD, LANES>(ranges, boundary, ws, bb, T, S, r); }, B, reduction, loss_out, loss_sign, red);
   const int b = blockIdx.y;
   const int i = blockIdx.x * 256 + threadIdx.x;
   const size_t cells = (size_t)T * r;
@@ -354,22 +374,19 @@
   float* gy_g = gyb + (size_t)b * cells;
   if (u.degenerate) {
     if ((size_t)i < cells) { gx_g[i] = 0.0f; gy_g[i] = 0.0f; }
-    if (i == 0) ans[b] = (u.Sn <= 0 || u.Tn <= 0) ? 0.0f : ((u.Sn == 1) ? 0.0f : -INFINITY);
+    if (i == 0) ans[b] = seg_ans_degenerate(u);
     return;
   }
   const SegWs<LANES> w(const_cast<float*>(ws) + (size_t)b * seg_floats_per_utt<LANES>(T, S), T, S);
   const SegBand<MOD, LANES> g(ranges, b, T, r, u.bd);
-  const int flags = *w.flags();
-  const int fl = flags & (kSegFlagBad | kSegFlagNaN);
+  const SegAns sa = seg_ans<MOD, LANES>(u, w, g);
+  const double ans2 = sa.ans2;
   const int sb = u.bd.sb, tb = u.bd.tb, se = u.bd.se, te = u.bd.te;
-  const double pend = w.PA[g.slotA(se, te)];
-  const double ans2 = pend;
-  const bool dead = (flags & (kSegFlagNoOrigin | kSegFlagNoEnd)) != 0 || !(pend > kNegThreshD);
-  if (i == 0) ans[b] = fl ? __builtin_nanf("") : (dead ? -INFINITY : (float)((ans2 + *w.shift_back()) * 0.6931471805599453));
+  if (i == 0) ans[b] = sa.ans;
   if ((size_t)i >= cells) return;
   const int t = i / r, k = i - t * r;
   float fx = 0.0f, fy = 0.0f;
-  if (!fl && !dead && t >= tb && t < te) {
+  if (!sa.off && t >= tb && t < te) {
     const int l0 = g.lo(t);
     const int s = l0 + k;
     if (s >= sb && s <= se) {
@@ -415,8 +432,17 @@
   return (size_t)B * (seg_lanes(r) == 8 ? seg_floats_per_utt<8>(T, S) : seg_floats_per_utt<16>(T, S));
 }
 
+BandFill mi_band_seg_fill(float* ws, int B, int T, int S, int r) {
+  const size_t per = mi_band_seg_workspace_floats(1, T, S, r);
+  if (!per || !ws || B <= 0) return BandFill{nullptr, 0, 0, nullptr, 0, 0};
+  const int lanes = seg_lanes(r);
+  float* hdr = lanes == 8 ? SegWs<8>(ws, T, S).hdr : SegWs<16>(ws, T, S).hdr;
+  return BandFill{reinterpret_cast<float2*>(ws), per / 2, 2 * seg_rows(T, S) * lanes, reinterpret_cast<int32_t*>(hdr), per, B};
+}
+
 int mi_band_seg(const float* pxb, const float* pyb, const int32_t* ranges, const int32_t* boundary, float* ws, size_t ws_floats,
-                float* ans, float* gxb, float* gyb, int B, int T, int S, int r, int modified, hipStream_t st) {
+                float* ans, float* gxb, float* gyb, int B, int T, int S, int r, int modified, hipStream_t st, bool filled,
+                float* loss_out, int reduction) {
   if (B == 0) return FTR_OK;
   const size_t need = mi_band_seg_workspace_floats(B, T, S, r);
   if (!need || !ws || ws_floats < need || (reinterpret_cast<uintptr_t>(ws) & 15) != 0) {
@@ -426,7 +452,6 @@
   const int lanes = seg_lanes(r);
   const size_t lds_t = seg_lds_bytes(T, S, lanes, false), lds_f = seg_lds_bytes(T, S, lanes, true);
   const unsigned cells_blocks = (unsigned)(((size_t)(T + 1) * r + 255) / 256);
-  const unsigned fill_blocks = (unsigned)((2 * seg_rows(T, S) * lanes + 255) / 256);
   const dim3 gseg(kSegMaxK, 2, B);
   constexpr size_t ceiling = 156 * 1024;
   const char* what = "mutual_information_band (segments)";
@@ -439,13 +464,16 @@
       int rcl = reserve_lds<transfer>(ceiling, what);
       if (rcl == FTR_OK) rcl = reserve_lds<final_k>(ceiling, what);
       if (rcl != FTR_OK) return rcl;
-      hipLaunchKernelGGL((band_seg_init_kernel<MODV, LV>), dim3(fill_blocks, B), dim3(256), 0, st, pxb, pyb, ranges, boundary, ws, T, S, r);
+      if (!filled) {
+        const BandFill f = mi_band_seg_fill(ws, B, T, S, r);
+        const size_t blocks = (f.n * (size_t)B + 255) / 256;
+        hipLaunchKernelGGL(band_seg_fill_kernel, dim3((unsigned)(blocks > 16384 ? 16384 : blocks)), dim3(256), 0, st, f);
+      }
       hipLaunchKernelGGL((band_seg_scatter_kernel<MODV, LV>), dim3(cells_blocks, B), dim3(256), 0, st, pxb, pyb, ranges, boundary, ws, T, S, r);
       hipLaunchKernelGGL(transfer, gseg, dim3(16 * LV), lds_t, st, boundary, ws, T, S);
-      hipLaunchKernelGGL((band_seg_prefix_kernel<MODV, LV>), dim3(2, B), dim3(64), sizeof(double) * (kSegMaxK - 1) * LV * LV, st, boundary, ws, T, S);
-      hipLaunchKernelGGL(final_k, gseg, dim3(64), lds_f, st, boundary, ws, T, S);
+      hipLaunchKernelGGL(final_k, gseg, dim3(128), lds_f, st, boundary, ws, T, S);
       hipLaunchKernelGGL((band_seg_occupancy_kernel<MODV, LV>), dim3((unsigned)(((size_t)T * r + 255) / 256), B), dim3(256), 0, st,
-                         ranges, boundary, ws, ans, gxb, gyb, T, S, r);
+                         ranges, boundary, ws, ans, gxb, gyb, T, S, r, loss_out, reduction, -1.0f, B);
       return FTR_OK;
     });
   });
diff --git a/tf-fast-rnnt_amd/csrc/pruned_logprobs.hip b/tf-fast-rnnt_amd/csrc/pruned_logprobs.hip
--- a/tf-fast-rnnt_amd/csrc/pruned_logprobs.hip
+++ b/tf-fast-rnnt_amd/csrc/pruned_logprobs.hip
@@ -7,25 +7,74 @@
 __device__ __forceinline__ float wave_max(float v) { return wave_max_dpp(v); }
 __device__ __forceinline__ float wave_sum(float v) { return wave_sum_dpp(v); }
 
-template <typename E, int NQ, bool HAT>
+struct BandRows { double delay_penalty; int T, S, r, modified; BandFill fill; };
+struct BandRow { int s, t, te, c; };
+__device__ __forceinline__ BandRow band_row_of(const BandRows& bd, const int32_t* __restrict__ symbols, const int32_t* __restrict__ ranges,
+                                               const int32_t* __restrict__ boundary, unsigned row, int blank, int C) {
+  const unsigned bt = row / (unsigned)bd.r, k = row - bt * (unsigned)bd.r;
+  const unsigned b = bt / (unsigned)bd.T;
+  BandRow o;
+  o.t = (int)(bt - b * (unsigned)bd.T);
+  o.s = ranges[(size_t)bt * bd.r] + (int)k;
+  o.te = boundary ? boundary[4 * b + 3] : bd.T;
+  o.c = blank;
+  if (o.s >= 0 && o.s < bd.S) o.c = min(max(symbols[(size_t)b * bd.S + o.s], 0), C - 1);
+  return o;
+}
+template <bool HAT>
+__device__ __forceinline__ void band_row_store(const BandRows& bd, const BandRow& o, float* __restrict__ pxb, float* __restrict__ pyb, size_t row,
+                                               float xb, float xs, float l, int blank) {
+  float vy = -INFINITY, vx = -INFINITY;
+  if (o.s >= 0 && o.s <= bd.S) {
+    if (HAT) {
+      hat_logprobs(xb, xs, l, o.c == blank, &vx, &vy);
+    } else {
+      vy = xb - l;
+    }
+    if (o.s < bd.S) {
+      if (!HAT) vx = xs - l;
+      if (!bd.modified && o.t == o.te) vx = -INFINITY;
+      if (bd.delay_penalty > 0.0) vx += (float)((((double)o.te - 1.0) / 2.0 - (double)o.t) * bd.delay_penalty);
+    }
+  }
+  pxb[row] = vx;
+  pyb[row] = vy;
+}
+
+template <typename E, int NQ, bool HAT, bool BAND>
 __global__ __launch_bounds__(256) void lse_rows_reg_kernel(const E* __restrict__ logits, float* __restrict__ lse,
-                                                           size_t rows, int C, int blank) {
+                                                           size_t rows, int C, int blank, const int32_t* __restrict__ symbols,
+                                                           const int32_t* __restrict__ ranges, const int32_t* __restrict__ boundary,
+                                                           float* __restrict__ pxb, float* __restrict__ pyb, const BandRows bd) {
   const int lane = threadIdx.x & 63;
-  const size_t rowi = (size_t)blockIdx.x * (blockDim.x >> 6) + (threadIdx.x >> 6);
-  if (rowi >= rows) return;
+  const unsigned wave = BAND ? (unsigned)__builtin_amdgcn_readfirstlane((int)(threadIdx.x >> 6)) : (threadIdx.x >> 6);
+  const size_t rowi = (size_t)blockIdx.x * (blockDim.x >> 6) + wave;
+  if (rowi >= rows) {
+    if (BAND) band_fill(bd.fill, (size_t)blockIdx.x * blockDim.x + threadIdx.x, (size_t)gridDim.x * blockDim.x);
+    return;
+  }
   const size_t row = rows - 1 - rowi;
   const int n4 = C >> 2;
   const f4 ninf = {-INFINITY, -INFINITY, -INFINITY, -INFINITY};
   const E* x = logits + row * C;
   f4 v[NQ];
+  float xbl = 0.0f;
 #pragma unroll
   for (int q = 0; q < NQ; ++q) {
     const int i = lane + 64 * q;
     v[q] = (i < n4) ? load4(x, i) : ninf;
     if (HAT) {
 #pragma unroll
-      for (int e = 0; e < 4; ++e) v[q][e] = (4 * i + e == blank) ? -INFINITY : v[q][e];
-    }
+      for (int e = 0; e < 4; ++e) {
+        if (BAND && 4 * i + e == blank) xbl = v[q][e];
+        v[q][e] = (4 * i + e == blank) ? -INFINITY : v[q][e];
+      }
+    }
+  }
+  BandRow br = {};
+  if (BAND) {
+    br = band_row_of(bd, symbols, ranges, boundary, (unsigned)row, blank, C);
+    band_fill(bd.fill, (size_t)blockIdx.x * blockDim.x + threadIdx.x, (size_t)gridDim.x * blockDim.x);
   }
   float m = -INFINITY;
 #pragma unroll
@@ -38,16 +87,40 @@
       sum += __expf(v[q][0] - m) + __expf(v[q][1] - m) + __expf(v[q][2] - m) + __expf(v[q][3] - m);
   }
   sum = wave_sum(sum);
-  if (lane == 0) lse[row] = m + __logf(sum);
-}
-
-template <typename E, bool VEC, bool HAT>
-__global__ void lse_rows_kernel(const E* __restrict__ logits, float* __restrict__ lse, size_t rows, int C, int blank) {
+  const float l = m + __logf(sum);
+  if (BAND) {
+    auto take = [&](int c) {
+      const int i4 = c >> 2, q0 = i4 >> 6, e0 = c & 3;
+      float pick = 0.0f;
+#pragma unroll
+      for (int q = 0; q < NQ; ++q) {
+#pragma unroll
+        for (int e = 0; e < 4; ++e) pick = (q == q0 && e == e0) ? v[q][e] : pick;
+      }
+      return __builtin_bit_cast(float, __builtin_amdgcn_readlane(__builtin_bit_cast(int, pick), i4 & 63));
+    };
+    const float xb = HAT ? __builtin_bit_cast(float, __builtin_amdgcn_readlane(__builtin_bit_cast(int, xbl), (blank >> 2) & 63)) : take(blank);
+    const float xs = take(br.c);
+    if (lane == 0) { lse[row] = l; band_row_store<HAT>(bd, br, pxb, pyb, row, xb, xs, l, blank); }
+  } else {
+    if (lane == 0) lse[row] = l;
+  }
+}
+
+template <typename E, bool VEC, bool HAT, bool BAND>
+__global__ void lse_rows_kernel(const E* __restrict__ logits, float* __restrict__ lse, size_t rows, int C, int blank,
+                                const int32_t* __restrict__ symbols, const int32_t* __restrict__ ranges, const int32_t* __restrict__ boundary,
+                                float* __restrict__ pxb, float* __restrict__ pyb, const BandRows bd) {
   const int lane = threadIdx.x & 63;
-  const size_t row = (size_t)blockIdx.x * (blockDim.x >> 6) + (threadIdx.x >> 6);
+  if (BAND) band_fill(bd.fill, (size_t)blockIdx.x * blockDim.x + threadIdx.x, (size_t)gridDim.x * blockDim.x);
+  const unsigned wave = BAND ? (unsigned)__builtin_amdgcn_readfirstlane((int)(threadIdx.x >> 6)) : (threadIdx.x >> 6);
+  const size_t row = (size_t)blockIdx.x * (blockDim.x >> 6) + wave;
   if (row >= rows) return;
   const E* x = logits + row * C;
+  BandRow br = {};
+  if (BAND) br = band_row_of(bd, symbols, ranges, boundary, (unsigned)row, blank, C);
   float m = -INFINITY;
+  float l;
   if (VEC) {
     const int n4 = C >> 2;
     for (int i = lane; i < n4; i += 64) {
@@ -69,14 +142,18 @@
       s += __expf(v[0] - m) + __expf(v[1] - m) + __expf(v[2] - m) + __expf(v[3] - m);
     }
     s = wave_sum(s);
-    if (lane == 0) lse[row] = m + __logf(s);
+    l = m + __logf(s);
   } else {
     for (int i = lane; i < C; i += 64) m = fmaxf(m, (HAT && i == blank) ? -INFINITY : elem_to_float(x[i]));
     m = wave_max(m);
     float s = 0.0f;
     for (int i = lane; i < C; i += 64) s += __expf(((HAT && i == blank) ? -INFINITY : elem_to_float(x[i])) - m);
     s = wave_sum(s);
-    if (lane == 0) lse[row] = m + __logf(s);
+    l = m + __logf(s);
+  }
+  if (lane == 0) {
+    lse[row] = l;
+    if (BAND) band_row_store<HAT>(bd, br, pxb, pyb, row, elem_to_float(x[blank]), elem_to_float(x[br.c]), l, blank);
   }
 }
 
@@ -205,19 +282,7 @@
 __global__ __launch_bounds__(256) void negated_reduce_kernel(const float* __restrict__ ans, int B, int reduction,
                                                              float* __restrict__ out, float sign) {
   __shared__ float red[4];
-  if (reduction == 0) {
-    for (int b = threadIdx.x; b < B; b += 256) out[b] = sign * ans[b];
-    return;
-  }
-  float s = 0.0f;
-  for (int b = threadIdx.x; b < B; b += 256) s += ans[b];
-  s = wave_sum(s);
-  if ((threadIdx.x & 63) == 0) red[threadIdx.x >> 6] = s;
-  __syncthreads();
-  if (threadIdx.x == 0) {
-    const float t = (red[0] + red[1]) + (red[2] + red[3]);
-    out[0] = sign * ((reduction == 1) ? t / (float)B : t);
-  }
+  negated_reduce_block([&](int b) { return ans[b]; }, B, reduction, out, sign, red);
 }
 }
 
@@ -228,25 +293,42 @@
 
 namespace {
 template <typename E>
-int lse_rows_of(const E* logits, float* lse, size_t rows, int C, int blank, int hat, hipStream_t st) {
+int lse_rows_of(const E* logits, float* lse, size_t rows, int C, int blank, int hat, hipStream_t st, const BandRows* band = nullptr,
+                const int32_t* symbols = nullptr, const int32_t* ranges = nullptr, const int32_t* boundary = nullptr, float* pxb = nullptr, float* pyb = nullptr) {
   if (rows == 0) return FTR_OK;
   { const int rc32 = require_rows_32bit("lse_rows", rows); if (rc32 != FTR_OK) return rc32; }
   const int wpb = 4;
   const unsigned blocks = (unsigned)((rows + wpb - 1) / wpb);
+  const BandRows bd = band ? *band : BandRows{};
   dispatch(hat != 0, [&](auto h) {
-    constexpr bool HAT = decltype(h)::value;
-    const bool vec4 = rows_vec4<E>(C, logits);
-    if (vec4 && C <= 2048)
-      dispatch_among<1, 2, 4, 8>(C <= 256 ? 1 : C <= 512 ? 2 : C <= 1024 ? 4 : 8, [&](auto n) {
-        hipLaunchKernelGGL((lse_rows_reg_kernel<E, decltype(n)::value, HAT>), dim3(blocks), dim3(64 * wpb), 0, st, logits, lse, rows, C, blank);
-      });
-    else
-      dispatch(vec4, [&](auto vec) {
-        hipLaunchKernelGGL((lse_rows_kernel<E, decltype(vec)::value, HAT>), dim3(blocks), dim3(64 * wpb), 0, st, logits, lse, rows, C, blank);
-      });
+    dispatch(band != nullptr, [&](auto bnd) {
+      constexpr bool HAT = decltype(h)::value, BAND = decltype(bnd)::value;
+      const bool vec4 = rows_vec4<E>(C, logits);
+      if (vec4 && C <= 2048)
+        dispatch_among<1, 2, 4, 8>(C <= 256 ? 1 : C <= 512 ? 2 : C <= 1024 ? 4 : 8, [&](auto n) {
+          hipLaunchKernelGGL((lse_rows_reg_kernel<E, decltype(n)::value, HAT, BAND>), dim3(blocks), dim3(64 * wpb), 0, st, logits, lse, rows, C, blank, symbols, ranges, boundary, pxb, pyb, bd);
+        });
+      else
+        dispatch(vec4, [&](auto vec) {
+          hipLaunchKernelGGL((lse_rows_kernel<E, decltype(vec)::value, HAT, BAND>), dim3(blocks), dim3(64 * wpb), 0, st, logits, lse, rows, C, blank, symbols, ranges, boundary, pxb, pyb, bd);
+        });
+    });
   });
   return check_launch("lse_rows");
 }
+}
+
+int pruned_band_fwd(const void* logits, int dtype, const int32_t* symbols, const int32_t* ranges, const int32_t* boundary,
+                    int blank, double delay_penalty, float* lse, float* pxb, float* pyb, int B, int T, int S, int C, int r,
+                    int modified, int hat, const BandFill& fill, hipStream_t st) {
+  const size_t rows = (size_t)B * T * r;
+  if (rows == 0) return FTR_OK;
+  { const int rc32 = require_rows_32bit("pruned_band_fwd", rows); if (rc32 != FTR_OK) return rc32; }
+  const BandRows bd{delay_penalty, T, S, r, modified, fill};
+  return dispatch_dtype(dtype, [&](auto tag) {
+    using E = typename decltype(tag)::type;
+    return lse_rows_of(static_cast<const E*>(logits), lse, rows, C, blank, hat, st, &bd, symbols, ranges, boundary, pxb, pyb);
+  });
 }
 
 int lse_rows(const float* logits, float* lse, size_t rows, int C, int blank, int hat, hipStream_t st) {
diff --git a/tf-fast-rnnt_amd/tf_fast_rnnt/_lib.py b/tf-fast-rnnt_amd/tf_fast_rnnt/_lib.py
--- a/tf-fast-rnnt_amd/tf_fast_rnnt/_lib.py
+++ b/tf-fast-rnnt_amd/tf_fast_rnnt/_lib.py
@@ -109,10 +109,18 @@
     "ftr_smoothed_logprobs_fused_bwd_am_w_f32": (_i, [_c_fp, _c_fp, _c_fp, _i, _f, _c_fp, _c_fp, _c_fp, _c_ip, _c_ip, _i, _f, _c_fp, _c_fp, _f, _c_fp, _c_fp, _i, _i, _i, _i, _i, _c_st]),
     "ftr_simple_logprobs_fused_bwd_am_w_columns": (_i, [_i, _i, _i]),
 }
+_BAND_LOSS_TAIL = [_c_ip, _c_ip, _c_ip, _i, ctypes.c_double, _i, _c_fp, ctypes.c_size_t, _c_fp, _c_fp, _c_fp, _c_fp, _c_fp, _i, _i, _i, _i, _i, _i]
+_BAND_LOSS_SIGNATURES = {
+    "ftr_pruned_band_loss_workspace_floats": (ctypes.c_size_t, [_i, _i, _i, _i]),
+    "ftr_pruned_band_loss_fwd_f32": (_i, [_c_fp] + _BAND_LOSS_TAIL + [_c_st]),
+    "ftr_hat_pruned_band_loss_fwd_f32": (_i, [_c_fp] + _BAND_LOSS_TAIL + [_c_st]),
+    "ftr_pruned_band_loss_fwd_dt": (_i, [_c_fp, _i] + _BAND_LOSS_TAIL + [_i, _c_st]),
+}
 EXPORTED_SYMBOLS = tuple(_SIGNATURES)
 LOWP_SYMBOLS = tuple(_LOWP_SIGNATURES)
 KD_SYMBOLS = tuple(_KD_SIGNATURES)
 FUSED_SYMBOLS = tuple(_FUSED_SIGNATURES)
+BAND_LOSS_SYMBOLS = tuple(_BAND_LOSS_SIGNATURES)
 FTR_KD_FULL, FTR_KD_COLLAPSED = 0, 1
 FTR_MI_WS_CLEAN = 1
 FTR_DTYPE_F32, FTR_DTYPE_BF16, FTR_DTYPE_FP16 = 0, 1, 2
@@ -127,7 +135,7 @@
                 f"{LIB_PATH} is missing: build the HIP extension first (python -c 'import __graft_entry__ as g; "
                 "g.build()' or make -C tf-fast-rnnt_amd/csrc).  tf_fast_rnnt has no CPU fallback.")
         handle = ctypes.CDLL(LIB_PATH)
-        for name, (restype, argtypes) in {**_SIGNATURES, **_LOWP_SIGNATURES, **_KD_SIGNATURES, **_FUSED_SIGNATURES}.items():
+        for name, (restype, argtypes) in {**_SIGNATURES, **_LOWP_SIGNATURES, **_KD_SIGNATURES, **_FUSED_SIGNATURES, **_BAND_LOSS_SIGNATURES}.items():
             fn = getattr(handle, name)
             fn.restype = restype
             fn.argtypes = argtypes
diff --git a/tf-fast-rnnt_amd/tf_fast_rnnt/rnnt_loss.py b/tf-fast-rnnt_amd/tf_fast_rnnt/rnnt_loss.py
--- a/tf-fast-rnnt_amd/tf_fast_rnnt/rnnt_loss.py
+++ b/tf-fast-rnnt_amd/tf_fast_rnnt/rnnt_loss.py
@@ -627,33 +627,31 @@
         x = logits.detach().contiguous()
         need = logits.requires_grad
         ctx.band = _band_path_ok(ranges, boundary, T, S, r)
+        ctx.meta = (int(termination_symbol), int(modified), int(code), bool(hat))
         if ctx.band:
             lse = torch.empty((B, T, r), dtype=torch.float32, device=x.device)
-            pxb = torch.empty((B, T, r), dtype=torch.float32, device=x.device)
-            pyb = torch.empty((B, T, r), dtype=torch.float32, device=x.device)
             gxb = torch.empty((B, T, r), dtype=torch.float32, device=x.device)
             gyb = torch.empty((B, T, r), dtype=torch.float32, device=x.device)
             ans = torch.empty((B,), dtype=torch.float32, device=x.device)
+            if B == 0:
+                return _negated_reduce_native(ans, code)
+            loss = torch.empty((B,) if code == 0 else (), dtype=torch.float32, device=x.device)
             with torch.cuda.device(x.device):
-                st = _stream_ptr(x)
-                _pruned_call("pruned_band_fwd", hat, x, (_ptr(symbols), _ptr(ranges), _ptr(boundary),
-                             int(termination_symbol), float(delay_penalty), _ptr(lse), _ptr(pxb), _ptr(pyb),
-                             B, T, S, C, r, int(modified)), (st,))
-                nws = _lib.lib().ftr_mutual_information_band_workspace_floats(B, T, S, r)
-                bws = torch.empty((nws,), dtype=torch.float32, device=x.device) if nws else None
-                _lib.call("ftr_mutual_information_band_ws_f32", _ptr(pxb), _ptr(pyb), _ptr(ranges), _ptr(boundary), _ptr(bws),
-                          nws, _ptr(ans), _ptr(gxb), _ptr(gyb), B, T, S, r, int(modified), st)
-                del bws
-            del pxb, pyb
+                nws = _lib.lib().ftr_pruned_band_loss_workspace_floats(B, T, S, r)
+                ws = torch.empty((nws,), dtype=torch.float32, device=x.device)
+                _pruned_call("pruned_band_loss_fwd", hat, x, (_ptr(symbols), _ptr(ranges), _ptr(boundary),
+                             int(termination_symbol), float(delay_penalty), int(code), _ptr(ws), nws, _ptr(lse), _ptr(gxb),
+                             _ptr(gyb), _ptr(ans), _ptr(loss), B, T, S, C, r, int(modified)), (_stream_ptr(x),))
+                del ws
             if need:
                 ctx.save_for_backward(x, symbols, ranges, lse, gxb, gyb, boundary)
+            return loss
         else:
             lse, px, py = _pruned_builder_fwd(x, symbols, ranges, boundary, termination_symbol, delay_penalty, modified, hat)
             ans, px_grad, py_grad = mi_forward_backward(px, py, boundary, need, ans_grad_is_one=True)
             del px, py
             if need:
                 ctx.save_for_backward(x, symbols, ranges, lse, px_grad, py_grad, boundary)
-        ctx.meta = (int(termination_symbol), int(modified), int(code), bool(hat))
         return _negated_reduce_native(ans, code)
 
     @staticmethod
```

Result: no change. 24580 utterances/s, median of 6 (+0.8%).
